# CPJKU/beat_this

Measured on AMD Instinct MI355X. Metric: audio-seconds processed/sec, higher is better.
Workload: dtype f32 activations, f16x3 products (3 x f16 MFMA on hi+lo operand halves, f32 accumulate); main-layer attention P.V: 2 x, probabilities as fp16 hi parts

## Files before the change

beat_this_amd/_lib.py:

```python
from __future__ import annotations

import ctypes as C
import os
import subprocess

import torch

PKG_DIR = os.path.dirname(os.path.abspath(__file__))
LIB_PATH = os.path.join(PKG_DIR, "libbeat_this_amd.so")
if os.environ.get("BT_DEV") == "1" and os.environ.get("BT_LIB_PATH"):
    LIB_PATH = os.environ["BT_LIB_PATH"]
SOURCES = ["gemm.hip", "gemm2.hip", "gemm3.hip", "gemm_mx8.hip", "attn.hip", "attn2.hip", "fused.hip", "fused2.hip", "qkv_front.hip", "frontend.hip", "logmel.hip",
           "tail.hip", "dbn.hip", "metrics.hip", "loss.hip", "data.hip", "train.hip", "optim.hip", "engine.hip"]
HEADERS = ["common.h", "chain.h", "kernels.h", "dropout.h", "train_mixed.inc", "attn_x3_loop.inc", "attn_hq2_loop.inc", os.path.join("..", "..", "include", "beat_this_amd.h")]

BT_OK, BT_ERR_ARG, BT_ERR_HIP, BT_ERR_WORKSPACE = 0, -1, -2, -3
ABI_VERSION = 600
PREC_F32, PREC_HALF, PREC_F32X3 = 0, 1, 3
OPT_X3_ATTN_P16, OPT_X3_GEMM_FP8, OPT_WS_GUARD = 1, 2, 3
MAX_LAYERS = 32
PROFILE_CATEGORIES = ["stem", "qkv_gemm", "attn_flash", "out_gemm", "ff1_gemm", "ff2_gemm", "conv_gemm",
                      "linear_gemm", "head", "ff_fused", "attn_freq_fused", "layer_tail"]

GEMM_EPI_STORE, GEMM_EPI_RESID, GEMM_EPI_QKV = 0, 1, 2
GEMM_F_RMS, GEMM_F_BIAS, GEMM_F_GELU, GEMM_F_OUT_F32, GEMM_F_A_F32, GEMM_F_CONV, GEMM_F_ROWMAP = 1, 2, 4, 8, 16, 32, 64


class PairWeights(C.Structure):
    _fields_ = [("dim", C.c_int32), ("heads", C.c_int32), ("w_qkvg", C.c_void_p * 2), ("b_gates", C.c_void_p),
                ("w_out", C.c_void_p * 2), ("w_ff1", C.c_void_p * 2), ("b_ff1", C.c_void_p),
                ("w_ff2", C.c_void_p * 2), ("b_ff2", C.c_void_p),
                ("w_ff_frag", C.c_void_p * 2), ("w_qkv_frag", C.c_void_p),
                ("w_outff_frag", C.c_void_p * 2), ("w_attnff_frag", C.c_void_p * 2),
                ("w_tail_frag", C.c_void_p),
                ("w_outff_frag_x3", C.c_void_p), ("w_attnff_frag_x3", C.c_void_p),
                ("w_qkvg_x3", C.c_void_p), ("w_out_x3", C.c_void_p), ("w_ff1_x3", C.c_void_p), ("w_ff2_x3", C.c_void_p),
                ("w_qkv_frag_x3", C.c_void_p),
                ("w_qkvg_f8", C.c_void_p), ("w_out_f8", C.c_void_p), ("w_ff1_f8", C.c_void_p), ("w_ff2_f8", C.c_void_p)]


class ModelDesc(C.Structure):
    _fields_ = [("transformer_dim", C.c_int32), ("n_layers", C.c_int32), ("sum_head", C.c_int32),
                ("partial_transformers", C.c_int32),
                ("bn1_scale", C.c_void_p), ("bn1_shift", C.c_void_p), ("stem_w", C.c_void_p), ("stem_b", C.c_void_p),
                ("front", (PairWeights * 2) * 3),
                ("conv_w", (C.c_void_p * 2) * 3), ("conv_b", C.c_void_p * 3),
                ("lin_w", C.c_void_p * 2), ("lin_b", C.c_void_p),
                ("layers", PairWeights * MAX_LAYERS),
                ("head_w", C.c_void_p), ("head_b", C.c_float * 2), ("rope", C.c_void_p), ("ff_mult", C.c_int32),
                ("norm_out_g", C.c_void_p), ("head_w_raw", C.c_void_p),
                ("conv_w_x3", C.c_void_p * 3), ("lin_w_x3", C.c_void_p), ("rope_len", C.c_int32)]


class LogmelTables(C.Structure):
    _fields_ = [("window", C.c_void_p), ("twiddle", C.c_void_p), ("mel_start", C.c_void_p),
                ("mel_len", C.c_void_p), ("mel_w", C.c_void_p)]


class GemmArgs(C.Structure):
    _fields_ = [("A", C.c_void_p), ("lda", C.c_int64), ("W", C.c_void_p), ("M", C.c_int32), ("N", C.c_int32),
                ("K", C.c_int32), ("epi", C.c_int32), ("flags", C.c_int32), ("bias", C.c_void_p),
                ("out", C.c_void_p), ("ldo", C.c_int64), ("x", C.c_void_p), ("ldx", C.c_int64),
                ("conv_C2", C.c_int32), ("conv_T", C.c_int32), ("conv_F", C.c_int32), ("gates", C.c_void_p),
                ("inner", C.c_int32), ("heads", C.c_int32), ("rope", C.c_void_p), ("pdiv", C.c_int32),
                ("pmod", C.c_int32), ("map_T", C.c_int32), ("map_F", C.c_int32)]


class AttnArgs(C.Structure):
    _fields_ = [("qkv", C.c_void_p), ("ld", C.c_int64), ("gates", C.c_void_p), ("out", C.c_void_p),
                ("n_seq", C.c_int32), ("L", C.c_int32), ("heads", C.c_int32), ("inner", C.c_int32),
                ("o_div", C.c_int32), ("o_outer", C.c_int64), ("o_inner", C.c_int64), ("o_tok", C.c_int64)]


class AttnFragArgs(C.Structure):
    _fields_ = [("q", C.c_void_p), ("k", C.c_void_p), ("v", C.c_void_p), ("gates", C.c_void_p), ("out", C.c_void_p),
                ("n_seq", C.c_int32), ("L", C.c_int32), ("heads", C.c_int32), ("inner", C.c_int32),
                ("nbp", C.c_int32), ("o_div", C.c_int32), ("o_outer", C.c_int64), ("o_inner", C.c_int64),
                ("o_tok", C.c_int64), ("x3", C.c_int32), ("out_f32", C.c_int32), ("status", C.c_void_p),
                ("scratch", C.c_void_p)]


class Gemm3Args(C.Structure):
    _fields_ = [("A", C.c_void_p), ("lda", C.c_int64), ("M", C.c_int32), ("K", C.c_int32), ("W", C.c_void_p),
                ("N", C.c_int32), ("epi", C.c_int32), ("bias", C.c_void_p), ("ssq_in", C.c_void_p),
                ("ssq_parts", C.c_int32), ("out", C.c_void_p), ("ldo", C.c_int64), ("x", C.c_void_p),
                ("ldx", C.c_int64), ("xb", C.c_void_p), ("ssq_out", C.c_void_p), ("n_seq", C.c_int32),
                ("L", C.c_int32), ("nbp", C.c_int32), ("heads", C.c_int32), ("rope", C.c_void_p), ("qf", C.c_void_p),
                ("kf", C.c_void_p), ("vf", C.c_void_p), ("gates", C.c_void_p), ("b_gates", C.c_void_p),
                ("no_resid", C.c_int32), ("gelu", C.c_int32), ("conv_C2", C.c_int32),
                ("conv_T", C.c_int32), ("conv_F", C.c_int32), ("x3", C.c_int32), ("status", C.c_void_p)]


class A2BPlan(C.Structure):
    _fields_ = [("n22", C.c_int64), ("n_frames", C.c_int64), ("result_words", C.c_int64), ("B", C.c_int32), ("T", C.c_int32),
                ("ws_bytes", C.c_size_t), ("off_wave22", C.c_size_t), ("off_spect", C.c_size_t), ("off_chunks", C.c_size_t),
                ("off_chunk_logits", C.c_size_t), ("off_logits", C.c_size_t), ("off_result", C.c_size_t),
                ("off_forward", C.c_size_t), ("forward_bytes", C.c_size_t)]


class TrainItem(C.Structure):
    _fields_ = [("row", C.c_int64), ("ann_begin", C.c_int64), ("ann_end", C.c_int64), ("n", C.c_int32),
                ("start_frame", C.c_int32), ("op_begin", C.c_int32), ("op_end", C.c_int32), ("has_downbeats", C.c_int32),
                ("reserved", C.c_int32)]


class TrainOp(C.Structure):
    _fields_ = [("start", C.c_int32), ("length", C.c_int32), ("kind", C.c_int32), ("part_begin", C.c_int32),
                ("part_end", C.c_int32)]


class TrainPart(C.Structure):
    _fields_ = [("new_off", C.c_int32), ("old_off", C.c_int32)]


class TrainArgs(C.Structure):
    _fields_ = [("B", C.c_int32), ("T", C.c_int32), ("dim", C.c_int32), ("hidden", C.c_int32), ("rope_len", C.c_int32),
                ("residual", C.c_int32), ("sum_head", C.c_int32), ("reserved", C.c_int32), ("rope", C.c_void_p),
                ("gamma", C.c_void_p), ("w1", C.c_void_p), ("b1", C.c_void_p), ("w2", C.c_void_p), ("b2", C.c_void_p),
                ("w3", C.c_void_p), ("x", C.c_void_p), ("y", C.c_void_p), ("y2", C.c_void_p), ("save_o", C.c_void_p),
                ("save_lse", C.c_void_p), ("gy", C.c_void_p), ("gy2", C.c_void_p), ("gx", C.c_void_p), ("g_gamma", C.c_void_p),
                ("g_w1", C.c_void_p), ("g_b1", C.c_void_p), ("g_w2", C.c_void_p), ("g_b2", C.c_void_p), ("g_w3", C.c_void_p),
                ("ws", C.c_void_p), ("ws_bytes", C.c_size_t)]


class TrainDropout(C.Structure):
    _fields_ = [("p", C.c_float), ("reserved", C.c_uint32), ("seed", C.c_uint64), ("stream", C.c_uint64)]


class OptimTensor(C.Structure):
    _fields_ = [("param", C.c_void_p), ("offset", C.c_int64), ("numel", C.c_int64), ("group", C.c_int32), ("reserved", C.c_int32)]


class OptimChunk(C.Structure):
    _fields_ = [("tensor", C.c_int32), ("chunk", C.c_int32)]


class OptimGroup(C.Structure):
    _fields_ = [("decay", C.c_float), ("one_minus_beta1", C.c_float), ("beta2", C.c_float), ("one_minus_beta2", C.c_float),
                ("step_size", C.c_float), ("bias2_sqrt", C.c_float), ("eps", C.c_float), ("reserved", C.c_float)]


OPTIM_MAX_GROUPS = 8


class OptimHyper(C.Structure):
    _fields_ = [("n_groups", C.c_int32), ("zero_grads", C.c_int32), ("grad_scale", C.c_float), ("reserved", C.c_int32),
                ("g", OptimGroup * OPTIM_MAX_GROUPS)]


G3_FF1, G3_RESID, G3_QKV = 0, 1, 2
UNIT_STEM, UNIT_PARTIAL, UNIT_CONV, UNIT_LINEAR, UNIT_ATTN, UNIT_FF, UNIT_NORM, UNIT_FRONT_ATTN, UNIT_FRONT_FF = range(9)
TRAIN_UNIT_HEAD = 16
TRAIN_DW_ROWS, TRAIN_CS_ROWS, TRAIN_ATTN_BLOCK = 1024, 64, 64
DROP_ATTN_P, DROP_ATTN_OUT, DROP_FF_HIDDEN, DROP_FF_OUT = range(4)
OPTIM_CHUNK, OPTIM_NORM_SLICE = 4096, 4096

EXPORTS = {
    "bt_last_error": (C.c_char_p, []),
    "bt_version": (C.c_int, []),
    "bt_half_is_bf16": (C.c_int, []),
    "bt_struct_sizes": (None, [C.POINTER(C.c_int32)]),
    "bt_engine_create": (C.c_int, [C.POINTER(ModelDesc), C.POINTER(C.c_void_p)]),
    "bt_engine_destroy": (None, [C.c_void_p]),
    "bt_engine_set_option": (C.c_int, [C.c_void_p, C.c_int, C.c_int]),
    "bt_engine_get_option": (C.c_int, [C.c_void_p, C.c_int, C.POINTER(C.c_int)]),
    "bt_workspace_bytes": (C.c_size_t, [C.c_void_p, C.c_int, C.c_int, C.c_int]),
    "bt_workspace_regions": (C.c_int, [C.c_void_p, C.c_int, C.c_int, C.c_int, C.POINTER(C.c_int64), C.c_int]),
    "bt_forward": (C.c_int, [C.c_void_p, C.c_void_p, C.c_int, C.c_void_p, C.c_int, C.c_int, C.c_void_p, C.c_size_t,
                             C.c_void_p, C.c_void_p]),
    "bt_forward_stages": (C.c_int, [C.c_void_p, C.c_void_p, C.c_int, C.c_int, C.c_int, C.c_void_p, C.c_int, C.c_int, C.c_void_p,
                                    C.c_size_t, C.c_void_p, C.c_void_p, C.c_void_p]),
    "bt_forward_unit": (C.c_int, [C.c_void_p, C.c_void_p, C.c_int, C.c_int, C.c_int, C.c_void_p, C.c_void_p, C.c_int, C.c_int,
                                  C.c_void_p, C.c_size_t]),
    "bt_split_chunks": (C.c_int, [C.c_void_p, C.c_void_p, C.c_int64, C.c_void_p, C.c_int, C.c_int, C.c_void_p]),
    "bt_aggregate": (C.c_int, [C.c_void_p, C.c_void_p, C.c_void_p, C.c_void_p, C.c_int, C.c_int, C.c_int, C.c_int64,
                               C.c_void_p, C.c_void_p]),
    "bt_logmel": (C.c_int, [C.c_void_p, C.POINTER(LogmelTables), C.c_void_p, C.c_int64, C.c_void_p]),
    "bt_resample": (C.c_int, [C.c_void_p, C.c_void_p, C.c_int64, C.c_int, C.c_int, C.c_void_p, C.c_int, C.c_void_p,
                              C.c_int64]),
    "bt_peaks": (C.c_int, [C.c_void_p, C.c_void_p, C.c_int64, C.c_int, C.c_void_p, C.c_void_p]),
    "bt_deduplicate_peaks_host": (C.c_int, [C.c_void_p, C.c_int, C.c_double, C.c_void_p, C.POINTER(C.c_int32)]),
    "bt_postprocess_host": (C.c_int, [C.c_void_p, C.c_int, C.c_void_p, C.c_int, C.c_double, C.c_void_p,
                                      C.POINTER(C.c_int32), C.c_void_p, C.POINTER(C.c_int32)]),
    "bt_audio2beats_plan": (C.c_int, [C.c_void_p, C.c_int64, C.c_int, C.c_int, C.c_int, C.POINTER(A2BPlan)]),
    "bt_audio2beats_enqueue": (C.c_int, [C.c_void_p, C.c_void_p, C.c_int, C.POINTER(LogmelTables), C.c_void_p, C.c_int64, C.c_int, C.c_int,
                                         C.c_void_p, C.c_int, C.c_void_p, C.c_size_t, C.c_void_p, C.c_int]),
    "bt_profile_begin": (None, [C.c_void_p]),
    "bt_profile_end": (C.c_int, [C.c_void_p, C.c_void_p, C.c_void_p, C.c_int]),
    "bt_resample_batch": (C.c_int, [C.c_void_p, C.c_void_p, C.c_int, C.c_int64, C.c_int, C.c_int, C.c_void_p, C.c_int,
                                    C.c_void_p]),
    "bt_logmel_batch": (C.c_int, [C.c_void_p, C.POINTER(LogmelTables), C.c_void_p, C.c_int, C.c_int64, C.c_void_p]),
    "bt_split_chunks_batch": (C.c_int, [C.c_void_p, C.c_void_p, C.c_void_p, C.c_int, C.c_int, C.c_void_p]),
    "bt_aggregate_batch": (C.c_int, [C.c_void_p, C.c_void_p, C.c_void_p, C.c_void_p, C.c_void_p, C.c_int, C.c_int64,
                                     C.c_int, C.c_int, C.c_void_p, C.c_void_p]),
    "bt_peaks_batch": (C.c_int, [C.c_void_p, C.c_void_p, C.c_void_p, C.c_int, C.c_void_p, C.c_void_p]),
    "bt_peaks_host": (C.c_int, [C.c_void_p, C.c_int64, C.c_void_p, C.POINTER(C.c_int32)]),
    "bt_gemm": (C.c_int, [C.c_void_p, C.c_int, C.POINTER(GemmArgs)]),
    "bt_attention": (C.c_int, [C.c_void_p, C.c_int, C.POINTER(AttnArgs)]),
    "bt_gemm3": (C.c_int, [C.c_void_p, C.POINTER(Gemm3Args)]),
    "bt_gemm_mx8": (C.c_int, [C.c_void_p, C.c_void_p, C.c_void_p, C.c_void_p, C.c_void_p, C.c_void_p, C.c_int, C.c_int, C.c_int, C.c_int64]),
    "bt_attn_frag_blocks": (C.c_int, [C.c_int]),
    "bt_attention_frag": (C.c_int, [C.c_void_p, C.POINTER(AttnFragArgs)]),
    "bt_qkv_front": (C.c_int, [C.c_void_p, C.c_int, C.POINTER(PairWeights), C.c_void_p, C.c_void_p, C.c_int, C.c_int, C.c_int,
                               C.c_void_p, C.c_void_p, C.c_void_p, C.c_void_p, C.c_int]),
    "bt_outff_fused": (C.c_int, [C.c_void_p, C.c_int, C.POINTER(PairWeights), C.c_void_p, C.c_void_p, C.c_int64, C.c_void_p]),
    "bt_attnff_fused": (C.c_int, [C.c_void_p, C.c_int, C.POINTER(PairWeights), C.c_void_p, C.c_void_p, C.c_int64]),
    "bt_layer_tail": (C.c_int, [C.c_void_p, C.POINTER(PairWeights), C.c_int, C.c_void_p, C.c_void_p, C.c_int64, C.c_void_p,
                                C.c_void_p]),
    "bt_ff_fused": (C.c_int, [C.c_void_p, C.c_int, C.POINTER(PairWeights), C.c_void_p, C.c_int64]),
    "bt_dbn_tables": (C.c_int, [C.c_double, C.c_double, C.c_double, C.c_int, C.c_double, C.c_double, C.c_double, C.c_void_p,
                                C.c_int, C.c_void_p, C.POINTER(C.c_size_t)]),
    "bt_dbn_workspace_bytes": (C.c_size_t, [C.c_void_p, C.c_int, C.c_int64]),
    "bt_dbn_decode": (C.c_int, [C.c_void_p, C.c_void_p, C.c_void_p, C.c_void_p, C.c_int, C.c_void_p, C.c_int, C.c_int64,
                                C.c_void_p, C.c_void_p, C.c_size_t]),
    "bt_dbn_viterbi": (C.c_int, [C.c_void_p, C.c_void_p, C.c_void_p, C.c_int, C.c_void_p, C.c_int64, C.c_void_p, C.c_void_p,
                                 C.c_void_p, C.c_size_t]),
    "bt_dbn_viterbi_host": (C.c_int, [C.c_void_p, C.c_int, C.c_void_p, C.c_int64, C.c_void_p, C.c_void_p]),
    "bt_dbn_host": (C.c_int, [C.c_void_p, C.c_void_p, C.c_void_p, C.c_int64, C.c_void_p, C.POINTER(C.c_int32)]),
    "bt_dbn_host_act": (C.c_int, [C.c_void_p, C.c_void_p, C.c_int64, C.c_void_p, C.POINTER(C.c_int32)]),
    "bt_beat_metrics_workspace_bytes": (C.c_size_t, [C.c_int, C.c_int64, C.c_int64]),
    "bt_beat_metrics": (C.c_int, [C.c_void_p, C.c_void_p, C.c_void_p, C.c_void_p, C.c_void_p, C.c_int, C.c_double, C.c_double,
                                  C.c_double, C.c_double, C.c_double, C.c_void_p, C.c_size_t, C.c_void_p]),
    "bt_beat_metrics_host": (C.c_int, [C.c_void_p, C.c_void_p, C.c_void_p, C.c_void_p, C.c_int, C.c_double, C.c_double,
                                       C.c_double, C.c_double, C.c_double, C.c_void_p]),
    "bt_bce_loss_workspace_bytes": (C.c_size_t, [C.c_int, C.c_int64]),
    "bt_bce_loss": (C.c_int, [C.c_void_p, C.c_int, C.c_int, C.c_float, C.c_void_p, C.c_void_p, C.c_int, C.c_void_p, C.c_int,
                              C.c_void_p, C.c_int, C.c_void_p, C.c_int, C.c_int64, C.c_int64, C.c_void_p, C.c_size_t,
                              C.c_void_p, C.c_void_p, C.c_void_p, C.c_int, C.c_void_p, C.c_void_p]),
    "bt_bce_loss_backward": (C.c_int, [C.c_void_p, C.c_void_p, C.c_int64, C.c_void_p, C.c_int, C.c_int64, C.c_void_p, C.c_int]),
    "bt_bce_loss_host": (C.c_int, [C.c_int, C.c_int, C.c_float, C.c_void_p, C.c_int, C.c_void_p, C.c_int, C.c_void_p, C.c_int,
                                   C.c_void_p, C.c_int, C.c_void_p, C.c_void_p, C.c_void_p, C.c_void_p, C.c_void_p]),
    "bt_train_batch_struct_sizes": (None, [C.POINTER(C.c_int32)]),
    "bt_train_batch": (C.c_int, [C.c_void_p, C.c_void_p, C.c_int, C.c_int64, C.c_void_p, C.c_int, C.c_int, C.c_void_p, C.c_int,
                                 C.c_void_p, C.c_int, C.c_void_p, C.c_void_p, C.c_int64, C.c_double, C.c_void_p, C.c_int,
                                 C.c_void_p, C.c_void_p, C.c_void_p, C.c_void_p]),
    "bt_train_batch_host": (C.c_int, [C.c_void_p, C.c_int, C.c_int64, C.c_void_p, C.c_int, C.c_int, C.c_void_p, C.c_int,
                                      C.c_void_p, C.c_int, C.c_void_p, C.c_void_p, C.c_int64, C.c_double, C.c_void_p, C.c_int,
                                      C.c_void_p, C.c_void_p, C.c_void_p, C.c_void_p]),
    "bt_train_struct_sizes": (None, [C.POINTER(C.c_int32)]),
    "bt_train_workspace_bytes": (C.c_size_t, [C.c_int, C.c_int, C.c_int, C.c_int, C.c_int, C.c_int]),
    "bt_train_forward": (C.c_int, [C.c_void_p, C.c_int, C.POINTER(TrainArgs)]),
    "bt_train_backward": (C.c_int, [C.c_void_p, C.c_int, C.POINTER(TrainArgs)]),
    "bt_train_dropout_struct_sizes": (None, [C.POINTER(C.c_int32)]),
    "bt_train_workspace_bytes_dropout": (C.c_size_t, [C.c_int, C.c_int, C.c_int, C.c_int, C.c_int, C.c_int]),
    "bt_train_forward_dropout": (C.c_int, [C.c_void_p, C.c_int, C.POINTER(TrainArgs), C.POINTER(TrainDropout)]),
    "bt_train_backward_dropout": (C.c_int, [C.c_void_p, C.c_int, C.POINTER(TrainArgs), C.POINTER(TrainDropout)]),
    "bt_philox4x32_10_host": (None, [C.POINTER(C.c_uint32), C.POINTER(C.c_uint32), C.POINTER(C.c_uint32)]),
    "bt_dropout_mask_host": (C.c_int, [C.POINTER(TrainDropout), C.c_int, C.c_int, C.c_int, C.c_int, C.c_int, C.c_void_p]),
    "bt_train_workspace_bytes_mixed": (C.c_size_t, [C.c_int, C.c_int, C.c_int, C.c_int, C.c_int, C.c_int, C.c_int]),
    "bt_train_forward_mixed": (C.c_int, [C.c_void_p, C.c_int, C.POINTER(TrainArgs), C.POINTER(TrainDropout)]),
    "bt_train_backward_mixed": (C.c_int, [C.c_void_p, C.c_int, C.POINTER(TrainArgs), C.POINTER(TrainDropout)]),
    "bt_train_matmul_mixed": (C.c_int, [C.c_void_p, C.c_int, C.c_void_p, C.c_void_p, C.c_int, C.c_int, C.c_int, C.c_void_p]),
    "bt_optim_struct_sizes": (None, [C.POINTER(C.c_int32)]),
    "bt_optim_plan": (C.c_int, [C.c_int, C.c_void_p, C.c_void_p, C.c_void_p, C.c_int, C.c_void_p, C.POINTER(C.c_int64), C.c_void_p,
                                C.c_int64, C.POINTER(C.c_int64)]),
    "bt_grad_norm_workspace_bytes": (C.c_size_t, [C.c_int64]),
    "bt_grad_norm": (C.c_int, [C.c_void_p, C.c_void_p, C.c_int64, C.c_float, C.c_float, C.c_void_p, C.c_size_t, C.c_void_p]),
    "bt_adamw_step": (C.c_int, [C.c_void_p, C.c_void_p, C.c_int, C.c_void_p, C.c_int64, C.c_void_p, C.c_void_p, C.c_void_p,
                                C.c_int64, C.POINTER(OptimHyper), C.c_void_p]),
    "bt_grad_norm_host": (C.c_int, [C.c_void_p, C.c_int64, C.c_float, C.c_float, C.c_void_p]),
    "bt_adamw_step_host": (C.c_int, [C.c_void_p, C.c_int, C.c_void_p, C.c_int64, C.c_void_p, C.c_void_p, C.c_void_p, C.c_int64,
                                     C.POINTER(OptimHyper), C.c_void_p]),
}


HIPCC_FLAGS = ["-Xclang", "-target-feature", "-Xclang", "-packed-fp32-ops", "-mllvm", "-amdgpu-mfma-vgpr-form"]
FLAGS_BY_SOURCE = {"tail.hip": ["-Xclang", "-target-feature", "-Xclang", "-packed-fp32-ops"],
                   "dbn.hip": HIPCC_FLAGS + ["-ffp-contract=off"],
                   "metrics.hip": HIPCC_FLAGS + ["-ffp-contract=off"],
                   "loss.hip": HIPCC_FLAGS + ["-ffp-contract=off"],
                   "data.hip": HIPCC_FLAGS + ["-ffp-contract=off"],
                   "optim.hip": HIPCC_FLAGS + ["-ffp-contract=off"]}
EXTRA_DEFINES = (["-DBT_DEV"] if os.environ.get("BT_DEV_BUILD") == "1" else []) + os.environ.get("BT_DEFINES", "").split()


def build(force: bool = False, verbose: bool = False, lib_path: str | None = None, obj_dir: str | None = None,
          defines=()) -> str:
    from concurrent.futures import ThreadPoolExecutor

    src_dir = os.path.join(PKG_DIR, "csrc")
    obj_dir = obj_dir or os.path.join(PKG_DIR, "build")
    LIB_PATH = lib_path or os.path.join(PKG_DIR, "libbeat_this_amd.so")
    hdrs = [os.path.join(src_dir, h) for h in HEADERS] + [os.path.abspath(__file__)]
    hdr_time = max(os.path.getmtime(h) for h in hdrs)
    hipcc = os.environ.get("HIPCC", "/opt/rocm/bin/hipcc")
    common = [hipcc, "--offload-arch=gfx950", "-O3", "-std=c++17", "-fPIC"]
    import hashlib

    stamp_path = os.path.join(obj_dir, "flags.stamp")
    stamp = hashlib.sha256(repr((common[1:], HIPCC_FLAGS, sorted(FLAGS_BY_SOURCE.items()), EXTRA_DEFINES, list(defines))).encode()).hexdigest()
    try:
        if open(stamp_path).read().strip() != stamp:
            force = True
    except OSError:
        force = True
    todo, objs = [], []
    for name in SOURCES:
        src = os.path.join(src_dir, name)
        obj = os.path.join(obj_dir, name.replace(".hip", ".o"))
        objs.append(obj)
        if force or not os.path.exists(obj) or os.path.getmtime(obj) < max(os.path.getmtime(src), hdr_time):
            todo.append((src, obj))
    build.last_rebuilt = [os.path.basename(j[0]) for j in todo]
    if not todo and os.path.exists(LIB_PATH) and all(os.path.getmtime(LIB_PATH) >= os.path.getmtime(o) for o in objs):
        return LIB_PATH
    os.makedirs(obj_dir, exist_ok=True)
    if os.path.exists(stamp_path):
        os.unlink(stamp_path)

    def compile_one(job):
        flags = FLAGS_BY_SOURCE.get(os.path.basename(job[0]), HIPCC_FLAGS)
        cmd = [*common, *flags, *EXTRA_DEFINES, *defines, "-c", job[0], "-o", job[1]]
        if verbose:
            print(" ".join(cmd), flush=True)
        r = subprocess.run(cmd, stderr=subprocess.PIPE, text=True)
        err = "\n".join(l for l in r.stderr.splitlines() if "-packed-fp32-ops' is not a recognized feature" not in l)
        if err.strip():
            print(err, flush=True)
        if r.returncode:
            raise subprocess.CalledProcessError(r.returncode, cmd)

    with ThreadPoolExecutor(max_workers=min(len(todo), os.cpu_count() or 4) or 1) as pool:
        list(pool.map(compile_one, todo))
    cmd = [hipcc, "--offload-arch=gfx950", "-shared", "-fPIC", *objs, "-o", LIB_PATH]
    if verbose:
        print(" ".join(cmd), flush=True)
    subprocess.run(cmd, check=True)
    with open(stamp_path, "w") as f:
        f.write(stamp + "\n")
    return LIB_PATH


build.last_rebuilt = []


def device_asm_command(src: str, out: str, defines=()) -> list:
    flags = FLAGS_BY_SOURCE.get(os.path.basename(src), HIPCC_FLAGS)
    return [os.environ.get("HIPCC", "/opt/rocm/bin/hipcc"), "--offload-arch=gfx950", "-O3", "-std=c++17", "-fPIC", *flags,
            *EXTRA_DEFINES, *defines, "-S", "--cuda-device-only", src, "-o", out]


_lib = None


def lib():
    global _lib
    if _lib is None:
        if not os.path.exists(LIB_PATH):
            raise ImportError(
                f"{LIB_PATH} is missing: build it with `python -c 'import __graft_entry__ as g; g.build()'` "
                "(needs hipcc); beat_this_amd has no CPU/PyTorch fallback")
        handle = C.CDLL(LIB_PATH, mode=C.RTLD_GLOBAL)
        handle.bt_version.restype = C.c_int
        if handle.bt_version() != ABI_VERSION:
            raise ImportError(f"{LIB_PATH} has ABI version {handle.bt_version()}, this binding needs {ABI_VERSION}: rebuild it "
                              "(python -c 'import __graft_entry__ as g; g.build()')")
        for name, (res, args) in EXPORTS.items():
            fn = getattr(handle, name)
            fn.restype = res
# ... 42 lines not shown
```

beat_this_amd/csrc/chain.h:

```cpp
#pragma once
#include "common.h"

template <typename T> DEVI Frag<T> ldg_frag(const T* p);
template <> DEVI Frag<float> ldg_frag<float>(const float* p) {
  Frag<float> f;
#pragma unroll
  for (int i = 0; i < 4; ++i) f.v[i] = reinterpret_cast<const f32x4*>(p)[i];
  return f;
}
template <> DEVI Frag<hf> ldg_frag<hf>(const hf* p) {
  Frag<hf> f;
  f.v[0] = reinterpret_cast<const hfx8*>(p)[0];
  f.v[1] = reinterpret_cast<const hfx8*>(p)[1];
  return f;
}

DEVI void split_hl8(Frag<hl>& f, int h, const float (&v)[8]) {
  typedef __attribute__((ext_vector_type(4))) unsigned int u32x4;
  unsigned hi[4], lo[4];
#pragma unroll
  for (int j = 0; j < 4; j += 2)
    split_hl4(v[2 * j] * OpScale<hl>::ACT, v[2 * j + 1] * OpScale<hl>::ACT, v[2 * j + 2] * OpScale<hl>::ACT,
              v[2 * j + 3] * OpScale<hl>::ACT, hi[j], lo[j], hi[j + 1], lo[j + 1]);
  f.v[h] = __builtin_bit_cast(hfx8, u32x4{hi[0], hi[1], hi[2], hi[3]});
  f.v[2 + h] = __builtin_bit_cast(hfx8, u32x4{lo[0], lo[1], lo[2], lo[3]});
}
template <> DEVI Frag<hl> ldg_frag<hl>(const hl* p) {
  Frag<hl> f;
  const f32x4* q = reinterpret_cast<const f32x4*>(p);
#pragma unroll
  for (int h = 0; h < 2; ++h) {
    const f32x4 a = q[2 * h], b = q[2 * h + 1];
    const float v[8] = {a[0], a[1], a[2], a[3], b[0], b[1], b[2], b[3]};
    split_hl8(f, h, v);
  }
  return f;
}

template <typename T> DEVI Frag<T> ldx_frag(const float* p, bool ok, float& ss);
template <> DEVI Frag<float> ldx_frag<float>(const float* p, bool ok, float& ss) {
  Frag<float> f;
#pragma unroll
  for (int i = 0; i < 4; ++i) {
    f.v[i] = ok ? reinterpret_cast<const f32x4*>(p)[i] : f32x4{0.f, 0.f, 0.f, 0.f};
#pragma unroll
    for (int j = 0; j < 4; ++j) ss = fmaf(f.v[i][j], f.v[i][j], ss);
  }
  return f;
}
template <> DEVI Frag<hf> ldx_frag<hf>(const float* p, bool ok, float& ss) {
  Frag<hf> f;
#pragma unroll
  for (int h = 0; h < 2; ++h) {
#pragma unroll
    for (int i = 0; i < 2; ++i) {
      f32x4 v = ok ? reinterpret_cast<const f32x4*>(p)[2 * h + i] : f32x4{0.f, 0.f, 0.f, 0.f};
#pragma unroll
      for (int j = 0; j < 4; ++j) {
        ss = fmaf(v[j], v[j], ss);
        f.v[h][4 * i + j] = (hf)v[j];
      }
    }
  }
  return f;
}

template <> DEVI Frag<hl> ldx_frag<hl>(const float* p, bool ok, float& ss) {
  Frag<hl> f;
#pragma unroll
  for (int h = 0; h < 2; ++h) {
    const f32x4 a = ok ? reinterpret_cast<const f32x4*>(p)[2 * h] : f32x4{0.f, 0.f, 0.f, 0.f};
    const f32x4 b = ok ? reinterpret_cast<const f32x4*>(p)[2 * h + 1] : f32x4{0.f, 0.f, 0.f, 0.f};
    const float v[8] = {a[0], a[1], a[2], a[3], b[0], b[1], b[2], b[3]};
#pragma unroll
    for (int j = 0; j < 8; ++j) ss = fmaf(v[j], v[j], ss);
    split_hl8(f, h, v);
  }
  return f;
}

template <typename T> DEVI Frag<T> pack_frag(const float (&h)[16]);
template <> DEVI Frag<float> pack_frag<float>(const float (&h)[16]) {
  Frag<float> f;
#pragma unroll
  for (int i = 0; i < 4; ++i) f.v[i] = f32x4{h[4 * i], h[4 * i + 1], h[4 * i + 2], h[4 * i + 3]};
  return f;
}
template <> DEVI Frag<hf> pack_frag<hf>(const float (&h)[16]) {
  Frag<hf> f;
#pragma unroll
  for (int s = 0; s < 2; ++s)
#pragma unroll
    for (int j = 0; j < 8; ++j) f.v[s][j] = (hf)h[8 * s + j];
  return f;
}

template <> DEVI Frag<hl> pack_frag<hl>(const float (&h)[16]) {
  Frag<hl> f;
#pragma unroll
  for (int s = 0; s < 2; ++s) {
    const float v[8] = {h[8 * s], h[8 * s + 1], h[8 * s + 2], h[8 * s + 3], h[8 * s + 4], h[8 * s + 5], h[8 * s + 6], h[8 * s + 7]};
    split_hl8(f, s, v);
  }
  return f;
}

DEVI void zero16(f32x16& a) {
#pragma unroll
  for (int r = 0; r < 16; ++r) a[r] = 0.f;
}

template <typename T> DEVI Frag<T> lds_frag(const char* tile, int lane);
template <> DEVI Frag<hf> lds_frag<hf>(const char* tile, int lane) {
  Frag<hf> f;
  f.v[0] = *reinterpret_cast<const hfx8*>(tile + lane * 16);
  f.v[1] = *reinterpret_cast<const hfx8*>(tile + 1024 + lane * 16);
  return f;
}
template <> DEVI Frag<hl> lds_frag<hl>(const char* tile, int lane) {
  Frag<hl> f;
#pragma unroll
  for (int i = 0; i < 4; ++i) f.v[i] = *reinterpret_cast<const hfx8*>(tile + i * 1024 + lane * 16);
  return f;
}
template <> DEVI Frag<float> lds_frag<float>(const char* tile, int lane) {
  Frag<float> f;
#pragma unroll
  for (int i = 0; i < 4; ++i) f.v[i] = *reinterpret_cast<const f32x4*>(tile + i * 1024 + lane * 16);
  return f;
}
```

beat_this_amd/csrc/engine.hip:

```cpp
#include <algorithm>
#include <cmath>
#include <cstddef>
#include <cstdio>
#include <cstring>
#include <mutex>
#include <string>
#include <vector>

#include "../../include/beat_this_amd.h"
#include "common.h"
#include "kernels.h"


static thread_local std::string g_err;
static int bt_set_error(int code, const std::string& msg) {
  g_err = msg;
  return code;
}
int bt_set_error_external(int code, const char* msg) { return bt_set_error(code, msg); }

namespace prof {
struct Rec { int cat; hipEvent_t a, b; };
struct State { bool on = false; std::vector<Rec> recs; };
struct Scope {
  State* st; size_t idx; hipStream_t s;
  Scope(State* state, int cat, hipStream_t stream) : st(state && state->on ? state : nullptr), idx(0), s(stream) {
    if (!st) return;
    Rec r; r.cat = cat;
    (void)hipEventCreate(&r.a); (void)hipEventCreate(&r.b);
    (void)hipEventRecord(r.a, s);
    idx = st->recs.size(); st->recs.push_back(r);
  }
  ~Scope() { if (st) (void)hipEventRecord(st->recs[idx].b, s); }
};
}

struct FwdGraph { int B, T, prec; void* ws; hipGraphExec_t exec; unsigned long stamp; };

struct bt_engine {
  bt_model_desc d;
  prof::State prof;
  std::mutex mu;
  std::vector<FwdGraph> graphs;
  unsigned long graph_clock = 0;
  hipStream_t cap_stream = nullptr;
  std::vector<int> warm;
  int x3_attn_p16 = 1;
  int x3_gemm_fp8 = 0;
  int ws_guard = 0;
};
enum { CAT_STEM = 0, CAT_QKV, CAT_ATTN_FLASH, CAT_OUT, CAT_FF1, CAT_FF2, CAT_CONV, CAT_LINEAR,
       CAT_HEAD, CAT_FF_FUSED, CAT_ATTN_FREQ_FUSED, CAT_LAYER_TAIL, CAT_COUNT };

namespace {

inline size_t align_up(size_t v, size_t a) { return (v + a - 1) / a * a; }

struct Workspace {
  float* xa; float* xb; float* xm; float* gates; void* xmb;
  void* qkv; void* ao; void* hid;
  void* qf; void* kf; void* vf; float* gates_h; int nbp;
  float* ssq[2];
  int* status;
  int* fix_mask;
  size_t total;
};

Workspace carve(char* base, int B, int T, int D, int ff_mult, int prec, size_t guard = 0,
                std::vector<int64_t>* regions = nullptr) {
  const bool x3 = prec == BT_PREC_F32X3;
  if (x3) prec = BT_PREC_F32;
  const size_t es = prec == BT_PREC_F32 ? 4 : 2;
  const size_t bt = (size_t)B * T;
  const size_t dmax = std::max<size_t>(1024, D);
  size_t off = 0;
  auto take = [&](size_t bytes) {
    size_t o = off;
    off += align_up(bytes, 256) + guard;
    if (regions) { regions->push_back((int64_t)o); regions->push_back((int64_t)(o + bytes)); }
    return base ? base + o : (char*)nullptr;
  };
  Workspace w;
  w.status = (int*)take(256);
  w.xa = (float*)take(bt * 1024 * 4);
  w.xb = (float*)take(bt * 1024 * 4);
  w.xm = (float*)take(bt * D * 4);
  w.xmb = take(bt * D * (x3 ? 4 : 2));
  w.gates = (float*)take(bt * std::max(32, D / 32) * 4);
  w.qkv = take(bt * 3 * dmax * es);
  w.ao = take(bt * dmax * es);
  w.hid = take(bt * std::max<size_t>(4 * 1024, (size_t)ff_mult * D) * es);
  w.nbp = attn_frag_blocks(T);
  w.qf = w.kf = w.vf = nullptr; w.gates_h = nullptr;
  if (prec == BT_PREC_HALF || x3) {
    const size_t sh = (size_t)B * std::max(32, D / 32);
    const size_t blk = x3 ? 4096 : 2048;
    w.qf = take(sh * w.nbp * blk); w.kf = take(sh * w.nbp * blk); w.vf = take(sh * w.nbp * blk);
    w.gates_h = (float*)take(sh * w.nbp * 32 * 4);
    w.fix_mask = x3 ? (int*)take(sh * w.nbp * 4) : nullptr;
    w.ssq[0] = (float*)take(bt * (D / 64 + 1) * 4);
    w.ssq[1] = (float*)take(bt * (D / 64 + 1) * 4);
  } else {
    w.ssq[0] = w.ssq[1] = nullptr;
    w.fix_mask = nullptr;
  }
  w.total = off;
  return w;
}

inline float* front_x(const Workspace& ws, int i) { return i & 1 ? ws.xb : ws.xa; }

StemP stem_params(const bt_model_desc& d, const float* spect, float* x, int B, int T) {
  StemP p;
  p.spect = spect; p.x = x; p.bn1_scale = d.bn1_scale; p.bn1_shift = d.bn1_shift;
  p.w = d.stem_w; p.bias = d.stem_b; p.B = B; p.T = T;
  return p;
}

GemmP conv_params(const bt_model_desc& d, int blk, int wp, const float* in, void* out, int B, int T, bool out_f32) {
  const int C = 32 << blk, F = 32 >> blk;
  GemmP g;
  memset(&g, 0, sizeof g);
  g.A = in; g.W = d.conv_w[blk][wp]; g.M = B * T * (F / 2); g.N = 2 * C; g.K = 6 * C;
  g.epi = GEMM_EPI_STORE; g.flags = GEMM_F_CONV | GEMM_F_A_F32 | GEMM_F_BIAS | GEMM_F_GELU | (out_f32 ? GEMM_F_OUT_F32 : 0);
  g.bias = d.conv_b[blk]; g.out = out; g.ldo = 2 * C;
  g.conv_C2 = 2 * C; g.conv_T = T; g.conv_F = F / 2;
  return g;
}

Gemm3P conv3_params(const bt_model_desc& d, const Workspace& ws, int blk, int B, int T, bool x3, bool out_half) {
  const int C = 32 << blk, F = 32 >> blk;
  float* out = front_x(ws, blk + 1);
  Gemm3P g;
  memset(&g, 0, sizeof g);
  g.A = ws.hid; g.lda = 2 * C; g.M = B * T * (F / 2); g.K = 6 * C; g.N = 2 * C;
  g.W = x3 ? d.conv_w_x3[blk] : d.conv_w[blk][BT_PREC_HALF];
  g.epi = G3_RESID; g.no_resid = 1; g.gelu = 1; g.bias = d.conv_b[blk]; g.ldx = 2 * C;
  g.conv_C2 = 2 * C; g.conv_T = T; g.conv_F = F / 2; g.x3 = x3; g.status = ws.status;
  g.x = out_half ? nullptr : out; g.xb = out_half ? (void*)out : nullptr;
  return g;
}

GemmP linear_params(const bt_model_desc& d, int wp, const float* in, float* out, void* xb, float* ssq_out, int B, int T) {
  GemmP g;
  memset(&g, 0, sizeof g);
  g.A = in; g.lda = 1024; g.W = d.lin_w[wp]; g.M = B * T; g.N = d.transformer_dim; g.K = 1024;
  g.epi = GEMM_EPI_STORE; g.flags = GEMM_F_A_F32 | GEMM_F_BIAS | GEMM_F_OUT_F32;
  g.bias = d.lin_b; g.out = out; g.ldo = d.transformer_dim; g.xb = xb; g.ssq_out = ssq_out;
  return g;
}

Gemm3P linear3_params(const bt_model_desc& d, const Workspace& ws, int B, int T, bool x3, bool out_f8) {
  const int D = d.transformer_dim;
  Gemm3P g;
  memset(&g, 0, sizeof g);
  g.A = front_x(ws, 3); g.lda = 1024; g.M = B * T; g.K = 1024; g.W = x3 ? d.lin_w_x3 : d.lin_w[BT_PREC_HALF]; g.N = D;
  g.epi = G3_RESID; g.no_resid = 1; g.bias = d.lin_b; g.x = ws.xm; g.ldx = D; g.xb = ws.xmb; g.ssq_out = ws.ssq[0];
  g.x3 = x3 ? 1 | (out_f8 ? G3_X3_OUT_F8 : 0) : 0; g.status = ws.status;
  return g;
}

HeadP head_params(const bt_model_desc& d, const float* x, const float* w, int prenorm, float* beat, float* downbeat, int M,
                  int* status) {
  HeadP p;
  p.x = x; p.w = w; p.b0 = d.head_b[0]; p.b1 = d.head_b[1];
  p.beat = beat; p.downbeat = downbeat; p.M = M; p.D = d.transformer_dim; p.sum_head = d.sum_head; p.prenorm = prenorm;
  p.status = status;
  return p;
}

template <class P>
void attn_rows(P& a, int B, int T, int F) {
  a.n_seq = B * F; a.L = T; a.o_div = F; a.o_outer = (long)T * F; a.o_inner = F > 1 ? 1 : 0; a.o_tok = F;
}

struct PairRoute {
  bool ff_fused;
  bool outff;
  bool split;
  bool time_frag;
};

struct FragLayer {
  bool qkv8;
  bool out8;
  bool ff8;
  bool next8;
  bool tail;
  bool shadow_dead;
};

enum { LAYERS_GENERIC, LAYERS_FRAG_HALF, LAYERS_FRAG_X3 };

struct Route {
  bool x3;
  int fp;
  int gp, wp;
  int x3_attn, x3_attn_front;
  bool half_shadow;
  int layers;
  struct Block { PairRoute freq, time; bool conv3; bool x_dead; } blk[3];
  bool lin3, lin_f8;
  struct Layer { PairRoute pair; FragLayer frag; } layer[BT_MAX_LAYERS];
};

#ifndef BT_SKIP_DEAD_STORES
#define BT_SKIP_DEAD_STORES 1
#endif
Route plan_route(const bt_engine& e, int B, int T, int prec, int first, int last, const Workspace& ws) {
  const bt_model_desc& d = e.d;
  const int D = d.transformer_dim;
  Route r;
  r.x3 = prec == BT_PREC_F32X3;
  r.fp = r.x3 ? BT_PREC_F32 : prec;
  r.gp = prec;
  r.wp = r.x3 ? BT_PREC_HALF : prec;
  r.x3_attn = r.x3 ? 4 | ((e.x3_attn_p16 == 1 || e.x3_attn_p16 == 2) ? BT_X3_P16 : 0) : 0;
  r.x3_attn_front = r.x3 ? 4 | (e.x3_attn_p16 >= 2 ? BT_X3_P16 : 0) : 0;
  auto pair = [&](const bt_pair_weights& w) {
    PairRoute p;
    p.ff_fused = w.dim <= 128 && w.w_ff_frag[r.fp];
    p.outff = p.ff_fused && w.w_outff_frag[r.fp] && w.w_attnff_frag[r.fp];
    p.split = r.x3 && w.w_outff_frag_x3 && w.w_attnff_frag_x3;
    p.time_frag = r.x3 ? p.outff && p.split && w.w_qkv_frag_x3 : p.ff_fused && r.fp == BT_PREC_HALF && w.w_qkv_frag;
    return p;
  };

  r.half_shadow = prec == BT_PREC_HALF && D >= 128 && D % 64 == 0;
  const long wide = (long)B * T * d.ff_mult * D;
  bool frag_x3 = r.x3 && D >= 128 && D % 128 == 0 && wide * 4 < 0x7fffffffL;
  for (int l = 0; frag_x3 && l < d.n_layers; ++l)
    frag_x3 = d.layers[l].w_qkvg_x3 && d.layers[l].w_out_x3 && d.layers[l].w_ff1_x3 && d.layers[l].w_ff2_x3;
  const bool frag_half = r.half_shadow && D % 128 == 0 && wide * 2 < 0x7fffffffL;
  r.layers = frag_x3 ? LAYERS_FRAG_X3 : frag_half ? LAYERS_FRAG_HALF : LAYERS_GENERIC;

  const bool lin3_fits = (frag_half || (frag_x3 && d.lin_w_x3)) && gemm3_supported(linear3_params(d, ws, B, T, frag_x3, false));
  for (int blk = 0; blk < 3; ++blk) {
    Route::Block& rb = r.blk[blk];
    rb.freq = pair(d.front[blk][0]);
    rb.time = pair(d.front[blk][1]);
    const Gemm3P cg = conv3_params(d, ws, blk, B, T, frag_x3, blk == 2 && lin3_fits);
    rb.conv3 = d.partial_transformers && rb.time.outff && (frag_x3 ? rb.time.split : frag_half) && cg.N >= 128 && cg.W &&
               gemm3_supported(cg);
    rb.x_dead = BT_SKIP_DEAD_STORES && rb.conv3 && frag_x3;
  }
  r.lin3 = lin3_fits && (!frag_x3 || r.blk[2].conv3);
  r.lin_f8 = r.lin3 && frag_x3 && e.x3_gemm_fp8 >= 2 && d.n_layers > 0 && d.layers[0].w_qkvg_f8;

  for (int l = 0; l < d.n_layers; ++l) {
    const bt_pair_weights& w = d.layers[l];
    FragLayer& f = r.layer[l].frag;
    r.layer[l].pair = pair(w);
    f.qkv8 = l == 0 ? first == 0 && r.lin_f8 : r.layer[l - 1].frag.next8;
    f.out8 = frag_x3 && e.x3_gemm_fp8 >= 2 && w.w_out_f8;
    f.ff8 = frag_x3 && e.x3_gemm_fp8 >= 1 && w.w_ff1_f8 && w.w_ff2_f8;
    f.next8 = frag_x3 && e.x3_gemm_fp8 >= 2 && l + 1 < d.n_layers && d.layers[l + 1].w_qkvg_f8 && w.w_ff2_f8;
    f.tail = frag_half && w.w_tail_frag && layer_tail_supported(D, d.ff_mult * D);
    f.shadow_dead = BT_SKIP_DEAD_STORES && frag_x3 && last == 2 && l == d.n_layers - 1;
  }
  return r;
}

#define CHECK_RC(what)                                                         \
  if (_rc != 0) {                                                              \
    char buf[160];                                                             \
    snprintf(buf, sizeof buf, "%s failed (code %d: %s)", what, _rc,            \
             _rc > 0 ? hipGetErrorString((hipError_t)_rc) : "bad arguments");  \
    return bt_set_error(_rc > 0 ? BT_ERR_HIP : BT_ERR_ARG, buf);               \
  }
#define LAUNCH(expr, what) \
  do { int _rc = (expr); CHECK_RC(what) } while (0)
#define LAUNCH_CAT(cat, st, expr, what) \
  do { int _rc; { prof::Scope _ps(pf, cat, st); _rc = (expr); } CHECK_RC(what) } while (0)


int check_rows(long M) {
  return M > 0x7fffffffL ? bt_set_error(BT_ERR_ARG, "batch too large for one forward call") : BT_OK;
}

int out_proj(prof::State* pf, const bt_pair_weights& pw, const Route& r, float* x, void* xs, const Workspace& ws, long M,
             hipStream_t s) {
  const int C = pw.dim;
  GemmP g;
  memset(&g, 0, sizeof g);
  g.A = ws.ao; g.lda = C; g.W = pw.w_out[r.wp]; g.M = (int)M; g.N = C; g.K = C;
  g.epi = GEMM_EPI_RESID; g.flags = 0; g.x = x; g.ldx = C; g.xb = xs;
  LAUNCH_CAT(CAT_OUT, s, launch_gemm(g, r.gp, s), "out-proj gemm");
  return BT_OK;
}

int qkv_attn(prof::State* pf, const bt_pair_weights& pw, const Route& r, const float* rope, float* x, void* xs,
             const Workspace& ws, int B, int T, int F, hipStream_t s) {
  const int C = pw.dim, H = pw.heads;
  GemmP g;
  memset(&g, 0, sizeof g);
  g.A = xs ? xs : (const void*)x; g.lda = C; g.W = pw.w_qkvg[r.wp]; g.M = B * T * F; g.N = 3 * C + H; g.K = C;
  g.epi = GEMM_EPI_QKV; g.flags = GEMM_F_RMS | (xs ? 0 : GEMM_F_A_F32) | (F > 1 ? GEMM_F_ROWMAP : 0);
  g.bias = pw.b_gates; g.out = ws.qkv; g.ldo = 3 * C; g.gates = ws.gates; g.inner = C; g.heads = H;
  g.rope = rope; g.map_T = T; g.map_F = F; g.pdiv = F; g.pmod = T;
  LAUNCH_CAT(CAT_QKV, s, launch_gemm(g, r.gp, s), "qkv gemm");
  AttnP a;
  memset(&a, 0, sizeof a);
  a.qkv = ws.qkv; a.ld = 3 * C; a.gates = ws.gates; a.out = ws.ao; a.heads = H; a.inner = C;
  attn_rows(a, B, T, F);
  LAUNCH_CAT(CAT_ATTN_FLASH, s, launch_attn_flash(a, r.gp, s), F > 1 ? "time attention" : "attention");
  return BT_OK;
}

int ff_half(prof::State* pf, const bt_pair_weights& pw, const PairRoute& pr, const Route& r, float* x, void* xs,
            const Workspace& ws, long M, int ff_mult, hipStream_t s) {
  const int C = pw.dim, HID = ff_mult * C;
  if (pr.ff_fused) {
    FusedFFP ff;
    ff.x = x; ff.M = M; ff.C = C; ff.wfrag = pw.w_ff_frag[r.fp]; ff.b1 = pw.b_ff1; ff.b2 = pw.b_ff2; ff.xb = xs;
    LAUNCH_CAT(CAT_FF_FUSED, s, launch_ff_fused(ff, r.fp, s), "fused feed-forward");
    return BT_OK;
  }
  GemmP g;
  memset(&g, 0, sizeof g);
  g.A = xs ? xs : (const void*)x; g.lda = C; g.W = pw.w_ff1[r.wp]; g.M = (int)M; g.N = HID; g.K = C;
  g.epi = GEMM_EPI_STORE; g.flags = GEMM_F_RMS | (xs ? 0 : GEMM_F_A_F32) | GEMM_F_BIAS | GEMM_F_GELU;
  g.bias = pw.b_ff1; g.out = ws.hid; g.ldo = HID;
  LAUNCH_CAT(CAT_FF1, s, launch_gemm(g, r.gp, s), "ff1 gemm");
  memset(&g, 0, sizeof g);
  g.A = ws.hid; g.lda = HID; g.W = pw.w_ff2[r.wp]; g.M = (int)M; g.N = C; g.K = HID;
  g.epi = GEMM_EPI_RESID; g.flags = GEMM_F_BIAS; g.bias = pw.b_ff2; g.x = x; g.ldx = C; g.xb = xs;
  LAUNCH_CAT(CAT_FF2, s, launch_gemm(g, r.gp, s), "ff2 gemm");
  return BT_OK;
}

int generic_layer(prof::State* pf, const bt_pair_weights& pw, const PairRoute& pr, const Route& r, const float* rope, float* x,
                  void* xs, const Workspace& ws, int B, int T, int ff_mult, bool attn, bool ff, hipStream_t s) {
  const long M = (long)B * T;
  if (int rc = check_rows(M)) return rc;
  if (attn) {
    if (int rc = qkv_attn(pf, pw, r, rope, x, xs, ws, B, T, 1, s)) return rc;
    if (int rc = out_proj(pf, pw, r, x, xs, ws, M, s)) return rc;
  }
  return ff ? ff_half(pf, pw, pr, r, x, xs, ws, M, ff_mult, s) : BT_OK;
}

int freq_half(prof::State* pf, const bt_pair_weights& pw, const PairRoute& pr, const Route& r, const float* rope, float* x,
              int B, int T, int F, hipStream_t s) {
  const long M = (long)B * T * F;
  if (int rc = check_rows(M)) return rc;
  if (!pr.outff) return bt_set_error(BT_ERR_ARG, "frequency-direction half needs bt_pair_weights.w_attnff_frag");
  FusedAttnFFP f;
  f.x = x; f.M = M; f.C = pw.dim; f.b_gates = pw.b_gates; f.rope = rope;
  f.wfrag = pr.split ? pw.w_attnff_frag_x3 : pw.w_attnff_frag[r.fp]; f.b1 = pw.b_ff1; f.b2 = pw.b_ff2;
  LAUNCH_CAT(CAT_ATTN_FREQ_FUSED, s, launch_attnff_fused(f, pr.split ? BT_PREC_F32X3 : r.fp, s),
             "fused frequency attention + feed-forward");
  return BT_OK;
}

int time_half(prof::State* pf, const bt_pair_weights& pw, const PairRoute& pr, const Route& r, const float* rope, float* x,
              const Workspace& ws, int B, int T, int F, void* shadow, bool shadow_only, hipStream_t s) {
  const long M = (long)B * T * F;
  if (int rc = check_rows(M)) return rc;
  if (pr.time_frag) {
    QkvFrontP qp;
    memset(&qp, 0, sizeof qp);
    qp.x = x; qp.B = B; qp.T = T; qp.F = F; qp.C = pw.dim; qp.wfrag = r.x3 ? pw.w_qkv_frag_x3 : pw.w_qkv_frag;
    qp.b_gates = pw.b_gates; qp.rope = rope;
    qp.q = ws.qf; qp.k = ws.kf; qp.v = ws.vf; qp.gates = ws.gates_h; qp.nbp = ws.nbp;
    qp.x3 = r.x3; qp.status = ws.status;
    LAUNCH_CAT(CAT_QKV, s, launch_qkv_front(qp, s), "frontend qkv projection");
    AttnFragP a;
    memset(&a, 0, sizeof a);
    a.q = ws.qf; a.k = ws.kf; a.v = ws.vf; a.gates = ws.gates_h; a.out = ws.ao; a.heads = pw.heads; a.inner = pw.dim;
    a.nbp = ws.nbp; attn_rows(a, B, T, F);
    a.x3 = r.x3_attn_front; a.out_f32 = 1; a.status = ws.status; a.fix_mask = ws.fix_mask;
    LAUNCH_CAT(CAT_ATTN_FLASH, s, launch_attn_frag(a, s), "time attention");
  } else if (int rc = qkv_attn(pf, pw, r, rope, x, nullptr, ws, B, T, F, s)) {
    return rc;
  }
  if (pr.outff) {
    FusedOutFFP f;
    f.x = x; f.M = M; f.C = pw.dim; f.ao = ws.ao; f.wfrag = pr.split ? pw.w_outff_frag_x3 : pw.w_outff_frag[r.fp];
    f.b1 = pw.b_ff1; f.b2 = pw.b_ff2; f.xb = shadow; f.abl = 0; f.shadow_only = shadow && shadow_only && pr.split;
    LAUNCH_CAT(CAT_FF_FUSED, s, launch_outff_fused(f, pr.split ? BT_PREC_F32X3 : r.fp, s), "fused out-projection + feed-forward");
    return BT_OK;
  }
  if (int rc = out_proj(pf, pw, r, x, nullptr, ws, M, s)) return rc;
  return ff_half(pf, pw, pr, r, x, nullptr, ws, M, 4, s);
}

int frag_layer(prof::State* pf, const bt_pair_weights& pw, const FragLayer& f, const Route& r, const float* rope,
               const Workspace& ws, int B, int T, int ff_mult, hipStream_t s) {
  const int D = pw.dim, H = pw.heads, HID = ff_mult * D;
  const int M = B * T;
  const int parts = D / 64;
  int* status = r.x3 ? ws.status : nullptr;
  auto w = [&](const void* const* half, const void* hl32, const void* hl8, bool f8) { return !r.x3 ? half[BT_PREC_HALF] : f8 ? hl8 : hl32; };
  Gemm3P g;
  memset(&g, 0, sizeof g);
  g.A = ws.xmb; g.lda = D; g.M = M; g.K = D; g.W = w(pw.w_qkvg, pw.w_qkvg_x3, pw.w_qkvg_f8, f.qkv8); g.N = 3 * D + H; g.epi = G3_QKV;
  g.ssq_in = ws.ssq[0]; g.ssq_parts = parts; g.x3 = r.x3 | (f.qkv8 ? G3_X3_F8 : 0); g.status = status;
  g.n_seq = B; g.L = T; g.nblk = (T + 31) / 32; g.nbp = ws.nbp; g.heads = H; g.inner = D; g.rope = rope;
  g.qf = ws.qf; g.kf = ws.kf; g.vf = ws.vf; g.gates = ws.gates_h; g.b_gates = pw.b_gates;
  LAUNCH_CAT(CAT_QKV, s, launch_gemm3(g, s), r.x3 ? "qkv gemm (hi + lo)" : "qkv gemm");
  AttnFragP a;
  memset(&a, 0, sizeof a);
  a.q = ws.qf; a.k = ws.kf; a.v = ws.vf; a.gates = ws.gates_h; a.out = ws.ao; a.heads = H; a.inner = D; a.nbp = ws.nbp;
  attn_rows(a, B, T, 1);
  a.x3 = r.x3_attn; a.out_f32 = f.out8 ? 2 : 0; a.status = status; a.fix_mask = ws.fix_mask;
  LAUNCH_CAT(CAT_ATTN_FLASH, s, launch_attn_frag(a, s), r.x3 ? "attention (hi + lo)" : "attention");
  if (f.tail) {
    LayerTailP t;
    t.x = ws.xm; t.M = M; t.C = D; t.hidden = HID; t.ao = ws.ao; t.wfrag = pw.w_tail_frag; t.b1 = pw.b_ff1; t.b2 = pw.b_ff2;
    t.xb = ws.xmb; t.ssq_out = ws.ssq[0];
    LAUNCH_CAT(CAT_LAYER_TAIL, s, launch_layer_tail(t, s), "layer tail (out-projection + feed-forward)");
    return BT_OK;
  }
  memset(&g, 0, sizeof g);
  g.A = ws.ao; g.lda = D; g.M = M; g.K = D; g.W = w(pw.w_out, pw.w_out_x3, pw.w_out_f8, f.out8); g.N = D; g.epi = G3_RESID;
  g.x3 = r.x3 | (f.out8 ? G3_X3_F8 : 0) | (f.ff8 ? G3_X3_OUT_F8 : 0); g.status = status;
  g.x = ws.xm; g.ldx = D; g.xb = ws.xmb; g.ssq_out = ws.ssq[1];
  LAUNCH_CAT(CAT_OUT, s, launch_gemm3(g, s), r.x3 ? "out-proj gemm (hi + lo)" : "out-proj gemm");
  memset(&g, 0, sizeof g);
  g.A = ws.xmb; g.lda = D; g.M = M; g.K = D; g.W = w(pw.w_ff1, pw.w_ff1_x3, pw.w_ff1_f8, f.ff8); g.N = HID; g.epi = G3_FF1;
  g.x3 = r.x3 | (f.ff8 ? G3_X3_F8 | G3_X3_OUT_F8 : 0); g.status = status;
  g.bias = pw.b_ff1; g.ssq_in = ws.ssq[1]; g.ssq_parts = parts; g.out = ws.hid; g.ldo = HID;
  LAUNCH_CAT(CAT_FF1, s, launch_gemm3(g, s), r.x3 ? "ff1 gemm (hi + lo)" : "ff1 gemm");
  memset(&g, 0, sizeof g);
  g.A = ws.hid; g.lda = HID; g.M = M; g.K = HID; g.W = w(pw.w_ff2, pw.w_ff2_x3, pw.w_ff2_f8, f.ff8); g.N = D; g.epi = G3_RESID;
  g.x3 = r.x3 | (f.ff8 ? G3_X3_F8 : 0) | (f.next8 ? G3_X3_OUT_F8 : 0); g.status = status;
  g.bias = pw.b_ff2; g.x = ws.xm; g.ldx = D; g.xb = f.shadow_dead ? nullptr : ws.xmb; g.ssq_out = f.shadow_dead ? nullptr : ws.ssq[0];
  LAUNCH_CAT(CAT_FF2, s, launch_gemm3(g, s), r.x3 ? "ff2 gemm (hi + lo)" : "ff2 gemm");
  return BT_OK;
}

int frontend(prof::State* pf, const bt_model_desc& d, const Route& r, const float* spect, const Workspace& ws, int B, int T,
             hipStream_t s) {
  const StemP sp = stem_params(d, spect, front_x(ws, 0), B, T);
  LAUNCH_CAT(CAT_STEM, s, launch_stem(sp, s), "stem");
  for (int blk = 0; blk < 3; ++blk) {
    const Route::Block& rb = r.blk[blk];
    float* x = front_x(ws, blk);
    if (d.partial_transformers) {
      if (int rc = freq_half(pf, d.front[blk][0], rb.freq, r, d.rope, x, B, T, 32 >> blk, s)) return rc;
      if (int rc = time_half(pf, d.front[blk][1], rb.time, r, d.rope, x, ws, B, T, 32 >> blk, rb.conv3 ? ws.hid : nullptr, rb.x_dead, s))
        return rc;
    }
    if (rb.conv3) {
      const Gemm3P g = conv3_params(d, ws, blk, B, T, r.layers == LAYERS_FRAG_X3, blk == 2 && r.lin3);
      LAUNCH_CAT(CAT_CONV, s, launch_gemm3(g, s), "frontend conv gemm");
    } else {
      const GemmP g = conv_params(d, blk, r.wp, x, front_x(ws, blk + 1), B, T, !(blk == 2 && r.lin3));
      LAUNCH_CAT(CAT_CONV, s, launch_gemm(g, r.gp, s), "frontend conv gemm");
    }
  }
  if (r.lin3) {
    const Gemm3P g = linear3_params(d, ws, B, T, r.layers == LAYERS_FRAG_X3, r.lin_f8);
    LAUNCH_CAT(CAT_LINEAR, s, launch_gemm3(g, s), "frontend linear gemm");
    return BT_OK;
  }
  const GemmP g = linear_params(d, r.wp, front_x(ws, 3), ws.xm, r.half_shadow ? ws.xmb : nullptr,
                                r.layers == LAYERS_FRAG_HALF ? ws.ssq[0] : nullptr, B, T);
  LAUNCH_CAT(CAT_LINEAR, s, launch_gemm(g, r.gp, s), "frontend linear gemm");
  if (r.layers == LAYERS_FRAG_X3)
    LAUNCH_CAT(CAT_LINEAR, s, launch_shadow_ssq(ws.xm, ws.xmb, ws.ssq[0], (long)B * T, d.transformer_dim, s, 1), "hl32 shadow of the residual stream");
  return BT_OK;
}

}

extern "C" {

const char* bt_last_error(void) { return g_err.c_str(); }
int bt_version(void) { return BT_ABI_VERSION; }
int bt_half_is_bf16(void) { return BT_HALF_IS_BF16; }
void bt_struct_sizes(int32_t* out) {
  out[0] = (int32_t)sizeof(bt_pair_weights); out[1] = (int32_t)sizeof(bt_model_desc);
  out[2] = (int32_t)sizeof(bt_logmel_tables); out[3] = (int32_t)sizeof(bt_gemm_args);
  out[4] = (int32_t)sizeof(bt_attn_args); out[5] = (int32_t)offsetof(bt_model_desc, layers);
  out[6] = (int32_t)offsetof(bt_model_desc, rope);
  out[7] = (int32_t)sizeof(bt_attn_frag_args);
  out[8] = (int32_t)sizeof(bt_gemm3_args);
}

int bt_engine_create(const bt_model_desc* desc, bt_engine** out) {
  if (!desc || !out) return bt_set_error(BT_ERR_ARG, "null argument");
  if (desc->transformer_dim % 32 || desc->transformer_dim < 32 || desc->transformer_dim > 1024 ||
      desc->n_layers < 0 || desc->n_layers > BT_MAX_LAYERS || desc->ff_mult < 1 || desc->ff_mult > 16)
    return bt_set_error(BT_ERR_ARG, "unsupported transformer_dim / n_layers / ff_mult");
  bt_engine* e = new bt_engine;
  e->d = *desc;
  *out = e;
  return BT_OK;
}
static void drop_graphs(bt_engine* e) {
  for (auto& g : e->graphs) (void)hipGraphExecDestroy(g.exec);
  e->graphs.clear();
  e->warm.clear();
}
void bt_engine_destroy(bt_engine* e) {
  if (!e) return;
  for (auto& r : e->prof.recs) { (void)hipEventDestroy(r.a); (void)hipEventDestroy(r.b); }
  drop_graphs(e);
  if (e->cap_stream) (void)hipStreamDestroy(e->cap_stream);
  delete e;
}

int bt_engine_set_option(bt_engine* e, int option, int value) {
  if (!e) return bt_set_error(BT_ERR_ARG, "null argument");
  std::lock_guard<std::mutex> lock(e->mu);
  if (option == BT_OPT_X3_ATTN_P16 && value >= 0 && value <= 3) { if (e->x3_attn_p16 != value) drop_graphs(e); e->x3_attn_p16 = value; return BT_OK; }
  if (option == BT_OPT_X3_GEMM_FP8 && value >= 0 && value <= 2) { if (e->x3_gemm_fp8 != value) drop_graphs(e); e->x3_gemm_fp8 = value; return BT_OK; }
  if (option == BT_OPT_WS_GUARD && value >= 0 && value % 256 == 0) { if (e->ws_guard != value) drop_graphs(e); e->ws_guard = value; return BT_OK; }
  return bt_set_error(BT_ERR_ARG, "unknown engine option / value");
}
int bt_engine_get_option(const bt_engine* e, int option, int* value) {
  if (!e || !value) return bt_set_error(BT_ERR_ARG, "null argument");
  if (option == BT_OPT_X3_ATTN_P16) { *value = e->x3_attn_p16; return BT_OK; }
  if (option == BT_OPT_X3_GEMM_FP8) { *value = e->x3_gemm_fp8; return BT_OK; }
  if (option == BT_OPT_WS_GUARD) { *value = e->ws_guard; return BT_OK; }
  return bt_set_error(BT_ERR_ARG, "unknown engine option");
}

size_t bt_workspace_bytes(const bt_engine* e, int B, int T, int prec) {
  if (!e || B <= 0 || T <= 0) return 0;
  return carve(nullptr, B, T, e->d.transformer_dim, e->d.ff_mult, prec, (size_t)e->ws_guard).total;
}

int bt_workspace_regions(const bt_engine* e, int B, int T, int prec, int64_t* begin_end, int max) {
  if (!e || B <= 0 || T <= 0 || max < 0 || (max > 0 && !begin_end)) return bt_set_error(BT_ERR_ARG, "bad argument to bt_workspace_regions");
  if (prec != BT_PREC_F32 && prec != BT_PREC_HALF && prec != BT_PREC_F32X3) return bt_set_error(BT_ERR_ARG, "unknown precision");
  std::vector<int64_t> r;
  carve(nullptr, B, T, e->d.transformer_dim, e->d.ff_mult, prec, (size_t)e->ws_guard, &r);
  const int n = (int)(r.size() / 2);
  for (int i = 0; i < std::min(n, max); ++i) { begin_end[2 * i] = r[2 * i]; begin_end[2 * i + 1] = r[2 * i + 1]; }
  return n;
}

int bt_forward(bt_engine* e, void* stream, int prec, const float* d_spect, int B, int T, void* d_ws, size_t ws_bytes,
               float* d_beat, float* d_downbeat) {
  return bt_forward_stages(e, stream, prec, 0, 2, d_spect, B, T, d_ws, ws_bytes, nullptr, d_beat, d_downbeat);
}

int bt_forward_stages(bt_engine* e, void* stream, int prec, int first, int last, const float* d_spect, int B, int T, void* d_ws,
                      size_t ws_bytes, float* d_out, float* d_beat, float* d_downbeat) {
  if (!e || !d_spect || !d_ws) return bt_set_error(BT_ERR_ARG, "null argument");
  if (first < 0 || last > 2 || first > last) return bt_set_error(BT_ERR_ARG, "stages: need 0 <= first <= last <= 2");
  if (last == 2 ? (!d_beat || !d_downbeat) : !d_out) return bt_set_error(BT_ERR_ARG, "null output");
  const int max_T = e->d.rope_len > 0 ? e->d.rope_len : 1536;
  if (B <= 0 || T <= 0 || T > max_T)
    return bt_set_error(BT_ERR_ARG, "need B >= 1 and 1 <= T <= " + std::to_string(max_T) + " (bt_model_desc.rope_len: rows of the rotary table)");
  if (prec != BT_PREC_F32 && prec != BT_PREC_HALF && prec != BT_PREC_F32X3)
    return bt_set_error(BT_ERR_ARG, "unknown precision");
  const bt_model_desc& d = e->d;
  prof::State* pf = &e->prof;
  const int D = d.transformer_dim;
  const Workspace ws = carve((char*)d_ws, B, T, D, d.ff_mult, prec, (size_t)e->ws_guard);
  if (ws.total > ws_bytes) return bt_set_error(BT_ERR_WORKSPACE, "workspace too small");
  if (prec == BT_PREC_F32X3 && BT_HALF_IS_BF16) return bt_set_error(BT_ERR_ARG, "BT_PREC_F32X3 needs an IEEE fp16 build");
  const Route r = plan_route(*e, B, T, prec, first, last, ws);
  hipStream_t s = (hipStream_t)stream;
  if (r.x3) LAUNCH(launch_clear_words(ws.status, 1, s), "clearing the range flag");
  int* status = r.x3 ? ws.status : nullptr;

  const size_t xm_bytes = (size_t)B * T * D * 4;
  if (first == 2) {
    if (!d.head_w_raw) return bt_set_error(BT_ERR_ARG, "stage entry at task_heads needs head_w_raw");
    const HeadP hp = head_params(d, d_spect, d.head_w_raw, 1, d_beat, d_downbeat, B * T, nullptr);
    LAUNCH_CAT(CAT_HEAD, s, launch_head(hp, s), "head");
    return BT_OK;
  }
  if (first == 1) {
    if (hipMemcpyAsync(ws.xm, d_spect, xm_bytes, hipMemcpyDeviceToDevice, s) != hipSuccess)
      return bt_set_error(BT_ERR_HIP, "copy of the stage input");
    if (r.half_shadow)
      LAUNCH_CAT(CAT_LINEAR, s, launch_shadow_ssq(ws.xm, ws.xmb, r.layers == LAYERS_FRAG_HALF ? ws.ssq[0] : nullptr, (long)B * T, D, s), "stage entry");
    if (r.layers == LAYERS_FRAG_X3) LAUNCH_CAT(CAT_LINEAR, s, launch_shadow_ssq(ws.xm, ws.xmb, ws.ssq[0], (long)B * T, D, s, 1), "stage entry");
  }
  if (first == 0)
    if (int rc = frontend(pf, d, r, d_spect, ws, B, T, s)) return rc;
  if (last == 0) {
    if (hipMemcpyAsync(d_out, ws.xm, xm_bytes, hipMemcpyDeviceToDevice, s) != hipSuccess)
      return bt_set_error(BT_ERR_HIP, "copy of the stage output");
    if (r.x3) LAUNCH_CAT(CAT_HEAD, s, launch_finite_rows(ws.xm, (long)B * T, D, ws.status, s), "range check of the stage output");
    return BT_OK;
  }
  for (int l = 0; l < d.n_layers; ++l) {
    const Route::Layer& rl = r.layer[l];
    const int rc = r.layers == LAYERS_GENERIC
                       ? generic_layer(pf, d.layers[l], rl.pair, r, d.rope, ws.xm, r.half_shadow ? ws.xmb : nullptr, ws, B, T,
                                       d.ff_mult, true, true, s)
                       : frag_layer(pf, d.layers[l], rl.frag, r, d.rope, ws, B, T, d.ff_mult, s);
    if (rc) return rc;
  }
  if (last == 1) {
    if (!d.norm_out_g) return bt_set_error(BT_ERR_ARG, "stage exit after transformer_blocks needs norm_out_g");
    LAUNCH_CAT(CAT_HEAD, s, launch_norm_out(ws.xm, d.norm_out_g, d_out, (long)B * T, D, s, status), "final norm");
    return BT_OK;
  }
  const HeadP hp = head_params(d, ws.xm, d.head_w, 0, d_beat, d_downbeat, B * T, status);
  LAUNCH_CAT(CAT_HEAD, s, launch_head(hp, s), "head");
  return BT_OK;
}

int bt_forward_unit(bt_engine* e, void* stream, int prec, int unit, int index, const float* d_in, float* d_out, int B, int T,
                    void* d_ws, size_t ws_bytes) {
  if (!e || !d_in || !d_out || !d_ws) return bt_set_error(BT_ERR_ARG, "null argument");
  const bt_model_desc& d = e->d;
  const int max_T = d.rope_len > 0 ? d.rope_len : 1536;
  if (B <= 0 || T <= 0 || T > max_T) return bt_set_error(BT_ERR_ARG, "need B >= 1 and 1 <= T <= bt_model_desc.rope_len");
  if (prec == BT_PREC_F32X3) prec = BT_PREC_F32;
  if (prec != BT_PREC_F32 && prec != BT_PREC_HALF) return bt_set_error(BT_ERR_ARG, "unknown precision");
  prof::State* pf = &e->prof;
  const int D = d.transformer_dim;
  const Workspace ws = carve((char*)d_ws, B, T, D, d.ff_mult, prec, (size_t)e->ws_guard);
  if (ws.total > ws_bytes) return bt_set_error(BT_ERR_WORKSPACE, "workspace too small");
  const Route r = plan_route(*e, B, T, prec, 0, 0, ws);
  hipStream_t s = (hipStream_t)stream;
  const bool block_unit = unit == BT_UNIT_PARTIAL || unit == BT_UNIT_CONV;
  const bool layer_unit = unit == BT_UNIT_ATTN || unit == BT_UNIT_FF;
  const bool leaf_unit = unit == BT_UNIT_FRONT_ATTN || unit == BT_UNIT_FRONT_FF;
  if (leaf_unit && (index < 0 || index > 5 || !d.partial_transformers)) return bt_set_error(BT_ERR_ARG, "partial-transformer leaf index out of range");
  if (block_unit && (index < 0 || index > 2)) return bt_set_error(BT_ERR_ARG, "frontend block index out of range");
  if (layer_unit && (index < 0 || index >= d.n_layers)) return bt_set_error(BT_ERR_ARG, "layer index out of range");
  auto copy_in = [&](size_t bytes) -> int {
    if (d_in != d_out && hipMemcpyAsync(d_out, d_in, bytes, hipMemcpyDeviceToDevice, s) != hipSuccess)
      return bt_set_error(BT_ERR_HIP, "copy of the unit's input");
    return BT_OK;
  };
  switch (unit) {
    case BT_UNIT_STEM: {
      const StemP sp = stem_params(d, d_in, d_out, B, T);
      LAUNCH_CAT(CAT_STEM, s, launch_stem(sp, s), "stem");
      return BT_OK;
    }
    case BT_UNIT_PARTIAL: {
      if (!d.partial_transformers) return bt_set_error(BT_ERR_ARG, "this model has no partial transformers");
      const Route::Block& rb = r.blk[index];
      if (int rc = copy_in((size_t)B * T * 1024 * 4)) return rc;
      if (int rc = freq_half(pf, d.front[index][0], rb.freq, r, d.rope, d_out, B, T, 32 >> index, s)) return rc;
      return time_half(pf, d.front[index][1], rb.time, r, d.rope, d_out, ws, B, T, 32 >> index, nullptr, false, s);
    }
    case BT_UNIT_CONV: {
      const GemmP g = conv_params(d, index, r.wp, d_in, d_out, B, T, true);
      LAUNCH_CAT(CAT_CONV, s, launch_gemm(g, r.gp, s), "frontend conv gemm");
      return BT_OK;
    }
    case BT_UNIT_LINEAR: {
      const GemmP g = linear_params(d, r.wp, d_in, d_out, nullptr, nullptr, B, T);
      LAUNCH_CAT(CAT_LINEAR, s, launch_gemm(g, r.gp, s), "frontend linear gemm");
      return BT_OK;
    }
    case BT_UNIT_ATTN:
    case BT_UNIT_FF: {
      if (int rc = copy_in((size_t)B * T * D * 4)) return rc;
      return generic_layer(pf, d.layers[index], r.layer[index].pair, r, d.rope, d_out, nullptr, ws, B, T, d.ff_mult,
                           unit == BT_UNIT_ATTN, unit == BT_UNIT_FF, s);
    }
    case BT_UNIT_FRONT_ATTN:
    case BT_UNIT_FRONT_FF: {
      const bt_pair_weights& pw = d.front[index >> 1][index & 1];
      const Route::Block& rb = r.blk[index >> 1];
      if (int rc = copy_in((size_t)B * T * pw.dim * 4)) return rc;
      return generic_layer(pf, pw, index & 1 ? rb.time : rb.freq, r, d.rope, d_out, nullptr, ws, B, T, 4,
                           unit == BT_UNIT_FRONT_ATTN, unit == BT_UNIT_FRONT_FF, s);
    }
    case BT_UNIT_NORM:
      if (!d.norm_out_g) return bt_set_error(BT_ERR_ARG, "bt_model_desc.norm_out_g is not set");
      LAUNCH_CAT(CAT_HEAD, s, launch_norm_out(d_in, d.norm_out_g, d_out, (long)B * T, D, s), "final norm");
      return BT_OK;
    default:
      return bt_set_error(BT_ERR_ARG, "unknown unit");
  }
// ... 184 lines not shown
  plan->off_wave22 = take(up == down ? 0 : (size_t)n22 * 4);
  plan->off_spect = take((size_t)n * 128 * 4);
  plan->off_logits = take((size_t)2 * n * 4);
  plan->off_result = take((size_t)plan->result_words * 4);
  plan->ws_bytes = off;
  return BT_OK;
}

int bt_audio2beats_enqueue(bt_engine* e, void* stream, int prec, const bt_logmel_tables* t, const float* d_audio, int64_t n_in,
                           int up, int down, const float* d_filter, int half_len, void* d_ws, size_t ws_bytes, int32_t* h_result,
                           int use_graph) {
  if (!e || !t || !d_audio || !d_ws || !h_result) return bt_set_error(BT_ERR_ARG, "null argument");
  if (up != down && (!d_filter || half_len < 0)) return bt_set_error(BT_ERR_ARG, "resampling needs the polyphase filter");
  bt_a2b_plan pl;
  if (int rc = bt_audio2beats_plan(e, n_in, up, down, prec, &pl)) return rc;
  if (pl.ws_bytes > ws_bytes) return bt_set_error(BT_ERR_WORKSPACE, "workspace too small (bt_audio2beats_plan)");
  std::lock_guard<std::mutex> lock(e->mu);
  const int max_T = e->d.rope_len > 0 ? e->d.rope_len : 1536;
  if (pl.T > max_T) return bt_set_error(BT_ERR_ARG, "chunk longer than the rotary table");
  hipStream_t s = (hipStream_t)stream;
  char* ws = (char*)d_ws;
  float* wave22 = (float*)(ws + pl.off_wave22);
  float* spect = (float*)(ws + pl.off_spect);
  float* chunks = (float*)(ws + pl.off_chunks);
  float* cb = (float*)(ws + pl.off_chunk_logits);
  float* cd = cb + (size_t)pl.B * pl.T;
  float* beat = (float*)(ws + pl.off_logits);
  float* downb = beat + pl.n_frames;
  int32_t* res = (int32_t*)(ws + pl.off_result);
  void* fws = ws + pl.off_forward;
  const int border = 6;
  const float* a22 = d_audio;
  if (up != down) {
    const bt_span_t one{d_audio, (long)n_in, 0, (long)pl.n22};
    LAUNCH(launch_resample(one, nullptr, 1, (long)pl.n22, up, down, d_filter, half_len, wave22, s), "resample");
    a22 = wave22;
  }
  LogmelP lp;
  fill_logmel(lp, t, spect);
  lp.one = bt_span_t{a22, (long)pl.n22, 0, (long)pl.n_frames};
  lp.tracks = nullptr; lp.n_tracks = 1; lp.max_frames = (long)pl.n_frames;
  LAUNCH(launch_logmel(lp, s), "logmel");
  LAUNCH(launch_split(spect, (long)pl.n_frames, nullptr, nullptr, pl.B, pl.T, chunks, s, border), "split");
  const int warm_key = prec << 8 | pl.B;
  const bool graphable = use_graph && pl.T == 1500 && pl.B <= 16 && !e->prof.on &&
                         std::find(e->warm.begin(), e->warm.end(), warm_key) != e->warm.end();
  FwdGraph* g = nullptr;
  if (graphable) {
    for (auto& c : e->graphs)
      if (c.B == pl.B && c.T == pl.T && c.prec == prec && c.ws == d_ws) g = &c;
    if (!g) {
      hipGraph_t graph = nullptr;
      if (!e->cap_stream && hipStreamCreateWithFlags(&e->cap_stream, hipStreamNonBlocking) != hipSuccess) e->cap_stream = nullptr;
      if (e->cap_stream && hipStreamBeginCapture(e->cap_stream, hipStreamCaptureModeThreadLocal) == hipSuccess) {
        const int rc = bt_forward_stages(e, e->cap_stream, prec, 0, 2, chunks, pl.B, pl.T, fws, pl.forward_bytes, nullptr, cb, cd);
        const hipError_t he = hipStreamEndCapture(e->cap_stream, &graph);
        hipGraphExec_t exec = nullptr;
        if (rc == BT_OK && he == hipSuccess && graph && hipGraphInstantiate(&exec, graph, nullptr, nullptr, 0) == hipSuccess) {
          if (e->graphs.size() >= 8) {
            size_t old = 0;
            for (size_t i = 1; i < e->graphs.size(); ++i)
              if (e->graphs[i].stamp < e->graphs[old].stamp) old = i;
            (void)hipGraphExecDestroy(e->graphs[old].exec);
            e->graphs.erase(e->graphs.begin() + old);
          }
          e->graphs.push_back(FwdGraph{pl.B, pl.T, prec, d_ws, exec, 0});
          g = &e->graphs.back();
        }
        if (graph) (void)hipGraphDestroy(graph);
        (void)hipGetLastError();
      }
    }
  }
  if (g) {
    g->stamp = ++e->graph_clock;
    if (hipGraphLaunch(g->exec, s) != hipSuccess) return bt_set_error(BT_ERR_HIP, "replay of the captured forward");
  } else {
    if (int rc = bt_forward_stages(e, s, prec, 0, 2, chunks, pl.B, pl.T, fws, pl.forward_bytes, nullptr, cb, cd)) return rc;
    if (pl.T == 1500 && pl.B <= 16 && std::find(e->warm.begin(), e->warm.end(), warm_key) == e->warm.end()) e->warm.push_back(warm_key);
  }
  LAUNCH(launch_aggregate(cb, cd, nullptr, nullptr, nullptr, 1, pl.B, pl.T, border, (long)pl.n_frames, beat, downb, s), "aggregate");
  LAUNCH(launch_peaks(beat, (long)pl.n_frames, nullptr, 2, res, res + 2 * pl.n_frames, s), "peaks");
  if (prec == BT_PREC_F32X3) {
    if (hipMemcpyAsync(res + 2 * pl.n_frames + 2, fws, 4, hipMemcpyDeviceToDevice, s) != hipSuccess)
      return bt_set_error(BT_ERR_HIP, "copy of the range flag");
  } else if (hipMemsetAsync(res + 2 * pl.n_frames + 2, 0, 4, s) != hipSuccess) {
    return bt_set_error(BT_ERR_HIP, "clearing the range flag");
  }
  if (hipMemcpyAsync(h_result, res, (size_t)pl.result_words * 4, hipMemcpyDeviceToHost, s) != hipSuccess)
    return bt_set_error(BT_ERR_HIP, "device-to-host copy of the result");
  return BT_OK;
}

void bt_profile_begin(bt_engine* e) {
  if (!e) return;
  for (auto& r : e->prof.recs) { (void)hipEventDestroy(r.a); (void)hipEventDestroy(r.b); }
  e->prof.recs.clear();
  e->prof.on = true;
}

int bt_profile_end(bt_engine* e, double* ms_by_category, int32_t* launches_by_category, int n_categories) {
  if (!e) return bt_set_error(BT_ERR_ARG, "null engine");
  e->prof.on = false;
  if (!ms_by_category || !launches_by_category || n_categories < CAT_COUNT)
    return bt_set_error(BT_ERR_ARG, "need room for BT_PROFILE_CATEGORIES entries");
  for (int i = 0; i < n_categories; ++i) { ms_by_category[i] = 0.0; launches_by_category[i] = 0; }
  for (auto& r : e->prof.recs) {
    hipError_t e = hipEventSynchronize(r.b);
    float ms = 0.f;
    if (e == hipSuccess) e = hipEventElapsedTime(&ms, r.a, r.b);
    if (e != hipSuccess) return bt_set_error(BT_ERR_HIP, hipGetErrorString(e));
    ms_by_category[r.cat] += ms;
    launches_by_category[r.cat] += 1;
    (void)hipEventDestroy(r.a); (void)hipEventDestroy(r.b);
  }
  e->prof.recs.clear();
  return BT_OK;
}

int bt_ff_fused(void* stream, int prec, const bt_pair_weights* w, float* d_x, int64_t M) {
  if (!w || !d_x || M <= 0 || w->dim > 128 || !w->w_ff_frag[prec]) return bt_set_error(BT_ERR_ARG, "bad argument to bt_ff_fused");
  FusedFFP ff;
  ff.x = d_x; ff.M = M; ff.C = w->dim; ff.wfrag = w->w_ff_frag[prec]; ff.b1 = w->b_ff1; ff.b2 = w->b_ff2;
  ff.xb = nullptr;
  LAUNCH(launch_ff_fused(ff, prec, (hipStream_t)stream), "fused feed-forward");
  return BT_OK;
}

int bt_gemm(void* stream, int prec, const bt_gemm_args* a) {
  if (!a) return bt_set_error(BT_ERR_ARG, "null argument");
  GemmP g;
  memset(&g, 0, sizeof g);
  g.A = a->A; g.lda = a->lda; g.W = a->W; g.M = a->M; g.N = a->N; g.K = a->K; g.epi = a->epi; g.flags = a->flags;
  g.bias = a->bias; g.out = a->out; g.ldo = a->ldo; g.x = a->x; g.ldx = a->ldx;
  g.conv_C2 = a->conv_C2; g.conv_T = a->conv_T; g.conv_F = a->conv_F;
  g.gates = a->gates; g.inner = a->inner; g.heads = a->heads; g.rope = a->rope;
  g.pdiv = a->pdiv; g.pmod = a->pmod; g.map_T = a->map_T; g.map_F = a->map_F;
  LAUNCH(launch_gemm(g, prec, (hipStream_t)stream), "gemm");
  return BT_OK;
}

int bt_attention(void* stream, int prec, const bt_attn_args* a) {
  if (!a) return bt_set_error(BT_ERR_ARG, "null argument");
  AttnP p;
  memset(&p, 0, sizeof p);
  p.qkv = a->qkv; p.ld = a->ld; p.gates = a->gates; p.out = a->out; p.n_seq = a->n_seq; p.L = a->L;
  p.heads = a->heads; p.inner = a->inner; p.o_div = a->o_div; p.o_outer = a->o_outer; p.o_inner = a->o_inner;
  p.o_tok = a->o_tok;
  LAUNCH(launch_attn_flash(p, prec, (hipStream_t)stream), "attention (flash)");
  return BT_OK;
}

int bt_outff_fused(void* stream, int prec, const bt_pair_weights* w, const void* d_ao, float* d_x, int64_t M, void* d_xb) {
  if (prec != BT_PREC_F32 && prec != BT_PREC_HALF && prec != BT_PREC_F32X3) return bt_set_error(BT_ERR_ARG, "unknown precision");
  const void* wf = !w ? nullptr : prec == BT_PREC_F32X3 ? w->w_outff_frag_x3 : w->w_outff_frag[prec];
  if (!w || !d_ao || !d_x || M <= 0 || w->dim > 128 || !wf) return bt_set_error(BT_ERR_ARG, "bad argument to bt_outff_fused");
  FusedOutFFP f;
  f.x = d_x; f.M = M; f.C = w->dim; f.ao = d_ao; f.wfrag = wf; f.b1 = w->b_ff1; f.b2 = w->b_ff2;
  f.xb = prec == BT_PREC_F32 ? nullptr : d_xb; f.abl = 0; f.shadow_only = 0;
  LAUNCH(launch_outff_fused(f, prec, (hipStream_t)stream), "fused out-projection + feed-forward");
  return BT_OK;
}

int bt_attnff_fused(void* stream, int prec, const bt_pair_weights* w, const float* d_rope, float* d_x, int64_t M) {
  if (prec != BT_PREC_F32 && prec != BT_PREC_HALF && prec != BT_PREC_F32X3) return bt_set_error(BT_ERR_ARG, "unknown precision");
  const void* wf = !w ? nullptr : prec == BT_PREC_F32X3 ? w->w_attnff_frag_x3 : w->w_attnff_frag[prec];
  if (!w || !d_x || !d_rope || M <= 0 || w->dim > 128 || !wf) return bt_set_error(BT_ERR_ARG, "bad argument to bt_attnff_fused");
  FusedAttnFFP f;
  f.x = d_x; f.M = M; f.C = w->dim; f.b_gates = w->b_gates; f.rope = d_rope; f.wfrag = wf;
  f.b1 = w->b_ff1; f.b2 = w->b_ff2;
  LAUNCH(launch_attnff_fused(f, prec, (hipStream_t)stream), "fused frequency attention + feed-forward");
  return BT_OK;
}

int bt_layer_tail(void* stream, const bt_pair_weights* w, int hidden, const void* d_ao, float* d_x, int64_t M, void* d_xb,
                  float* d_ssq_out) {
  if (!w || !w->w_tail_frag || !d_ao || !d_x || M <= 0 || !layer_tail_supported(w->dim, hidden))
    return bt_set_error(BT_ERR_ARG, "bad argument to bt_layer_tail");
  LayerTailP t;
  t.x = d_x; t.M = M; t.C = w->dim; t.hidden = hidden; t.ao = d_ao; t.wfrag = w->w_tail_frag; t.b1 = w->b_ff1;
  t.b2 = w->b_ff2; t.xb = d_xb; t.ssq_out = d_ssq_out;
  LAUNCH(launch_layer_tail(t, (hipStream_t)stream), "layer tail");
  return BT_OK;
}

int bt_gemm3(void* stream, const bt_gemm3_args* a) {
  if (!a || !a->A || !a->W) return bt_set_error(BT_ERR_ARG, "null argument");
  Gemm3P g;
  memset(&g, 0, sizeof g);
  g.A = a->A; g.lda = a->lda; g.M = a->M; g.K = a->K; g.W = a->W; g.N = a->N; g.epi = a->epi; g.bias = a->bias;
  g.ssq_in = a->ssq_in; g.ssq_parts = a->ssq_parts; g.out = a->out; g.ldo = a->ldo; g.x = a->x; g.ldx = a->ldx;
  g.xb = a->xb; g.ssq_out = a->ssq_out; g.n_seq = a->n_seq; g.L = a->L; g.nblk = (a->L + 31) / 32; g.nbp = a->nbp;
  g.heads = a->heads; g.inner = a->heads * 32; g.rope = a->rope; g.qf = a->qf; g.kf = a->kf; g.vf = a->vf;
  g.gates = a->gates; g.b_gates = a->b_gates;
  g.x3 = a->x3; g.status = a->status;
  g.no_resid = a->no_resid; g.gelu = a->gelu; g.conv_C2 = a->conv_C2; g.conv_T = a->conv_T; g.conv_F = a->conv_F;
  if (!gemm3_supported(g)) return bt_set_error(BT_ERR_ARG, "shape not supported by bt_gemm3");
  LAUNCH(launch_gemm3(g, (hipStream_t)stream), "gemm3");
  return BT_OK;
}

int bt_gemm_mx8(void* stream, const void* d_A, const void* d_SA, const void* d_W, const void* d_SW, float* d_out, int M, int N, int K,
                int64_t ldo) {
  GemmMx8P g;
  g.A = d_A; g.SA = d_SA; g.W = d_W; g.SW = d_SW; g.out = d_out; g.ldo = (long)ldo; g.M = M; g.N = N; g.K = K;
  if (!d_A || !d_SA || !d_W || !d_SW || !d_out || !gemm_mx8_supported(g)) return bt_set_error(BT_ERR_ARG, "bad argument to bt_gemm_mx8");
  LAUNCH(launch_gemm_mx8(g, (hipStream_t)stream), "MX e4m3 gemm");
  return BT_OK;
}

int bt_attn_frag_blocks(int L) { return L > 0 ? attn_frag_blocks(L) : 0; }

int bt_attention_frag(void* stream, const bt_attn_frag_args* a) {
  if (!a || !a->q || !a->k || !a->v || !a->gates || !a->out) return bt_set_error(BT_ERR_ARG, "null argument");
  AttnFragP p;
  memset(&p, 0, sizeof p);
  p.q = a->q; p.k = a->k; p.v = a->v; p.gates = a->gates; p.out = a->out; p.n_seq = a->n_seq; p.L = a->L;
  p.heads = a->heads; p.inner = a->inner; p.nbp = a->nbp; p.o_div = a->o_div; p.o_outer = a->o_outer;
  p.o_inner = a->o_inner; p.o_tok = a->o_tok;
  p.x3 = a->x3; p.out_f32 = a->out_f32; p.status = a->status; p.fix_mask = a->scratch;
  if (p.x3 > 0 && !p.fix_mask) return bt_set_error(BT_ERR_ARG, "bt_attention_frag: x3 needs the scratch words (overflow map)");
  LAUNCH(launch_attn_frag(p, (hipStream_t)stream), "attention (fragment-major)");
  return BT_OK;
}

int bt_qkv_front(void* stream, int prec, const bt_pair_weights* w, const float* d_rope, const float* d_x, int B, int T, int F,
                 void* d_q, void* d_k, void* d_v, float* d_gates, int nbp) {
  if (prec != BT_PREC_HALF && prec != BT_PREC_F32X3) return bt_set_error(BT_ERR_ARG, "bt_qkv_front: BT_PREC_HALF or BT_PREC_F32X3");
  const bool x3 = prec == BT_PREC_F32X3;
  const void* wf = !w ? nullptr : x3 ? w->w_qkv_frag_x3 : w->w_qkv_frag;
  if (!w || !wf || !d_rope || !d_x || !d_q || !d_k || !d_v || !d_gates || w->dim > 128)
    return bt_set_error(BT_ERR_ARG, "bad argument to bt_qkv_front");
  QkvFrontP p;
  memset(&p, 0, sizeof p);
  p.x = d_x; p.B = B; p.T = T; p.F = F; p.C = w->dim; p.wfrag = wf; p.b_gates = w->b_gates; p.rope = d_rope;
  p.q = d_q; p.k = d_k; p.v = d_v; p.gates = d_gates; p.nbp = nbp; p.x3 = x3;
  LAUNCH(launch_qkv_front(p, (hipStream_t)stream), "frontend qkv projection");
  return BT_OK;
}

}
```

beat_this_amd/csrc/fused2.hip:

```cpp
#include <cstdlib>
#include <type_traits>

#include "chain.h"
#include "kernels.h"

namespace {


typedef __amdgpu_buffer_rsrc_t rsrc_t;
typedef __attribute__((address_space(3))) void* lptr_t;
DEVI unsigned pk2_hf(float a, float b) {
  const hfx2 t = {(hf)a, (hf)b};
  return __builtin_bit_cast(unsigned, t);
}

#ifdef BT_DEV
__device__ long long* g_f2_dbg = nullptr;
#define F2_DBG g_f2_dbg
#define F2_ABL(p) ((p).abl)
#else
#define F2_DBG ((long long*)nullptr)
#define F2_ABL(p) 0
#endif

template <typename T, int C>
struct WRing {
  static constexpr int KT = C / 32;
  static constexpr int TILE_B = 32 * 32 * (int)sizeof(T);
  static constexpr int STEP_B = 2 * KT * TILE_B;
#ifndef BT_F2_NST_HL128
#define BT_F2_NST_HL128 2
#endif
#ifndef BT_F2_NST_HL64
#define BT_F2_NST_HL64 2
#endif
  static constexpr bool HL = sizeof(T) == 4 && !std::is_same<T, float>::value;
  static constexpr int NST = C == 128 ? (HL ? BT_F2_NST_HL128 : 3) : (HL && C == 64 ? BT_F2_NST_HL64 : 4);
  static constexpr int CH = STEP_B / 4096;
  rsrc_t rs;
  char* lds;
  int tid, wave, total;
  long long t_wait = 0, t_bar = 0;
  bool timing = false;
  DEVI void issue(int s) {
    if (s >= total) return;
    char* dst = lds + (s % NST) * STEP_B + wave * 1024;
#pragma unroll
    for (int i = 0; i < CH; ++i)
      __builtin_amdgcn_raw_ptr_buffer_load_lds(rs, (lptr_t)(dst + i * 4096), 16, tid * 16, s * STEP_B + i * 4096, 0, 0);
  }
  DEVI void prologue() {
#pragma unroll
    for (int s = 0; s < NST - 1; ++s) issue(s);
  }
  DEVI const char* acquire(int s) {
    const int ahead = min(NST - 2, total - 1 - s);
    long long q0 = 0, q1 = 0;
    if (timing) q0 = clock64();
    if (ahead >= 2) asm volatile("s_waitcnt vmcnt(%0) lgkmcnt(0)" ::"n"(2 * CH) : "memory");
    else if (ahead == 1) asm volatile("s_waitcnt vmcnt(%0) lgkmcnt(0)" ::"n"(CH) : "memory");
    else asm volatile("s_waitcnt vmcnt(0) lgkmcnt(0)" ::: "memory");
    if (timing) q1 = clock64();
    __builtin_amdgcn_s_barrier();
    if (timing) { const long long q2 = clock64(); t_wait += q1 - q0; t_bar += q2 - q1; }
    issue(s + NST - 1);
    return lds + (s % NST) * STEP_B;
  }
};

template <typename T, int C, bool STORE_X = true>
DEVI void ff_tail(WRing<T, C>& ws, int step0, float (&xn)[C / 32][16], const float* b1s, const float* b2,
                  float* xrow, hf* xbrow, bool ok, int lane, int g) {
  constexpr int KT = C / 32, HB = 4 * C / 32;
  constexpr int TILE_B = WRing<T, C>::TILE_B;
  float ss = 0.f;
#pragma unroll
  for (int kt = 0; kt < KT; ++kt)
#pragma unroll
    for (int r = 0; r < 16; ++r) ss = fmaf(xn[kt][r], xn[kt][r], ss);
  ss += __shfl_xor(ss, 32);
  constexpr float PW = OpScale<T>::PW;
  const float scale = sqrtf((float)C) / fmaxf(sqrtf(ss), 1e-12f) * PW;
  Frag<T> xf[KT];
#pragma unroll
  for (int kt = 0; kt < KT; ++kt) xf[kt] = pack_frag<T>(xn[kt]);
  f32x16 acc2[KT];
#pragma unroll
  for (int mt = 0; mt < KT; ++mt)
#pragma unroll
    for (int r = 0; r < 16; ++r) acc2[mt][r] = xn[mt][r] * (1.f / PW);
#pragma unroll 1
  for (int hb = 0; hb < HB; ++hb) {
    const char* wb = ws.acquire(step0 + hb);
    f32x16 acc1;
    zero16(acc1);
#pragma unroll
    for (int kt = 0; kt < KT; ++kt) mma32(acc1, lds_frag<T>(wb + kt * TILE_B, lane), xf[kt]);
    float h[16];
#pragma unroll
    for (int a = 0; a < 4; ++a) {
      const f32x4 b = *reinterpret_cast<const f32x4*>(b1s + hb * 32 + 8 * a + 4 * g);
#pragma unroll
      for (int j = 0; j < 4; ++j) h[4 * a + j] = gelu_t<T>(fmaf(acc1[4 * a + j], scale, b[j]));
    }
    const Frag<T> hf = pack_frag<T>(h);
#pragma unroll
    for (int mt = 0; mt < KT; ++mt) mma32(acc2[mt], lds_frag<T>(wb + (KT + mt) * TILE_B, lane), hf);
  }
#pragma unroll
  for (int mt = 0; mt < KT; ++mt) {
    f32x4 v[4];
#pragma unroll
    for (int a = 0; a < 4; ++a) {
      const int f0 = mt * 32 + 8 * a + 4 * g;
      const f32x4 b = *reinterpret_cast<const f32x4*>(b2 + f0);
#pragma unroll
      for (int j = 0; j < 4; ++j) v[a][j] = fmaf(acc2[mt][4 * a + j], PW, b[j]);
      if constexpr (STORE_X) {
        if (ok) *reinterpret_cast<f32x4*>(xrow + f0) = v[a];
      }
    }
    if (xbrow) {
      typedef __attribute__((ext_vector_type(4))) unsigned int u32x4;
      if constexpr (std::is_same<T, hl>::value) {
#pragma unroll
        for (int k = 0; k < 2; ++k) {
          unsigned xh[2], xl[2], yh[2], yl[2];
#pragma unroll
          for (int i = 0; i < 2; ++i) {
            split_hl4(v[2 * k][2 * i], v[2 * k][2 * i + 1], v[2 * k + 1][2 * i], v[2 * k + 1][2 * i + 1], xh[i], xl[i], yh[i], yl[i]);
          }
          auto h0 = __builtin_amdgcn_permlane32_swap(xh[0], yh[0], false, false);
          auto h1 = __builtin_amdgcn_permlane32_swap(xh[1], yh[1], false, false);
          auto l0 = __builtin_amdgcn_permlane32_swap(xl[0], yl[0], false, false);
          auto l1 = __builtin_amdgcn_permlane32_swap(xl[1], yl[1], false, false);
          if (ok) {
            *reinterpret_cast<u32x4*>(xbrow + mt * 64 + 16 * k + 8 * g) = u32x4{h0[0], h1[0], h0[1], h1[1]};
            *reinterpret_cast<u32x4*>(xbrow + mt * 64 + 32 + 16 * k + 8 * g) = u32x4{l0[0], l1[0], l0[1], l1[1]};
          }
        }
      } else {
#pragma unroll
      for (int k = 0; k < 2; ++k) {
        const unsigned x0 = pk2_hf(v[2 * k][0], v[2 * k][1]), x1 = pk2_hf(v[2 * k][2], v[2 * k][3]);
        const unsigned y0 = pk2_hf(v[2 * k + 1][0], v[2 * k + 1][1]), y1 = pk2_hf(v[2 * k + 1][2], v[2 * k + 1][3]);
        auto r0 = __builtin_amdgcn_permlane32_swap(x0, y0, false, false);
        auto r1 = __builtin_amdgcn_permlane32_swap(x1, y1, false, false);
        if (ok) *reinterpret_cast<u32x4*>(xbrow + mt * 32 + 16 * k + 8 * g) = u32x4{r0[0], r1[0], r0[1], r1[1]};
      }
      }
    }
  }
}

template <typename T, int C, bool STORE_X = true>
__global__ __launch_bounds__(256) void outff_fused_kernel(const FusedOutFFP p) {
  constexpr int KT = C / 32, HB = 4 * C / 32;
  constexpr int TILE_B = WRing<T, C>::TILE_B, STEP_B = WRing<T, C>::STEP_B, NST = WRing<T, C>::NST;
  __shared__ __attribute__((aligned(16))) char wl[NST * STEP_B + 4 * C * 4];
  float* b1s = reinterpret_cast<float*>(wl + NST * STEP_B);
  const int tid = threadIdx.x, lane = tid & 63, wave = __builtin_amdgcn_readfirstlane(tid >> 6);
  const int g = lane >> 5, lr = lane & 31;
  const long tok = ((long)blockIdx.x * 4 + wave) * 32 + lr;
  const bool ok_st = tok < p.M && !(F2_ABL(p) & 2);
  const bool ok = tok < p.M && !(F2_ABL(p) & 1);
  float* xrow = p.x + (tok < p.M ? tok : 0) * C;
  for (int i = tid; i < 4 * C; i += 256) b1s[i] = p.b1[i];

  const T* arow = reinterpret_cast<const T*>(p.ao) + (ok ? tok : 0) * C;
  Frag<T> af[KT];
#pragma unroll
  for (int kt = 0; kt < KT; ++kt) af[kt] = ldg_frag<T>(arow + kt * 32 + 16 * g);
  float xn[KT][16];
#pragma unroll
  for (int mt = 0; mt < KT; ++mt)
#pragma unroll
    for (int a = 0; a < 4; ++a) {
      const f32x4 v = ok ? *reinterpret_cast<const f32x4*>(xrow + mt * 32 + 8 * a + 4 * g) : f32x4{0.f, 0.f, 0.f, 0.f};
#pragma unroll
      for (int j = 0; j < 4; ++j) xn[mt][4 * a + j] = v[j];
    }
  WRing<T, C> ws;
  ws.rs = __builtin_amdgcn_make_buffer_rsrc(const_cast<void*>(p.wfrag), 0, (unsigned)((KT + HB) * STEP_B), 0x00020000);
  ws.lds = wl; ws.tid = tid; ws.wave = wave; ws.total = KT + HB;
  __syncthreads();
  asm volatile("s_waitcnt vmcnt(0)" ::: "memory");
  ws.prologue();
#pragma unroll
  for (int mt = 0; mt < KT; ++mt) {
    const char* wb = ws.acquire(mt);
    f32x16 acc;
    zero16(acc);
#pragma unroll
    for (int kt = 0; kt < KT; ++kt) mma32(acc, lds_frag<T>(wb + kt * TILE_B, lane), af[kt]);
#pragma unroll
    for (int r = 0; r < 16; ++r) xn[mt][r] = fmaf(acc[r], OpScale<T>::PW, xn[mt][r]);
  }
  hf* xbrow = p.xb ? reinterpret_cast<hf*>(p.xb) + tok * C * (std::is_same<T, hl>::value ? 2 : 1) : nullptr;
  ff_tail<T, C, STORE_X>(ws, KT, xn, b1s, p.b2, xrow, xbrow, ok_st, lane, g);
}

template <typename T, int C>
__global__ __launch_bounds__(256) void attnff_fused_kernel(const FusedAttnFFP p) {
  constexpr int KT = C / 32;
  constexpr int H = C / 32;
  constexpr int F = 1024 / C;
  constexpr int HB = 4 * C / 32;
  constexpr int TILE_B = WRing<T, C>::TILE_B, STEP_B = WRing<T, C>::STEP_B, NST = WRing<T, C>::NST;
  __shared__ __attribute__((aligned(16))) char wl[NST * STEP_B + 4 * C * 4];
  float* b1s = reinterpret_cast<float*>(wl + NST * STEP_B);
  const int tid = threadIdx.x, lane = tid & 63, wave = __builtin_amdgcn_readfirstlane(tid >> 6);
  const int g = lane >> 5, lr = lane & 31;
  const long tok = ((long)blockIdx.x * 4 + wave) * 32 + lr;
  const bool ok = tok < p.M;
  float* xrow = p.x + (ok ? tok : 0) * C;
  long long* dbg = F2_DBG;
  const long long t_in = dbg ? clock64() : 0;
  for (int i = tid; i < 4 * C; i += 256) b1s[i] = p.b1[i];

  float ss = 0.f;
  Frag<T> xf[KT];
#pragma unroll
  for (int kt = 0; kt < KT; ++kt) xf[kt] = ldx_frag<T>(xrow + kt * 32 + 16 * g, ok, ss);
  ss += __shfl_xor(ss, 32);
  constexpr float PW = OpScale<T>::PW, PA = OpScale<T>::PA;
  const float scale = sqrtf((float)C) / fmaxf(sqrtf(ss), 1e-12f) * PW;
  float sk[16];
#pragma unroll
  for (int r = 0; r < 16; ++r) sk[r] = __shfl(scale, crow(r, g));
  const int pos = (int)(tok & (F - 1));
  f32x2 cs[8];
#pragma unroll
  for (int a = 0; a < 4; ++a)
#pragma unroll
    for (int b = 0; b < 2; ++b)
      cs[2 * a + b] = *reinterpret_cast<const f32x2*>(p.rope + ((long)pos * 16 + 4 * a + 2 * g + b) * 2);
  float bg[H];
#pragma unroll
  for (int hd = 0; hd < H; ++hd) bg[hd] = p.b_gates[hd];
  WRing<T, C> ws;
  ws.rs = __builtin_amdgcn_make_buffer_rsrc(const_cast<void*>(p.wfrag), 0, (unsigned)((1 + 2 * H + HB) * STEP_B), 0x00020000);
  ws.lds = wl; ws.tid = tid; ws.wave = wave; ws.total = 1 + 2 * H + HB;
  __syncthreads();
  asm volatile("s_waitcnt vmcnt(0)" ::: "memory");
  ws.timing = dbg != nullptr;
  const long long t_ring = dbg ? clock64() : 0;
  ws.prologue();

  float gate[H];
  {
    const char* wb = ws.acquire(0);
    f32x16 ag;
    zero16(ag);
#pragma unroll
    for (int kt = 0; kt < KT; ++kt) mma32(ag, lds_frag<T>(wb + kt * TILE_B, lane), xf[kt]);
#pragma unroll
    for (int hd = 0; hd < H; ++hd) {
      float v = __shfl(ag[hd], lr);
      gate[hd] = sigmoidf(fmaf(v, scale, bg[hd]));
    }
  }

  f32x16 acco[KT];
#pragma unroll
  for (int mt = 0; mt < KT; ++mt) zero16(acco[mt]);
#pragma unroll 1
  for (int hd = 0; hd < H; ++hd) {
    float pr[16], l = 0.f;
    {
      const char* wb = ws.acquire(1 + 2 * hd);
      f32x16 aq, ak;
      zero16(aq); zero16(ak);
#pragma unroll
      for (int kt = 0; kt < KT; ++kt) {
        mma32(aq, lds_frag<T>(wb + kt * TILE_B, lane), xf[kt]);
        mma32(ak, lds_frag<T>(wb + (KT + kt) * TILE_B, lane), xf[kt]);
      }
      float q[16], k[16];
#pragma unroll
      for (int a = 0; a < 4; ++a)
#pragma unroll
        for (int b = 0; b < 2; ++b) {
          const f32x2 t = cs[2 * a + b];
          const int r = 4 * a + 2 * b;
          const float q0 = aq[r] * scale, q1 = aq[r + 1] * scale, k0 = ak[r] * scale, k1 = ak[r + 1] * scale;
          q[r] = q0 * t.x - q1 * t.y; q[r + 1] = q1 * t.x + q0 * t.y;
          k[r] = k0 * t.x - k1 * t.y; k[r + 1] = k1 * t.x + k0 * t.y;
        }
      f32x16 sc;
      zero16(sc);
      mma32(sc, pack_frag<T>(k), pack_frag<T>(q));
      float mx = -1e30f;
#pragma unroll
      for (int r = 0; r < 16; ++r) {
        sc[r] *= PA;
        if (F < 32 && ((crow(r, g) ^ lr) & ~(F - 1))) sc[r] = -1e30f;
        mx = fmaxf(mx, sc[r]);
      }
      mx = fmaxf(mx, __shfl_xor(mx, 32));
#pragma unroll
      for (int r = 0; r < 16; ++r) {
        pr[r] = __builtin_amdgcn_exp2f(sc[r] - mx);
        l += pr[r];
      }
      l += __shfl_xor(l, 32);
    }
    {
      const char* wb = ws.acquire(2 + 2 * hd);
      f32x16 av;
      zero16(av);
#pragma unroll
      for (int kt = 0; kt < KT; ++kt) mma32(av, xf[kt], lds_frag<T>(wb + kt * TILE_B, lane));
      float v[16];
#pragma unroll
      for (int r = 0; r < 16; ++r) v[r] = av[r] * sk[r];
      f32x16 ao;
      zero16(ao);
      mma32(ao, pack_frag<T>(v), pack_frag<T>(pr));
      float gsel = gate[0];
#pragma unroll
      for (int k = 1; k < H; ++k) gsel = hd == k ? gate[k] : gsel;
      const float fin = gsel / l * PA;
      float o[16];
#pragma unroll
      for (int r = 0; r < 16; ++r) o[r] = ao[r] * fin;
      const Frag<T> of = pack_frag<T>(o);
#pragma unroll
      for (int mt = 0; mt < KT; ++mt) mma32(acco[mt], lds_frag<T>(wb + (KT + mt) * TILE_B, lane), of);
    }
  }
  f32x4 xv[KT][4];
#pragma unroll
  for (int mt = 0; mt < KT; ++mt)
#pragma unroll
    for (int a = 0; a < 4; ++a)
      xv[mt][a] = ok ? *reinterpret_cast<const f32x4*>(xrow + mt * 32 + 8 * a + 4 * g) : f32x4{0.f, 0.f, 0.f, 0.f};
  asm volatile("s_waitcnt vmcnt(0)" ::: "memory");
  __builtin_amdgcn_sched_barrier(0);
  float xn[KT][16];
#pragma unroll
  for (int mt = 0; mt < KT; ++mt)
#pragma unroll
    for (int a = 0; a < 4; ++a)
#pragma unroll
      for (int j = 0; j < 4; ++j) xn[mt][4 * a + j] = fmaf(acco[mt][4 * a + j], PW, xv[mt][a][j]);
  const long long t_ff = dbg ? clock64() : 0;
  ff_tail<T, C>(ws, 1 + 2 * H, xn, b1s, p.b2, xrow, nullptr, ok, lane, g);
  if (dbg && lane == 0) {
    long long* d = dbg + ((long)blockIdx.x * 4 + wave) * 6;
    d[0] = t_ring - t_in; d[1] = t_ff - t_ring; d[2] = clock64() - t_ff; d[3] = ws.t_wait; d[4] = ws.t_bar; d[5] = 0;
  }
}

template <typename T>
int launch_outff_t(const FusedOutFFP& p, hipStream_t s) {
  dim3 grid((unsigned)((p.M + 127) / 128)), block(256);
  if constexpr (std::is_same<T, hl>::value) {
    if (p.shadow_only) {
      if (!p.xb) return -2;
      switch (p.C) {
        case 64: hipLaunchKernelGGL((outff_fused_kernel<T, 64, false>), grid, block, 0, s, p); break;
        case 128: hipLaunchKernelGGL((outff_fused_kernel<T, 128, false>), grid, block, 0, s, p); break;
        default: return -2;
      }
      return (int)hipGetLastError();
    }
  } else if (p.shadow_only) {
    return -2;
  }
  switch (p.C) {
    case 32: hipLaunchKernelGGL((outff_fused_kernel<T, 32>), grid, block, 0, s, p); break;
    case 64: hipLaunchKernelGGL((outff_fused_kernel<T, 64>), grid, block, 0, s, p); break;
    case 128: hipLaunchKernelGGL((outff_fused_kernel<T, 128>), grid, block, 0, s, p); break;
    default: return -2;
  }
  return (int)hipGetLastError();
}
template <typename T>
int launch_attnff_t(const FusedAttnFFP& p, hipStream_t s) {
  dim3 grid((unsigned)((p.M + 127) / 128)), block(256);
  switch (p.C) {
    case 32: hipLaunchKernelGGL((attnff_fused_kernel<T, 32>), grid, block, 0, s, p); break;
    case 64: hipLaunchKernelGGL((attnff_fused_kernel<T, 64>), grid, block, 0, s, p); break;
    case 128: hipLaunchKernelGGL((attnff_fused_kernel<T, 128>), grid, block, 0, s, p); break;
    default: return -2;
  }
  return (int)hipGetLastError();
}

}

#ifdef BT_DEV
extern "C" int bt_debug_fused2_buffer(void* buf) {
  return (int)hipMemcpyToSymbol(HIP_SYMBOL(g_f2_dbg), &buf, sizeof buf);
}
#endif

int launch_outff_fused(const FusedOutFFP& p0, int prec, hipStream_t s) {
  if (p0.M <= 0) return -2;
  FusedOutFFP p = p0;
  p.abl = 0;
#ifdef BT_DEV
  static const int abl = getenv("BT_F2_ABL") ? atoi(getenv("BT_F2_ABL")) : 0;
  p.abl = abl;
#endif
  if (prec == BT_PREC_F32X3) return BT_HALF_IS_BF16 ? -2 : launch_outff_t<hl>(p, s);
  return prec == BT_PREC_F32 ? launch_outff_t<float>(p, s) : launch_outff_t<hf>(p, s);
}
int launch_attnff_fused(const FusedAttnFFP& p, int prec, hipStream_t s) {
  if (p.M <= 0) return -2;
  if (prec == BT_PREC_F32X3) return BT_HALF_IS_BF16 ? -2 : launch_attnff_t<hl>(p, s);
  return prec == BT_PREC_F32 ? launch_attnff_t<float>(p, s) : launch_attnff_t<hf>(p, s);
}
```

beat_this_amd/csrc/kernels.h:

```cpp
#pragma once
#include <hip/hip_runtime.h>
#include <stdint.h>

#ifndef BT_PREC_F32
#define BT_PREC_F32 0
#define BT_PREC_HALF 1
#endif
#ifndef BT_PREC_F32X3
#define BT_PREC_F32X3 3
#endif

enum {
  GEMM_EPI_STORE = 0,
  GEMM_EPI_RESID = 1,
  GEMM_EPI_QKV = 2
};
enum {
  GEMM_F_RMS = 1,
  GEMM_F_BIAS = 2,
  GEMM_F_GELU = 4,
  GEMM_F_OUT_F32 = 8,
  GEMM_F_A_F32 = 16,
  GEMM_F_CONV = 32,
  GEMM_F_ROWMAP = 64
};

struct GemmP {
  const void* A;
  long lda;
  const void* W;
  int M, N, K;
  int epi, flags;
  const float* bias;
  void* out;
  long ldo;
  float* x;
  long ldx;
  void* xb;
  float* ssq_out;
  int conv_C2, conv_T, conv_F;
  float* gates;
  int inner;
  int heads;
  const float* rope;
  int pdiv, pmod;
  int map_T, map_F;
};
int launch_gemm(const GemmP& p, int prec, hipStream_t s);

enum { G3_FF1 = 0, G3_RESID = 1, G3_QKV = 2 };
struct Gemm3P {
  const void* A; long lda; int M, K;
  const void* W; int N;
  int epi;
  const float* bias;
  const float* ssq_in; int ssq_parts;
  void* out; long ldo;
  float* x; long ldx; void* xb;
  float* ssq_out;
  int n_seq, L, nblk, nbp, heads, inner;
  const float* rope; void* qf; void* kf; void* vf; float* gates; const float* b_gates;
  int no_resid;
  int gelu;
  int conv_C2, conv_T, conv_F;
  int x3;
  int* status;
};
enum { G3_X3_F8 = 0x100, G3_X3_OUT_F8 = 0x200 };
bool gemm3_supported(const Gemm3P& p);
int launch_gemm3(const Gemm3P& p, hipStream_t s);

struct GemmMx8P {
  const void* A; const void* SA;
  const void* W; const void* SW;
  float* out; long ldo;
  int M, N, K;
};
bool gemm_mx8_supported(const GemmMx8P& p);
int launch_gemm_mx8(const GemmMx8P& p, hipStream_t s);

struct AttnP {
  const void* qkv;
  long ld;
  const float* gates;
  void* out;
  int n_seq, L, heads, inner;
  int o_div;
  long o_outer, o_inner, o_tok;
};
int launch_attn_flash(const AttnP& p, int prec, hipStream_t s);

struct AttnFragP {
  const void* q; const void* k; const void* v;
  const float* gates;
  void* out;
  int n_seq, L, heads, inner, nbp;
  int o_div;
  long o_outer, o_inner, o_tok;
  int x3, out_f32;
  int* status;
  int* fix_mask;
};
int attn_frag_blocks(int L);
int launch_attn_frag(const AttnFragP& p, hipStream_t s);

struct QkvFrontP {
  const float* x;
  int B, T, F, C;
  const void* wfrag;
  const float* b_gates;
  const float* rope;
  void* q; void* k; void* v;
  float* gates;
  int nbp;
  int x3;
  int* status;
};
int launch_qkv_front(const QkvFrontP& p, hipStream_t s);

struct FusedFFP {
  float* x; long M; int C;
  const void* wfrag;
  const float* b1; const float* b2;
  void* xb;
};
int launch_ff_fused(const FusedFFP& p, int prec, hipStream_t s);

struct FusedOutFFP {
  float* x; long M; int C;
  const void* ao;
  const void* wfrag;
  const float* b1; const float* b2;
  void* xb;
  int abl;
  int shadow_only;
};
int launch_outff_fused(const FusedOutFFP& p, int prec, hipStream_t s);
struct FusedAttnFFP {
  float* x; long M; int C;
  const float* b_gates; const float* rope;
  const void* wfrag;
  const float* b1; const float* b2;
};
int launch_attnff_fused(const FusedAttnFFP& p, int prec, hipStream_t s);

struct LayerTailP {
  float* x; long M; int C; int hidden;
  const void* ao;
  const void* wfrag;
  const float* b1; const float* b2;
  void* xb;
  float* ssq_out;
};
bool layer_tail_supported(int C, int hidden);
int launch_layer_tail(const LayerTailP& p, hipStream_t s);

struct StemP {
  const float* spect;
  float* x;
  const float* bn1_scale; const float* bn1_shift;
  const float* w;
  const float* bias;
  int B, T;
};
int launch_stem(const StemP& p, hipStream_t s);

struct HeadP {
  const float* x;
  const float* w;
  float b0, b1;
  float* beat; float* downbeat;
  int M, D, sum_head;
  int prenorm;
  int* status;
};
int launch_head(const HeadP& p, hipStream_t s);
int launch_clear_words(int* w, int n, hipStream_t s);
int launch_norm_out(const float* x, const float* gamma, float* y, long M, int D, hipStream_t s, int* status = nullptr);
int launch_finite_rows(const float* x, long M, int D, int* status, hipStream_t s);
int launch_shadow_ssq(const float* x, void* xb, float* ssq, long M, int D, hipStream_t s, int hl32 = 0);

struct bt_span_t { const float* data; long n; long out_off; long n_out; };

int launch_split(const float* spect, long n_frames, const int* starts, const int* table, int B, int T, float* chunks,
                 hipStream_t s, int border = 0);
int launch_aggregate(const float* cb, const float* cd, const int* starts, const int* table, const int* pieces, int n_pieces,
                     int B, int T, int border, long n_frames, float* beat, float* downbeat, hipStream_t s);
int launch_resample(const bt_span_t& one, const bt_span_t* tracks, int n_tracks, long max_n_out, int up, int down,
                    const float* h, int half, float* y, hipStream_t s);
int launch_peaks(const float* logits, long n, const int* spans, int n_arrays, int* idx, int* count, hipStream_t s);

struct LogmelP {
  bt_span_t one;
  const bt_span_t* tracks;
  int n_tracks; long max_frames;
  const float* window;
  const float* twiddle;
  const int* mel_start;
  const int* mel_len;
  const float* mel_w;
  float* spect;
};
int launch_logmel(const LogmelP& p, hipStream_t s);
```

beat_this_amd/csrc/qkv_front.hip:

```cpp
#include "chain.h"
#include "kernels.h"

namespace {

typedef const __attribute__((address_space(1))) void* gptr_t;
typedef __attribute__((address_space(3))) void* lptr_t;

DEVI void split2q(float a, float b, unsigned& whi, unsigned& wlo, float& amax) {
  split_hl(a, b, whi, wlo);
  amax = fmaxf(amax, fmaxf(fabsf(a), fabsf(b)));
}

template <typename T, int C>
__global__ __launch_bounds__(256, (sizeof(T) == 2 ? (C == 32 ? 4 : C == 64 ? 3 : 2) : (C == 32 ? 3 : 2)))
void qkv_front_kernel(const QkvFrontP p) {
  constexpr bool X3 = sizeof(T) == 4;
  constexpr int KT = C / 32;
  constexpr int H = C / 32;
  constexpr int TILE_B = 1024 * (int)sizeof(T);
  constexpr int BLK_E = X3 ? 2048 : 1024;
  constexpr int STEP_B = 3 * KT * TILE_B;
  constexpr int NCH = STEP_B / 16;
  constexpr int NBUF = (X3 && C == 128) ? 1 : 2;
  __shared__ __attribute__((aligned(16))) char wl[NBUF * STEP_B];
  const int tid = threadIdx.x, lane = tid & 63, wave = __builtin_amdgcn_readfirstlane(tid >> 6);
  const int g = lane >> 5, lr = lane & 31;
  const int nblk = (p.T + 31) >> 5;
  const long wb_id = (long)blockIdx.x * 4 + wave;
  const long n_wb = (long)p.B * p.F * nblk;
  const bool wave_ok = wb_id < n_wb;
  const long wbc = wave_ok ? wb_id : n_wb - 1;
  const int sq = (int)(wbc / nblk), blk = (int)(wbc - (long)sq * nblk);
  const int b = sq / p.F, f = sq - b * p.F;
  const int t = blk * 32 + lr;
  const bool ok = wave_ok && t < p.T;
  const float* xrow = p.x + (((long)b * p.T + (ok ? t : 0)) * p.F + f) * C;
  const char* Wf = reinterpret_cast<const char*>(p.wfrag);

  auto stage = [&](int step, int buf) {
    const int nch = step < H ? NCH : KT * TILE_B / 16;
#pragma unroll
    for (int i = 0; i < (NCH + 255) / 256; ++i) {
      const int c0 = i * 256 + wave * 64;
      if (c0 < nch)
        __builtin_amdgcn_global_load_lds((gptr_t)(Wf + (long)step * STEP_B + (c0 + lane) * 16),
                                         (lptr_t)(wl + buf * STEP_B + c0 * 16), 16, 0, 0);
    }
  };
  if (NBUF == 2) stage(0, 0);

  float ss = 0.f, amax = 0.f;
  Frag<T> xf[KT];
#pragma unroll
  for (int kt = 0; kt < KT; ++kt) xf[kt] = ldx_frag<T>(xrow + kt * 32 + 16 * g, ok, ss);
  ss += __shfl_xor(ss, 32);
  const float scale = sqrtf((float)C) / fmaxf(sqrtf(ss), 1e-12f) * OpScale<T>::PW;
  float sk[16];
#pragma unroll
  for (int r = 0; r < 16; ++r) sk[r] = __shfl(scale, crow(r, g));
  f32x2 cs[8];
#pragma unroll
  for (int a = 0; a < 4; ++a)
#pragma unroll
    for (int bb = 0; bb < 2; ++bb)
      cs[2 * a + bb] = *reinterpret_cast<const f32x2*>(p.rope + ((long)(ok ? t : 0) * 16 + 4 * a + 2 * g + bb) * 2);

  hf* qf = reinterpret_cast<hf*>(p.q);
  hf* kf = reinterpret_cast<hf*>(p.k);
  hf* vf = reinterpret_cast<hf*>(p.v);
  __syncthreads();
#pragma unroll 1
  for (int step = 0; step <= H; ++step) {
    const char* wb = wl + (NBUF == 2 ? (step & 1) * STEP_B : 0);
    if (NBUF == 2) {
      if (step < H) stage(step + 1, (step + 1) & 1);
    } else {
      stage(step, 0);
      __syncthreads();
    }
    if (step < H) {
      const int hd = step;
      f32x16 aq, ak, av;
      zero16(aq); zero16(ak); zero16(av);
#pragma unroll
      for (int kt = 0; kt < KT; ++kt) {
        mma32(aq, lds_frag<T>(wb + kt * TILE_B, lane), xf[kt]);
        mma32(ak, lds_frag<T>(wb + (KT + kt) * TILE_B, lane), xf[kt]);
        mma32(av, xf[kt], lds_frag<T>(wb + (2 * KT + kt) * TILE_B, lane));
      }
      if (wave_ok) {
        const long base = (((long)sq * H + hd) * p.nbp + blk) * BLK_E;
#pragma unroll
        for (int a = 0; a < 4; ++a) {
          float q[4], k[4];
#pragma unroll
          for (int bb = 0; bb < 2; ++bb) {
            const f32x2 cth = cs[2 * a + bb];
            const int r = 4 * a + 2 * bb;
            const float q0 = aq[r] * scale, q1 = aq[r + 1] * scale, k0 = ak[r] * scale, k1 = ak[r + 1] * scale;
            q[2 * bb] = q0 * cth.x - q1 * cth.y; q[2 * bb + 1] = q1 * cth.x + q0 * cth.y;
            k[2 * bb] = k0 * cth.x - k1 * cth.y; k[2 * bb + 1] = k1 * cth.x + k0 * cth.y;
          }
          const long off = base + (a * 32 + lr) * 8 + 4 * g;
          if constexpr (X3) {
            typedef __attribute__((ext_vector_type(2))) unsigned int u32x2;
            unsigned qh[2], ql[2], kh[2], kl[2];
            split2q(q[0], q[1], qh[0], ql[0], amax); split2q(q[2], q[3], qh[1], ql[1], amax);
            split2q(k[0], k[1], kh[0], kl[0], amax); split2q(k[2], k[3], kh[1], kl[1], amax);
            *reinterpret_cast<u32x2*>(qf + off) = u32x2{qh[0], qh[1]}; *reinterpret_cast<u32x2*>(qf + off + 1024) = u32x2{ql[0], ql[1]};
            *reinterpret_cast<u32x2*>(kf + off) = u32x2{kh[0], kh[1]}; *reinterpret_cast<u32x2*>(kf + off + 1024) = u32x2{kl[0], kl[1]};
          } else {
            *reinterpret_cast<hfx4*>(qf + off) = hfx4{(hf)q[0], (hf)q[1], (hf)q[2], (hf)q[3]};
            *reinterpret_cast<hfx4*>(kf + off) = hfx4{(hf)k[0], (hf)k[1], (hf)k[2], (hf)k[3]};
          }
        }
#pragma unroll
        for (int s = 0; s < 2; ++s) {
          if constexpr (X3) {
            typedef __attribute__((ext_vector_type(4))) unsigned int u32x4;
            unsigned oh[4], ol[4];
#pragma unroll
            for (int j = 0; j < 4; ++j)
              split2q(av[8 * s + 2 * j] * sk[8 * s + 2 * j], av[8 * s + 2 * j + 1] * sk[8 * s + 2 * j + 1], oh[j], ol[j], amax);
            *reinterpret_cast<u32x4*>(vf + base + (s * 64 + lane) * 8) = u32x4{oh[0], oh[1], oh[2], oh[3]};
            *reinterpret_cast<u32x4*>(vf + base + 1024 + (s * 64 + lane) * 8) = u32x4{ol[0], ol[1], ol[2], ol[3]};
          } else {
            hfx8 o;
#pragma unroll
            for (int j = 0; j < 8; ++j) o[j] = (hf)(av[8 * s + j] * sk[8 * s + j]);
            *reinterpret_cast<hfx8*>(vf + base + (s * 64 + lane) * 8) = o;
          }
        }
      }
    } else {
      f32x16 ag;
      zero16(ag);
#pragma unroll
      for (int kt = 0; kt < KT; ++kt) mma32(ag, lds_frag<T>(wb + kt * TILE_B, lane), xf[kt]);
      if (wave_ok && g == 0) {
#pragma unroll
        for (int hd = 0; hd < H; ++hd)
          p.gates[((long)sq * H + hd) * p.nbp * 32 + t] = sigmoidf(fmaf(ag[hd], scale, p.b_gates[hd]));
      }
    }
    __syncthreads();
  }
  if (X3 && p.status && __any(!(amax <= 65504.f)) && lane == 0) atomicOr(p.status, 1);
}

}

int launch_qkv_front(const QkvFrontP& p, hipStream_t s) {
  if (p.B <= 0 || p.T <= 0 || p.F <= 0 || p.nbp < attn_frag_blocks(p.T)) return -2;
  const long n_wb = (long)p.B * p.F * ((p.T + 31) / 32);
  dim3 grid((unsigned)((n_wb + 3) / 4)), block(256);
  if (p.x3) {
    if (BT_HALF_IS_BF16) return -2;
    switch (p.C) {
      case 32: hipLaunchKernelGGL((qkv_front_kernel<hl, 32>), grid, block, 0, s, p); break;
      case 64: hipLaunchKernelGGL((qkv_front_kernel<hl, 64>), grid, block, 0, s, p); break;
      case 128: hipLaunchKernelGGL((qkv_front_kernel<hl, 128>), grid, block, 0, s, p); break;
      default: return -2;
    }
    return (int)hipGetLastError();
  }
  switch (p.C) {
    case 32: hipLaunchKernelGGL((qkv_front_kernel<hf, 32>), grid, block, 0, s, p); break;
    case 64: hipLaunchKernelGGL((qkv_front_kernel<hf, 64>), grid, block, 0, s, p); break;
    case 128: hipLaunchKernelGGL((qkv_front_kernel<hf, 128>), grid, block, 0, s, p); break;
    default: return -2;
  }
  return (int)hipGetLastError();
}
```

beat_this_amd/pack.py:

```python
from __future__ import annotations

import collections
import ctypes as C
import math
import threading

import torch

from . import _lib, tables

LOG2E = 1.4426950408889634
BN_EPS = 1e-5


def perm32(w: torch.Tensor) -> torch.Tensor:
    idx = torch.tensor([(r & 3) + 8 * (r >> 2) + 4 * g for g in range(2) for r in range(16)])
    n, k = w.shape
    return w.reshape(n, k // 32, 32)[:, :, idx].reshape(n, k).contiguous()


def fragment_tiles(w: torch.Tensor) -> torch.Tensor:
    r, k = w.shape
    t = w.reshape(r // 32, 32, k // 32, 2, 16)
    return t.permute(0, 2, 3, 1, 4).reshape(r // 32, k // 32, 64, 16)
# ... 153 lines not shown
        return t.data_ptr()

    def _hl8(self, w: torch.Tensor) -> int:
        if _lib.lib().bt_half_is_bf16() or not hasattr(torch, "float8_e4m3fn"):
            return 0
        w = _pad_rows(w.to(torch.float32), 256)
        n, k = w.shape
        hi = w.to(torch.float16)
        lo = (w - hi.to(torch.float32)) * 2048.0
        t = torch.empty((n, k // 32, 128), dtype=torch.uint8)
        t[:, :, :64] = hi.contiguous().view(n, k // 32, 32).view(torch.uint8)
        t[:, :, 64:96] = w.clamp(-448, 448).to(torch.float8_e4m3fn).view(torch.uint8).view(n, k // 32, 32)
        t[:, :, 96:] = lo.clamp(-448, 448).to(torch.float8_e4m3fn).view(torch.uint8).view(n, k // 32, 32)
        t = t.contiguous().to(self.device)
        self._keep.append(t)
        return t.data_ptr()

    def ensure_hl8(self):
        todo, self._hl8_todo = self._hl8_todo, []
        if not todo:
            return None
        old, n_keep = [(pw, field, getattr(pw, field)) for pw, field, _, _ in todo], len(self._keep)
        for pw, field, src, rows in todo:
            w = self._by_ptr[getattr(pw, src)[0]][:rows].cpu()
            setattr(pw, field, self._hl8(w))

        def undo():
            for pw, field, value in old:
                setattr(pw, field, value)
            del self._keep[n_keep:]
            self._hl8_todo = todo
        return undo

    def _pair(self, pw, sd, pa: str, pf: str, dim: int, x3: bool = False) -> None:
        heads = dim // 32
        pw.dim, pw.heads = dim, heads
        ga = sd[pa + "norm.gamma"]
        wqkv = sd[pa + "to_qkv.weight"].clone()
        wqkv[:dim] *= LOG2E / math.sqrt(32.0)
        wg = sd[pa + "to_gates.weight"]
        w = torch.cat([wqkv, wg], 0) * ga[None, :]
        pw.w_qkvg[0], pw.w_qkvg[1] = self._mat(w)
        if dim <= 128:
            qflat = qkv_fragment_major(_pad_rows(w.to(torch.float32)), dim)
            qf = qflat.to(_lib.half_torch_dtype()).to(self.device)
            self._keep.append(qf)
            pw.w_qkv_frag = qf.data_ptr()
            if not _lib.lib().bt_half_is_bf16():
                pw.w_qkv_frag_x3 = self._x3_stream(qflat)
        pw.b_gates = self._f32(sd[pa + "to_gates.bias"])
        pw.w_out[0], pw.w_out[1] = self._mat(sd[pa + "to_out.0.weight"])
        if x3 and dim % 128 == 0:
            pw.w_qkvg_x3 = self._hl32(w)
            pw.w_out_x3 = self._hl32(sd[pa + "to_out.0.weight"])
            pw.w_ff1_x3 = self._hl32(sd[pf + "net.1.weight"] * sd[pf + "net.0.gamma"][None, :])
            pw.w_ff2_x3 = self._hl32(sd[pf + "net.4.weight"])
            if hasattr(self, "_hl8_todo"):
                self._hl8_todo += [(pw, "w_qkvg_f8", "w_qkvg", w.shape[0]), (pw, "w_out_f8", "w_out", dim),
                                   (pw, "w_ff1_f8", "w_ff1", sd[pf + "net.1.weight"].shape[0]), (pw, "w_ff2_f8", "w_ff2", dim)]
        if dim <= 128 and sd[pf + "net.1.weight"].shape[0] == 4 * dim:
            w1 = (sd[pf + "net.1.weight"] * sd[pf + "net.0.gamma"][None, :]).to(torch.float32)
            w2p = perm32(sd[pf + "net.4.weight"].to(torch.float32))
            f32 = ff_fragment_major(w1, w2p, 4).to(self.device)
            b16 = ff_fragment_major(w1, w2p, 8).to(_lib.half_torch_dtype()).to(self.device)
            self._keep += [f32, b16]
            pw.w_ff_frag[0], pw.w_ff_frag[1] = f32.data_ptr(), b16.data_ptr()
            wo = sd[pa + "to_out.0.weight"].to(torch.float32)
            w1p = perm32(w1)
            for i, (epp, dt) in enumerate(((4, torch.float32), (8, _lib.half_torch_dtype()))):
                ot = fragment_tiles(wo)
                ot = ot.reshape(ot.shape[0], ot.shape[1], 64, 16 // epp, epp).permute(0, 1, 3, 2, 4)
                ot = torch.cat([ot, torch.zeros_like(ot)], 1).reshape(-1)
                flat = torch.cat([ot, ff_fragment_major(w1p, w2p, epp)])
                t = flat.to(dt).to(self.device)
                self._keep.append(t)
                pw.w_outff_frag[i] = t.data_ptr()
                if i == 1 and dt == torch.float16:
                    pw.w_outff_frag_x3 = self._x3_stream(flat)
                kt = dim // 32

                def pieces(tiles):
                    sh = tiles.shape[:-2]
                    return tiles.reshape(*sh, 64, 16 // epp, epp).transpose(-3, -2).reshape(-1)
                qt = fragment_tiles(_pad_rows(w.to(torch.float32))[:3 * dim + 32])
                opt = fragment_tiles(perm32(wo))
                steps = [pieces(qt[3 * heads]), torch.zeros(kt * 32 * 32)]
                for hd in range(heads):
                    steps += [pieces(qt[hd]), pieces(qt[heads + hd]), pieces(qt[2 * heads + hd]), pieces(opt[:, hd])]
                steps.append(ff_fragment_major(w1p, w2p, epp))
                flat = torch.cat(steps)
                t = flat.to(dt).to(self.device)
                self._keep.append(t)
                pw.w_attnff_frag[i] = t.data_ptr()
                if i == 1 and dt == torch.float16:
                    pw.w_attnff_frag_x3 = self._x3_stream(flat)
        gf = sd[pf + "net.0.gamma"]
        pw.w_ff1[0], pw.w_ff1[1] = self._mat(sd[pf + "net.1.weight"] * gf[None, :])
        pw.b_ff1 = self._f32(sd[pf + "net.1.bias"])
        pw.w_ff2[0], pw.w_ff2[1] = self._mat(sd[pf + "net.4.weight"])
        pw.b_ff2 = self._f32(sd[pf + "net.4.bias"])
        hidden = sd[pf + "net.1.weight"].shape[0]
        if dim in (256, 512) and hidden % 64 == 0 and 128 <= hidden <= 4096:
            w1 = (sd[pf + "net.1.weight"] * gf[None, :]).to(torch.float32)
            t = tail_fragment_major(sd[pa + "to_out.0.weight"].to(torch.float32), perm32(w1),
                                    perm32(sd[pf + "net.4.weight"].to(torch.float32)))
            t = t.to(_lib.half_torch_dtype()).to(self.device)
            self._keep.append(t)
            pw.w_tail_frag = t.data_ptr()


class PackedPair:

    def __init__(self, sd: dict, attn_prefix: str, ff_prefix: str, dim: int, device):
        self.device = torch.device(device)
        self._keep: list[torch.Tensor] = []
        self.weights = _lib.PairWeights()
        sd = {k: v.detach().to("cpu", torch.float32) for k, v in sd.items()}
        PackedModel._pair(self, self.weights, sd, attn_prefix, ff_prefix, dim, x3=True)

    _f32 = PackedModel._f32
    _mat = PackedModel._mat
    _hl32 = PackedModel._hl32
    _hl8 = PackedModel._hl8
    _x3_stream = PackedModel._x3_stream


class Engine:

    def __init__(self, packed: PackedModel):
        self.packed = packed
        self.device = packed.device
        h = C.c_void_p()
        _lib.check(_lib.lib().bt_engine_create(C.byref(packed.desc), C.byref(h)))
        self._h = h
        self._ws = collections.OrderedDict()
        self._graphs = collections.OrderedDict()
        self._graph_ws = {}
        self._a2b_ws = {}
        self._graphs_ok = True
        self.profiling = False
        self._lock = threading.Lock()
        self.last_fallbacks = 0

    def __del__(self):
        try:
            if getattr(self, "_h", None):
                _lib.lib().bt_engine_destroy(self._h)
                self._h = None
        except Exception:
            pass

    MAX_WORKSPACES = 4
    SHRINK_AFTER = 8
    OPTIONS = {"x3_attn_p16": 1, "x3_gemm_fp8": 2, "ws_guard": 3}

    def set_options(self, opts: dict) -> None:
        for name in opts:
            if name not in self.OPTIONS:
                raise ValueError(f"unknown engine option {name!r} (known: {sorted(self.OPTIONS)})")
        if int(opts.get("x3_gemm_fp8", 0)) > 0:
            undo = self.packed.ensure_hl8()
            if undo is not None:
                self._rebuild_handle(undo)
        for name, value in opts.items():
            _lib.check(_lib.lib().bt_engine_set_option(self._h, self.OPTIONS[name], int(value)))
        self._drop_graphs()

    def _drop_graphs(self) -> None:
        self._graphs = collections.OrderedDict()
        self._graph_ws = {}

    def _rebuild_handle(self, undo) -> None:
        torch.cuda.synchronize(self.device)
        lib, h = _lib.lib(), C.c_void_p()
        try:
            _lib.check(lib.bt_engine_create(C.byref(self.packed.desc), C.byref(h)))
            for name, opt in self.OPTIONS.items():
                _lib.check(lib.bt_engine_set_option(h, opt, self.get_option(name)))
        except Exception:
            if h.value:
                lib.bt_engine_destroy(h)
            undo()
            raise
        old, self._h = self._h, h
        lib.bt_engine_destroy(old)
        self._drop_graphs()

    def get_option(self, name: str) -> int:
        v = C.c_int(0)
        _lib.check(_lib.lib().bt_engine_get_option(self._h, self.OPTIONS[name], C.byref(v)))
        return int(v.value)

    def ensure_positions(self, T: int) -> None:
        if T <= self.packed.desc.rope_len:
            return
        p = self.packed
        old = p.desc.rope, p.desc.rope_len, p._rope_t
        p.set_positions(-(-T // 512) * 512)

        def undo():
            p.desc.rope, p.desc.rope_len, p._rope_t = old
        self._rebuild_handle(undo)

    def _workspace(self, need: int) -> torch.Tensor:
        key = torch.cuda.current_stream(self.device)
        ws, small = self._ws.pop(key, (None, 0))
        if ws is not None and ws.numel() < need:
            ws = None
        elif ws is not None and ws.numel() > 4 * need:
            small += 1
            if small >= self.SHRINK_AFTER:
                ws = None
        else:
            small = 0
        if ws is None:
            ws, small = torch.empty(need, dtype=torch.uint8, device=self.device), 0
        self._ws[key] = (ws, small)
        while len(self._ws) > self.MAX_WORKSPACES:
            self._ws.popitem(last=False)
        return ws

    def forward(self, spect: torch.Tensor, prec: int):
        return self.forward_stages(spect, prec, 0, 2)

    def forward_stages(self, spect: torch.Tensor, prec: int, first: int, last: int, logits_out=None, checks=None):
        _lib.require_gpu(spect, "stage input")
        B, T, M = spect.shape
        D = self.packed.desc.transformer_dim
        if M != (128 if first == 0 else D):
            raise ValueError(f"expected {128 if first == 0 else D} input features, got {M}")
        x = spect.to(torch.float32).contiguous()
        self.ensure_positions(T)
        need = _lib.lib().bt_workspace_bytes(self._h, B, T, prec)
        if need == 0:
            raise ValueError("empty batch")
        ws = self._workspace(need)
        beat = down = out = None
        if last == 2 and logits_out is not None:
            beat, down = logits_out
            for t in (beat, down):
                if t.dtype != torch.float32 or tuple(t.shape) != (B, T) or not t.is_contiguous() or t.device != x.device:
                    raise ValueError("logits_out: two contiguous fp32 (batch, time) tensors on the input's device")
        elif last == 2:
            beat = torch.empty((B, T), dtype=torch.float32, device=self.device)
            down = torch.empty((B, T), dtype=torch.float32, device=self.device)
        else:
            out = torch.empty((B, T, D), dtype=torch.float32, device=self.device)
        with torch.cuda.device(self.device):
            _lib.check(_lib.lib().bt_forward_stages(self._h, _lib.stream_ptr(self.device), prec, first, last, x.data_ptr(), B, T,
                                                    ws.data_ptr(), ws.numel(), _lib.ptr(out), _lib.ptr(beat), _lib.ptr(down)))
            if prec == _lib.PREC_F32X3:
                flag = ws[:4].view(torch.int32)
                if checks is not None:
                    host = torch.empty(1, dtype=torch.int32, pin_memory=True)
                    host.copy_(flag, non_blocking=True)
                    ev = torch.cuda.Event()
                    ev.record(torch.cuda.current_stream(self.device))
                    checks.append((host, ev))
                elif int(flag.item()) != 0:
                    self._count_fallback()
                    return self.forward_stages(spect, _lib.PREC_F32, first, last, logits_out=logits_out)
        return (beat, down) if last == 2 else out

    def forward_unit(self, x: torch.Tensor, prec: int, unit: int, index: int, out_shape) -> torch.Tensor:
        _lib.require_gpu(x, "sub-module input")
        B, T = int(x.shape[0]), int(x.shape[1])
        if B == 0 or T == 0:
            raise ValueError("empty batch")
        if prec == _lib.PREC_F32X3:
            prec = _lib.PREC_F32
        x = x.to(torch.float32).contiguous()
        self.ensure_positions(T)
        ws = self._workspace(_lib.lib().bt_workspace_bytes(self._h, B, T, prec))
        out = torch.empty(tuple(out_shape), dtype=torch.float32, device=self.device)
        with torch.cuda.device(self.device):
            _lib.check(_lib.lib().bt_forward_unit(self._h, _lib.stream_ptr(self.device), prec, unit, index, x.data_ptr(),
                                                  out.data_ptr(), B, T, ws.data_ptr(), ws.numel()))
        return out

    GRAPH_MAX_CHUNKS = 11
    GRAPH_T = 1500
    GRAPH_MAX_ENTRIES = 12

    def graph_forward(self, B: int, T: int, prec: int):
        if not self._graphs_ok or T != self.GRAPH_T or B > self.GRAPH_MAX_CHUNKS or self.profiling:
            return None
        stream = torch.cuda.current_stream(self.device)
        key = (stream, B, T, prec)
        e = self._graphs.pop(key, None)
        if e is None:
            try:
                e = _GraphEntry(self, B, T, prec, stream)
            except Exception as err:
                self._graphs_ok = False
                self._graph_error = repr(err)
                return None
        cache = self._graphs
        cache[key] = e
        while len(cache) > self.GRAPH_MAX_ENTRIES:
            cache.popitem(last=False)
        return e

    def _graph_workspace(self, stream, need: int) -> torch.Tensor:
        pool = self._graph_ws
        ws = pool.get(stream)
        if ws is None or ws.numel() < need:
            ws = pool[stream] = torch.empty(need, dtype=torch.uint8, device=self.device)
# ... 69 lines not shown
```

include/beat_this_amd.h:

```cpp
#ifndef BEAT_THIS_AMD_H
#define BEAT_THIS_AMD_H
#include <stddef.h>
#include <stdint.h>

#ifdef __cplusplus
extern "C" {
#endif

#define BT_OK 0
#define BT_ERR_ARG (-1)
#define BT_ERR_HIP (-2)
#define BT_ERR_WORKSPACE (-3)

#define BT_PREC_F32 0
#define BT_PREC_HALF 1

#define BT_PREC_F32X3 3

#define BT_MAX_LAYERS 32

typedef struct bt_engine bt_engine;

typedef struct {
  int32_t dim, heads;
  const void* w_qkvg[2];
  const float* b_gates;
  const void* w_out[2];
  const void* w_ff1[2];
  const float* b_ff1;
  const void* w_ff2[2];
  const float* b_ff2;
  const void* w_ff_frag[2];
  const void* w_qkv_frag;
  const void* w_outff_frag[2];
  const void* w_attnff_frag[2];
  const void* w_tail_frag;
  const void* w_outff_frag_x3;
  const void* w_attnff_frag_x3;
  const void* w_qkvg_x3;
  const void* w_out_x3;
  const void* w_ff1_x3;
  const void* w_ff2_x3;
  const void* w_qkv_frag_x3;
  const void* w_qkvg_f8;
  const void* w_out_f8;
  const void* w_ff1_f8;
  const void* w_ff2_f8;
} bt_pair_weights;

typedef struct {
  int32_t transformer_dim, n_layers, sum_head, partial_transformers;
  const float* bn1_scale;
  const float* bn1_shift;
  const float* stem_w;
  const float* stem_b;
  bt_pair_weights front[3][2];
  const void* conv_w[3][2];
  const float* conv_b[3];
  const void* lin_w[2];
  const float* lin_b;
  bt_pair_weights layers[BT_MAX_LAYERS];
  const float* head_w;
  float head_b[2];
  const float* rope;
  int32_t ff_mult;
  const float* norm_out_g;
  const float* head_w_raw;
  const void* conv_w_x3[3];
  const void* lin_w_x3;
  int32_t rope_len;
} bt_model_desc;

typedef struct {
  const float* window;
  const float* twiddle;
  const int32_t* mel_start;
  const int32_t* mel_len;
  const float* mel_w;
} bt_logmel_tables;

const char* bt_last_error(void);
#define BT_ABI_VERSION 600
int bt_version(void);
int bt_half_is_bf16(void);
void bt_struct_sizes(int32_t* out);

int bt_engine_create(const bt_model_desc* desc, bt_engine** out);
void bt_engine_destroy(bt_engine* e);
#define BT_OPT_X3_ATTN_P16 1
#define BT_OPT_X3_GEMM_FP8 2
#define BT_OPT_WS_GUARD 3
int bt_engine_set_option(bt_engine* e, int option, int value);
int bt_engine_get_option(const bt_engine* e, int option, int* value);
size_t bt_workspace_bytes(const bt_engine* e, int B, int T, int prec);
int bt_workspace_regions(const bt_engine* e, int B, int T, int prec, int64_t* begin_end, int max);

int bt_forward(bt_engine* e, void* stream, int prec, const float* d_spect, int B, int T, void* d_ws,
               size_t ws_bytes, float* d_beat, float* d_downbeat);

int bt_forward_stages(bt_engine* e, void* stream, int prec, int first, int last, const float* d_in, int B, int T, void* d_ws,
                      size_t ws_bytes, float* d_out, float* d_beat, float* d_downbeat);

enum { BT_UNIT_STEM = 0, BT_UNIT_PARTIAL = 1, BT_UNIT_CONV = 2, BT_UNIT_LINEAR = 3, BT_UNIT_ATTN = 4, BT_UNIT_FF = 5, BT_UNIT_NORM = 6,
       BT_UNIT_FRONT_ATTN = 7, BT_UNIT_FRONT_FF = 8 };
int bt_forward_unit(bt_engine* e, void* stream, int prec, int unit, int index, const float* d_in, float* d_out, int B, int T,
                    void* d_ws, size_t ws_bytes);

int bt_split_chunks(void* stream, const float* d_spect, int64_t n_frames, const int32_t* d_starts, int B, int T,
                    float* d_chunks);
int bt_aggregate(void* stream, const float* d_chunk_beat, const float* d_chunk_downbeat, const int32_t* d_starts,
                 int B, int T, int border, int64_t n_frames, float* d_beat, float* d_downbeat);

int bt_logmel(void* stream, const bt_logmel_tables* tables, const float* d_audio, int64_t n_samples,
              float* d_spect);

typedef struct { const float* d_in; int64_t n_in; int64_t out_off; int64_t n_out; } bt_span;
int bt_resample_batch(void* stream, const bt_span* d_tracks, int n_tracks, int64_t max_n_out, int up, int down,
                      const float* d_filter, int half_len, float* d_out);
int bt_logmel_batch(void* stream, const bt_logmel_tables* tables, const bt_span* d_tracks, int n_tracks,
                    int64_t max_frames, float* d_spect);
int bt_split_chunks_batch(void* stream, const float* d_spect, const int32_t* d_chunk_table, int B, int T, float* d_chunks);
int bt_aggregate_batch(void* stream, const float* d_chunk_beat, const float* d_chunk_downbeat, const int32_t* d_chunk_table,
                       const int32_t* d_pieces, int n_pieces, int64_t max_frames, int T, int border, float* d_beat,
                       float* d_downbeat);

int bt_resample(void* stream, const float* d_in, int64_t n_in, int up, int down, const float* d_filter, int half_len,
                float* d_out, int64_t n_out);

int bt_peaks(void* stream, const float* d_logits, int64_t n, int n_arrays, int32_t* d_idx, int32_t* d_count);
int bt_peaks_batch(void* stream, const float* d_logits, const int32_t* d_spans, int n_arrays, int32_t* d_idx,
                   int32_t* d_count);
int bt_peaks_host(const float* logits, int64_t n, int32_t* idx, int32_t* count);

int bt_dbn_tables(double fps, double min_bpm, double max_bpm, int num_tempi, double transition_lambda,
                  double observation_lambda, double threshold, const int32_t* beats_per_bar, int n_hmm, void* tables,
                  size_t* bytes);
size_t bt_dbn_workspace_bytes(const void* tables, int n_tracks, int64_t total_frames);
int bt_dbn_decode(void* stream, const void* tables, const void* d_tables, const void* d_logits, int f64,
                  const int32_t* d_spans, int n_tracks, int64_t total_frames, int32_t* d_out, void* d_ws, size_t ws_bytes);
int bt_dbn_viterbi(void* stream, const void* tables, const void* d_tables, int hmm, const double* d_dens, int64_t n,
                   int32_t* d_path, double* d_log_prob, void* d_ws, size_t ws_bytes);
int bt_dbn_viterbi_host(const void* tables, int hmm, const double* dens, int64_t n, int32_t* path, double* log_prob);
int bt_dbn_host(const void* tables, const double* beat, const double* downbeat, int64_t n, int32_t* rows, int32_t* n_rows);
int bt_dbn_host_act(const void* tables, const double* act, int64_t n, int32_t* rows, int32_t* n_rows);

#define BT_METRICS_COLS 12
#define BT_METRICS_NONFINITE 1
#define BT_METRICS_UNSORTED 2
#define BT_METRICS_LATE 4
#define BT_METRICS_NEAREST 64
#define BT_METRICS_OFFSETS 128
size_t bt_beat_metrics_workspace_bytes(int n_tracks, int64_t total_ref, int64_t total_est);
int bt_beat_metrics(void* stream, const double* d_ref, const int64_t* d_ref_off, const double* d_est, const int64_t* d_est_off,
                    int n_tracks, double min_beat_time, double f_window, double cemgil_sigma, double phase_thr,
                    double period_thr, void* d_ws, size_t ws_bytes, double* d_out);
int bt_beat_metrics_host(const double* ref, const int64_t* ref_off, const double* est, const int64_t* est_off, int n_tracks,
                         double min_beat_time, double f_window, double cemgil_sigma, double phase_thr, double period_thr,
                         double* out);

#define BT_LOSS_MASKED 0
#define BT_LOSS_SHIFT_TOLERANT 1
#define BT_LOSS_SPLITTED 2
#define BT_LOSS_F32 0
#define BT_LOSS_F16 1
#define BT_LOSS_BF16 2
#define BT_LOSS_U8 3
#define BT_LOSS_MAX_TOLERANCE 32
#define BT_LOSS_SEGMENT 256
size_t bt_bce_loss_workspace_bytes(int n_rows, int64_t max_len);
int bt_bce_loss(void* stream, int kind, int tolerance, float pos_weight, const float* d_pos_weight, const void* d_logits,
                int logit_dtype, const void* d_targets, int target_dtype, const void* d_mask, int mask_dtype,
                const int64_t* d_offsets, int n_rows, int64_t min_len, int64_t max_len, void* d_ws, size_t ws_bytes,
                double* d_row_sum, int64_t* d_row_count, void* d_loss, int loss_dtype, float* d_grad, float* d_terms);
int bt_bce_loss_backward(void* stream, const float* d_grad, int64_t n, const void* d_grad_output, int grad_output_dtype,
                         int64_t count, void* d_grad_in, int grad_in_dtype);
int bt_bce_loss_host(int kind, int tolerance, float pos_weight, const void* logits, int logit_dtype, const void* targets,
                     int target_dtype, const void* mask, int mask_dtype, const int64_t* offsets, int n_rows, double* row_sum,
                     int64_t* row_count, double* total, float* grad, float* terms);

#define BT_MASK_ZERO 0
#define BT_MASK_PERMUTE 1
#define BT_TRAIN_FRAME_BLOCK 64
typedef struct {
  int64_t row;
  int64_t ann_begin, ann_end;
  int32_t n;
  int32_t start_frame;
  int32_t op_begin, op_end;
  int32_t has_downbeats;
  int32_t reserved;
} bt_train_item;
typedef struct {
  int32_t start, length, kind;
  int32_t part_begin, part_end;
} bt_train_op;
typedef struct {
  int32_t new_off, old_off;
} bt_train_part;
void bt_train_batch_struct_sizes(int32_t* out);
int bt_train_batch(void* stream, const void* d_store, int store_dtype, int64_t store_rows, const bt_train_item* d_items, int B,
                   int L, const bt_train_op* d_ops, int n_ops, const bt_train_part* d_parts, int n_parts,
                   const double* d_ann_time, const int32_t* d_ann_value, int64_t n_ann, double fps, void* d_spect,
                   int spect_dtype, uint8_t* d_truth_beat, uint8_t* d_truth_downbeat, uint8_t* d_padding_mask,
                   uint8_t* d_downbeat_mask);
int bt_train_batch_host(const void* store, int store_dtype, int64_t store_rows, const bt_train_item* items, int B, int L,
                        const bt_train_op* ops, int n_ops, const bt_train_part* parts, int n_parts, const double* ann_time,
                        const int32_t* ann_value, int64_t n_ann, double fps, void* spect, int spect_dtype, uint8_t* truth_beat,
                        uint8_t* truth_downbeat, uint8_t* padding_mask, uint8_t* downbeat_mask);

int bt_deduplicate_peaks_host(const int32_t* idx, int n, double width, double* out, int32_t* n_out);
int bt_postprocess_host(const int32_t* beat_idx, int n_beat_idx, const int32_t* down_idx, int n_down_idx,
                        double fps, double* beats, int32_t* n_beats, double* downbeats, int32_t* n_downbeats);

typedef struct {
  int64_t n22, n_frames, result_words;
  int32_t B, T;
  size_t ws_bytes, off_wave22, off_spect, off_chunks, off_chunk_logits, off_logits, off_result, off_forward, forward_bytes;
} bt_a2b_plan;
int bt_audio2beats_plan(const bt_engine* e, int64_t n_in, int up, int down, int prec, bt_a2b_plan* plan);
int bt_audio2beats_enqueue(bt_engine* e, void* stream, int prec, const bt_logmel_tables* tables, const float* d_audio, int64_t n_in,
                           int up, int down, const float* d_filter, int half_len, void* d_ws, size_t ws_bytes, int32_t* h_result,
                           int use_graph);

#define BT_CAT_STEM 0
#define BT_CAT_QKV_GEMM 1
#define BT_CAT_ATTN_FLASH 2
#define BT_CAT_OUT_GEMM 3
#define BT_CAT_FF1_GEMM 4
#define BT_CAT_FF2_GEMM 5
#define BT_CAT_CONV_GEMM 6
#define BT_CAT_LINEAR_GEMM 7
#define BT_CAT_HEAD 8
#define BT_CAT_FF_FUSED 9
#define BT_CAT_ATTN_FREQ_FUSED 10
#define BT_CAT_LAYER_TAIL 11
#define BT_PROFILE_CATEGORIES 12
void bt_profile_begin(bt_engine* e);
int bt_profile_end(bt_engine* e, double* ms_by_category, int32_t* launches_by_category, int n_categories);

typedef struct {
  const void* A; int64_t lda; const void* W; int32_t M, N, K; int32_t epi, flags;
  const float* bias; void* out; int64_t ldo; float* x; int64_t ldx;
  int32_t conv_C2, conv_T, conv_F;
  float* gates; int32_t inner, heads; const float* rope; int32_t pdiv, pmod, map_T, map_F;
} bt_gemm_args;
int bt_gemm(void* stream, int prec, const bt_gemm_args* a);

typedef struct {
  const void* qkv; int64_t ld; const float* gates; void* out;
  int32_t n_seq, L, heads, inner, o_div; int64_t o_outer, o_inner, o_tok;
} bt_attn_args;
int bt_attention(void* stream, int prec, const bt_attn_args* a);

#define BT_X3_P16 8
typedef struct {
  const void* q; const void* k; const void* v; const float* gates; void* out;
  int32_t n_seq, L, heads, inner, nbp, o_div; int64_t o_outer, o_inner, o_tok;
  int32_t x3, out_f32; int32_t* status;
  int32_t* scratch;
} bt_attn_frag_args;
int bt_gemm_mx8(void* stream, const void* d_A, const void* d_SA, const void* d_W, const void* d_SW, float* d_out, int M, int N,
                int K, int64_t ldo);

typedef struct {
  const void* A; int64_t lda; int32_t M, K; const void* W; int32_t N, epi; const float* bias;
  const float* ssq_in; int32_t ssq_parts; void* out; int64_t ldo; float* x; int64_t ldx; void* xb; float* ssq_out;
  int32_t n_seq, L, nbp, heads; const float* rope; void* qf; void* kf; void* vf; float* gates; const float* b_gates;
  int32_t no_resid;
  int32_t gelu, conv_C2, conv_T, conv_F;
  int32_t x3; int32_t* status;
} bt_gemm3_args;
int bt_gemm3(void* stream, const bt_gemm3_args* a);
int bt_attn_frag_blocks(int L);
int bt_attention_frag(void* stream, const bt_attn_frag_args* a);
int bt_qkv_front(void* stream, int prec, const bt_pair_weights* w, const float* d_rope, const float* d_x, int B, int T, int F,
                 void* d_q, void* d_k, void* d_v, float* d_gates, int nbp);
int bt_ff_fused(void* stream, int prec, const bt_pair_weights* w, float* d_x, int64_t M);
int bt_outff_fused(void* stream, int prec, const bt_pair_weights* w, const void* d_ao, float* d_x, int64_t M, void* d_xb);
int bt_attnff_fused(void* stream, int prec, const bt_pair_weights* w, const float* d_rope, float* d_x, int64_t M);
int bt_layer_tail(void* stream, const bt_pair_weights* w, int hidden, const void* d_ao, float* d_x, int64_t M, void* d_xb,
                  float* d_ssq_out);

#define BT_TRAIN_UNIT_HEAD 16
#define BT_TRAIN_DW_ROWS 1024
#define BT_TRAIN_CS_ROWS 64
#define BT_TRAIN_ATTN_BLOCK 64
typedef struct {
  int32_t B, T, dim, hidden, rope_len, residual, sum_head, reserved;
  const float* rope;
  const float* gamma; const float* w1; const float* b1; const float* w2; const float* b2; const float* w3;
  const float* x; float* y; float* y2; float* save_o; float* save_lse;
  const float* gy; const float* gy2;
  float* gx; float* g_gamma; float* g_w1; float* g_b1; float* g_w2; float* g_b2; float* g_w3;
  void* ws; size_t ws_bytes;
} bt_train_args;
void bt_train_struct_sizes(int32_t* out);
size_t bt_train_workspace_bytes(int unit, int backward, int B, int T, int dim, int hidden);
int bt_train_forward(void* stream, int unit, const bt_train_args* a);
int bt_train_backward(void* stream, int unit, const bt_train_args* a);

#define BT_DROP_ATTN_P 0
#define BT_DROP_ATTN_OUT 1
#define BT_DROP_FF_HIDDEN 2
#define BT_DROP_FF_OUT 3
typedef struct {
  float p; uint32_t reserved; uint64_t seed; uint64_t stream;
} bt_train_dropout;
void bt_train_dropout_struct_sizes(int32_t* out);
size_t bt_train_workspace_bytes_dropout(int unit, int backward, int B, int T, int dim, int hidden);
int bt_train_forward_dropout(void* stream, int unit, const bt_train_args* a, const bt_train_dropout* dropout);
int bt_train_backward_dropout(void* stream, int unit, const bt_train_args* a, const bt_train_dropout* dropout);
void bt_philox4x32_10_host(const uint32_t* ctr, const uint32_t* key, uint32_t* out);
int bt_dropout_mask_host(const bt_train_dropout* dropout, int site, int B, int T, int dim, int hidden, uint8_t* out);

size_t bt_train_workspace_bytes_mixed(int unit, int backward, int B, int T, int dim, int hidden, int with_dropout);
int bt_train_forward_mixed(void* stream, int unit, const bt_train_args* a, const bt_train_dropout* dropout_or_null);
int bt_train_backward_mixed(void* stream, int unit, const bt_train_args* a, const bt_train_dropout* dropout_or_null);
int bt_train_matmul_mixed(void* stream, int form, const float* A, const float* B, int M, int N, int K, float* C);

#define BT_OPTIM_CHUNK 4096
#define BT_OPTIM_NORM_SLICE 4096
#define BT_OPTIM_MAX_GROUPS 8
typedef struct {
  float* param; int64_t offset, numel; int32_t group, reserved;
} bt_optim_tensor;
typedef struct {
  int32_t tensor, chunk;
} bt_optim_chunk;
typedef struct {
  float decay, one_minus_beta1, beta2, one_minus_beta2, step_size, bias2_sqrt, eps, reserved;
} bt_optim_group;
typedef struct {
  int32_t n_groups, zero_grads; float grad_scale; int32_t reserved;
  bt_optim_group g[BT_OPTIM_MAX_GROUPS];
} bt_optim_hyper;
void bt_optim_struct_sizes(int32_t* out);
int bt_optim_plan(int n_tensors, const void* const* params, const int64_t* numel, const int32_t* groups, int n_groups,
                  bt_optim_tensor* tensors, int64_t* total, bt_optim_chunk* chunks, int64_t chunk_capacity, int64_t* n_chunks);
size_t bt_grad_norm_workspace_bytes(int64_t total);
int bt_grad_norm(void* stream, const float* d_grad, int64_t total, float grad_scale, float max_norm, void* d_ws, size_t ws_bytes,
                 float* d_record);
int bt_adamw_step(void* stream, const bt_optim_tensor* d_tensors, int n_tensors, const bt_optim_chunk* d_chunks, int64_t n_chunks,
                  float* d_grad, float* d_m, float* d_v, int64_t total, const bt_optim_hyper* hyper, const float* d_coef);
int bt_grad_norm_host(const float* grad, int64_t total, float grad_scale, float max_norm, float* record);
int bt_adamw_step_host(const bt_optim_tensor* tensors, int n_tensors, const bt_optim_chunk* chunks, int64_t n_chunks, float* grad,
                       float* m, float* v, int64_t total, const bt_optim_hyper* hyper, const float* coef);

#ifdef __cplusplus
}
#endif
#endif
```

Before: 62700.

## Add persistent LDS-resident-weight kernels for frontend qkv, attnff and outff

Adds persistent-grid variants of the frontend QKV projection, frequency attention+FF, and out-projection+FF kernels for the x3 path. Each workgroup loads the full weight image into LDS once via buffer-to-LDS loads, then loops over work blocks while prefetching the next block's activation rows into registers. This removes the repeated per-block weight streaming of the tiled kernels. The persistent form is enabled by default through a new engine option. It raises LDS use and lowers occupancy, and adds new API entry points that take a form and workgroup count.

```diff
diff --git a/beat_this_amd/_lib.py b/beat_this_amd/_lib.py
--- a/beat_this_amd/_lib.py
+++ b/beat_this_amd/_lib.py
@@ -17,7 +17,8 @@
 BT_OK, BT_ERR_ARG, BT_ERR_HIP, BT_ERR_WORKSPACE = 0, -1, -2, -3
 ABI_VERSION = 600
 PREC_F32, PREC_HALF, PREC_F32X3 = 0, 1, 3
-OPT_X3_ATTN_P16, OPT_X3_GEMM_FP8, OPT_WS_GUARD = 1, 2, 3
+OPT_X3_ATTN_P16, OPT_X3_GEMM_FP8, OPT_WS_GUARD, OPT_FRONT_PERSISTENT = 1, 2, 3, 4
+FRONT_FORM_DEFAULT, FRONT_FORM_TILED, FRONT_FORM_PERSISTENT = 0, 1, 2
 MAX_LAYERS = 32
 PROFILE_CATEGORIES = ["stem", "qkv_gemm", "attn_flash", "out_gemm", "ff1_gemm", "ff2_gemm", "conv_gemm",
                       "linear_gemm", "head", "ff_fused", "attn_freq_fused", "layer_tail"]
@@ -205,6 +206,11 @@
                                C.c_void_p, C.c_void_p, C.c_void_p, C.c_void_p, C.c_int]),
     "bt_outff_fused": (C.c_int, [C.c_void_p, C.c_int, C.POINTER(PairWeights), C.c_void_p, C.c_void_p, C.c_int64, C.c_void_p]),
     "bt_attnff_fused": (C.c_int, [C.c_void_p, C.c_int, C.POINTER(PairWeights), C.c_void_p, C.c_void_p, C.c_int64]),
+    "bt_qkv_front_ex": (C.c_int, [C.c_void_p, C.c_int, C.POINTER(PairWeights), C.c_void_p, C.c_void_p, C.c_int, C.c_int, C.c_int,
+                                  C.c_void_p, C.c_void_p, C.c_void_p, C.c_void_p, C.c_int, C.c_int, C.c_int]),
+    "bt_outff_fused_ex": (C.c_int, [C.c_void_p, C.c_int, C.POINTER(PairWeights), C.c_void_p, C.c_void_p, C.c_int64, C.c_void_p,
+                                    C.c_int, C.c_int]),
+    "bt_attnff_fused_ex": (C.c_int, [C.c_void_p, C.c_int, C.POINTER(PairWeights), C.c_void_p, C.c_void_p, C.c_int64, C.c_int, C.c_int]),
     "bt_layer_tail": (C.c_int, [C.c_void_p, C.POINTER(PairWeights), C.c_int, C.c_void_p, C.c_void_p, C.c_int64, C.c_void_p,
                                 C.c_void_p]),
     "bt_ff_fused": (C.c_int, [C.c_void_p, C.c_int, C.POINTER(PairWeights), C.c_void_p, C.c_int64]),
diff --git a/beat_this_amd/csrc/chain.h b/beat_this_amd/csrc/chain.h
--- a/beat_this_amd/csrc/chain.h
+++ b/beat_this_amd/csrc/chain.h
@@ -79,6 +79,41 @@
   return f;
 }
 
+struct RawFrag { f32x4 v[4]; };
+DEVI RawFrag ldg_raw(const float* p) {
+  RawFrag r;
+#pragma unroll
+  for (int i = 0; i < 4; ++i) r.v[i] = reinterpret_cast<const f32x4*>(p)[i];
+  return r;
+}
+DEVI RawFrag ldx_raw(const float* p, bool ok) {
+  RawFrag r;
+#pragma unroll
+  for (int i = 0; i < 4; ++i) r.v[i] = ok ? reinterpret_cast<const f32x4*>(p)[i] : f32x4{0.f, 0.f, 0.f, 0.f};
+  return r;
+}
+DEVI Frag<hl> split_raw(const RawFrag& r) {
+  Frag<hl> f;
+#pragma unroll
+  for (int h = 0; h < 2; ++h) {
+    const f32x4 a = r.v[2 * h], b = r.v[2 * h + 1];
+    const float v[8] = {a[0], a[1], a[2], a[3], b[0], b[1], b[2], b[3]};
+    split_hl8(f, h, v);
+  }
+  return f;
+}
+DEVI Frag<hl> split_raw(const RawFrag& r, float& ss) {
+  Frag<hl> f;
+#pragma unroll
+  for (int h = 0; h < 2; ++h) {
+    const f32x4 a = r.v[2 * h], b = r.v[2 * h + 1];
+    const float v[8] = {a[0], a[1], a[2], a[3], b[0], b[1], b[2], b[3]};
+#pragma unroll
+    for (int j = 0; j < 8; ++j) ss = fmaf(v[j], v[j], ss);
+    split_hl8(f, h, v);
+  }
+  return f;
+}
 template <typename T> DEVI Frag<T> pack_frag(const float (&h)[16]);
 template <> DEVI Frag<float> pack_frag<float>(const float (&h)[16]) {
   Frag<float> f;
@@ -129,3 +164,13 @@
   for (int i = 0; i < 4; ++i) f.v[i] = *reinterpret_cast<const f32x4*>(tile + i * 1024 + lane * 16);
   return f;
 }
+
+template <int NW, int PIECE>
+DEVI void lds_image_load(char* dst, __amdgpu_buffer_rsrc_t rs, int bytes, int lane, int wave) {
+  typedef __attribute__((address_space(3))) void* lds_t;
+  static_assert(PIECE == 16 || PIECE == 4, "piece size");
+  constexpr int OP_B = 64 * PIECE;
+  for (int off = wave * OP_B; off < bytes; off += NW * OP_B)
+    if constexpr (PIECE == 16) __builtin_amdgcn_raw_ptr_buffer_load_lds(rs, (lds_t)(dst + off), 16, lane * 16, off, 0, 0);
+    else __builtin_amdgcn_raw_ptr_buffer_load_lds(rs, (lds_t)(dst + off), 4, lane * 4, off, 0, 0);
+}
diff --git a/beat_this_amd/csrc/engine.hip b/beat_this_amd/csrc/engine.hip
--- a/beat_this_amd/csrc/engine.hip
+++ b/beat_this_amd/csrc/engine.hip
@@ -47,6 +47,7 @@
   std::vector<int> warm;
   int x3_attn_p16 = 1;
   int x3_gemm_fp8 = 0;
+  int front_persistent = 1;
   int ws_guard = 0;
 };
 enum { CAT_STEM = 0, CAT_QKV, CAT_ATTN_FLASH, CAT_OUT, CAT_FF1, CAT_FF2, CAT_CONV, CAT_LINEAR,
@@ -179,6 +180,7 @@
   bool outff;
   bool split;
   bool time_frag;
+  int persistent;
 };
 
 struct FragLayer {
@@ -223,6 +225,12 @@
     p.outff = p.ff_fused && w.w_outff_frag[r.fp] && w.w_attnff_frag[r.fp];
     p.split = r.x3 && w.w_outff_frag_x3 && w.w_attnff_frag_x3;
     p.time_frag = r.x3 ? p.outff && p.split && w.w_qkv_frag_x3 : p.ff_fused && r.fp == BT_PREC_HALF && w.w_qkv_frag;
+    p.persistent = 0;
+    if (r.x3 && e.front_persistent) {
+      if (p.split && front_persistent_routed(FRONT_K_ATTNFF, w.dim)) p.persistent |= FRONT_K_ATTNFF;
+      if (p.split && front_persistent_routed(FRONT_K_OUTFF, w.dim)) p.persistent |= FRONT_K_OUTFF;
+      if (p.time_frag && front_persistent_routed(FRONT_K_QKV, w.dim)) p.persistent |= FRONT_K_QKV;
+    }
     return p;
   };
 
@@ -348,7 +356,8 @@
   FusedAttnFFP f;
   f.x = x; f.M = M; f.C = pw.dim; f.b_gates = pw.b_gates; f.rope = rope;
   f.wfrag = pr.split ? pw.w_attnff_frag_x3 : pw.w_attnff_frag[r.fp]; f.b1 = pw.b_ff1; f.b2 = pw.b_ff2;
-  LAUNCH_CAT(CAT_ATTN_FREQ_FUSED, s, launch_attnff_fused(f, pr.split ? BT_PREC_F32X3 : r.fp, s),
+  LAUNCH_CAT(CAT_ATTN_FREQ_FUSED, s,
+             launch_attnff_fused(f, pr.split ? BT_PREC_F32X3 : r.fp, s, pr.persistent & FRONT_K_ATTNFF ? FRONT_FORM_PERSISTENT : FRONT_FORM_TILED),
              "fused frequency attention + feed-forward");
   return BT_OK;
 }
@@ -364,7 +373,8 @@
     qp.b_gates = pw.b_gates; qp.rope = rope;
     qp.q = ws.qf; qp.k = ws.kf; qp.v = ws.vf; qp.gates = ws.gates_h; qp.nbp = ws.nbp;
     qp.x3 = r.x3; qp.status = ws.status;
-    LAUNCH_CAT(CAT_QKV, s, launch_qkv_front(qp, s), "frontend qkv projection");
+    LAUNCH_CAT(CAT_QKV, s, launch_qkv_front(qp, s, pr.persistent & FRONT_K_QKV ? FRONT_FORM_PERSISTENT : FRONT_FORM_TILED),
+               "frontend qkv projection");
     AttnFragP a;
     memset(&a, 0, sizeof a);
     a.q = ws.qf; a.k = ws.kf; a.v = ws.vf; a.gates = ws.gates_h; a.out = ws.ao; a.heads = pw.heads; a.inner = pw.dim;
@@ -378,7 +388,9 @@
     FusedOutFFP f;
     f.x = x; f.M = M; f.C = pw.dim; f.ao = ws.ao; f.wfrag = pr.split ? pw.w_outff_frag_x3 : pw.w_outff_frag[r.fp];
     f.b1 = pw.b_ff1; f.b2 = pw.b_ff2; f.xb = shadow; f.abl = 0; f.shadow_only = shadow && shadow_only && pr.split;
-    LAUNCH_CAT(CAT_FF_FUSED, s, launch_outff_fused(f, pr.split ? BT_PREC_F32X3 : r.fp, s), "fused out-projection + feed-forward");
+    LAUNCH_CAT(CAT_FF_FUSED, s,
+               launch_outff_fused(f, pr.split ? BT_PREC_F32X3 : r.fp, s, pr.persistent & FRONT_K_OUTFF ? FRONT_FORM_PERSISTENT : FRONT_FORM_TILED),
+               "fused out-projection + feed-forward");
     return BT_OK;
   }
   if (int rc = out_proj(pf, pw, r, x, nullptr, ws, M, s)) return rc;
@@ -507,6 +519,7 @@
   std::lock_guard<std::mutex> lock(e->mu);
   if (option == BT_OPT_X3_ATTN_P16 && value >= 0 && value <= 3) { if (e->x3_attn_p16 != value) drop_graphs(e); e->x3_attn_p16 = value; return BT_OK; }
   if (option == BT_OPT_X3_GEMM_FP8 && value >= 0 && value <= 2) { if (e->x3_gemm_fp8 != value) drop_graphs(e); e->x3_gemm_fp8 = value; return BT_OK; }
+  if (option == BT_OPT_FRONT_PERSISTENT && (value == 0 || value == 1)) { if (e->front_persistent != value) drop_graphs(e); e->front_persistent = value; return BT_OK; }
   if (option == BT_OPT_WS_GUARD && value >= 0 && value % 256 == 0) { if (e->ws_guard != value) drop_graphs(e); e->ws_guard = value; return BT_OK; }
   return bt_set_error(BT_ERR_ARG, "unknown engine option / value");
 }
@@ -515,6 +528,7 @@
   if (option == BT_OPT_X3_ATTN_P16) { *value = e->x3_attn_p16; return BT_OK; }
   if (option == BT_OPT_X3_GEMM_FP8) { *value = e->x3_gemm_fp8; return BT_OK; }
   if (option == BT_OPT_WS_GUARD) { *value = e->ws_guard; return BT_OK; }
+  if (option == BT_OPT_FRONT_PERSISTENT) { *value = e->front_persistent; return BT_OK; }
   return bt_set_error(BT_ERR_ARG, "unknown engine option");
 }
 
@@ -1005,24 +1019,41 @@
 }
 
 int bt_outff_fused(void* stream, int prec, const bt_pair_weights* w, const void* d_ao, float* d_x, int64_t M, void* d_xb) {
+  return bt_outff_fused_ex(stream, prec, w, d_ao, d_x, M, d_xb, 0, 0);
+}
+
+static bool bad_form(int prec, int form, int workgroups, int kernel, int dim) {
+  if (form < FRONT_FORM_DEFAULT || form > FRONT_FORM_PERSISTENT || workgroups < 0) return true;
+  return form == FRONT_FORM_PERSISTENT && !(prec == BT_PREC_F32X3 && front_persistent_exists(kernel, dim));
+}
+
+int bt_outff_fused_ex(void* stream, int prec, const bt_pair_weights* w, const void* d_ao, float* d_x, int64_t M, void* d_xb, int form,
+                      int workgroups) {
   if (prec != BT_PREC_F32 && prec != BT_PREC_HALF && prec != BT_PREC_F32X3) return bt_set_error(BT_ERR_ARG, "unknown precision");
   const void* wf = !w ? nullptr : prec == BT_PREC_F32X3 ? w->w_outff_frag_x3 : w->w_outff_frag[prec];
   if (!w || !d_ao || !d_x || M <= 0 || w->dim > 128 || !wf) return bt_set_error(BT_ERR_ARG, "bad argument to bt_outff_fused");
+  if (bad_form(prec, form, workgroups, FRONT_K_OUTFF, w->dim)) return bt_set_error(BT_ERR_ARG, "bt_outff_fused_ex: no such form for this precision / width");
   FusedOutFFP f;
   f.x = d_x; f.M = M; f.C = w->dim; f.ao = d_ao; f.wfrag = wf; f.b1 = w->b_ff1; f.b2 = w->b_ff2;
   f.xb = prec == BT_PREC_F32 ? nullptr : d_xb; f.abl = 0; f.shadow_only = 0;
-  LAUNCH(launch_outff_fused(f, prec, (hipStream_t)stream), "fused out-projection + feed-forward");
+  LAUNCH(launch_outff_fused(f, prec, (hipStream_t)stream, prec == BT_PREC_F32X3 ? form : FRONT_FORM_TILED, workgroups), "fused out-projection + feed-forward");
   return BT_OK;
 }
 
 int bt_attnff_fused(void* stream, int prec, const bt_pair_weights* w, const float* d_rope, float* d_x, int64_t M) {
+  return bt_attnff_fused_ex(stream, prec, w, d_rope, d_x, M, 0, 0);
+}
+
+int bt_attnff_fused_ex(void* stream, int prec, const bt_pair_weights* w, const float* d_rope, float* d_x, int64_t M, int form,
+                       int workgroups) {
   if (prec != BT_PREC_F32 && prec != BT_PREC_HALF && prec != BT_PREC_F32X3) return bt_set_error(BT_ERR_ARG, "unknown precision");
   const void* wf = !w ? nullptr : prec == BT_PREC_F32X3 ? w->w_attnff_frag_x3 : w->w_attnff_frag[prec];
   if (!w || !d_x || !d_rope || M <= 0 || w->dim > 128 || !wf) return bt_set_error(BT_ERR_ARG, "bad argument to bt_attnff_fused");
+  if (bad_form(prec, form, workgroups, FRONT_K_ATTNFF, w->dim)) return bt_set_error(BT_ERR_ARG, "bt_attnff_fused_ex: no such form for this precision / width");
   FusedAttnFFP f;
   f.x = d_x; f.M = M; f.C = w->dim; f.b_gates = w->b_gates; f.rope = d_rope; f.wfrag = wf;
   f.b1 = w->b_ff1; f.b2 = w->b_ff2;
-  LAUNCH(launch_attnff_fused(f, prec, (hipStream_t)stream), "fused frequency attention + feed-forward");
+  LAUNCH(launch_attnff_fused(f, prec, (hipStream_t)stream, prec == BT_PREC_F32X3 ? form : FRONT_FORM_TILED, workgroups), "fused frequency attention + feed-forward");
   return BT_OK;
 }
 
@@ -1079,17 +1110,23 @@
 
 int bt_qkv_front(void* stream, int prec, const bt_pair_weights* w, const float* d_rope, const float* d_x, int B, int T, int F,
                  void* d_q, void* d_k, void* d_v, float* d_gates, int nbp) {
+  return bt_qkv_front_ex(stream, prec, w, d_rope, d_x, B, T, F, d_q, d_k, d_v, d_gates, nbp, 0, 0);
+}
+
+int bt_qkv_front_ex(void* stream, int prec, const bt_pair_weights* w, const float* d_rope, const float* d_x, int B, int T, int F,
+                    void* d_q, void* d_k, void* d_v, float* d_gates, int nbp, int form, int workgroups) {
   if (prec != BT_PREC_HALF && prec != BT_PREC_F32X3) return bt_set_error(BT_ERR_ARG, "bt_qkv_front: BT_PREC_HALF or BT_PREC_F32X3");
   const bool x3 = prec == BT_PREC_F32X3;
   const void* wf = !w ? nullptr : x3 ? w->w_qkv_frag_x3 : w->w_qkv_frag;
   if (!w || !wf || !d_rope || !d_x || !d_q || !d_k || !d_v || !d_gates || w->dim > 128)
     return bt_set_error(BT_ERR_ARG, "bad argument to bt_qkv_front");
+  if (bad_form(prec, form, workgroups, FRONT_K_QKV, w->dim)) return bt_set_error(BT_ERR_ARG, "bt_qkv_front_ex: no such form for this precision / width");
   QkvFrontP p;
   memset(&p, 0, sizeof p);
   p.x = d_x; p.B = B; p.T = T; p.F = F; p.C = w->dim; p.wfrag = wf; p.b_gates = w->b_gates; p.rope = d_rope;
   p.q = d_q; p.k = d_k; p.v = d_v; p.gates = d_gates; p.nbp = nbp; p.x3 = x3;
-  LAUNCH(launch_qkv_front(p, (hipStream_t)stream), "frontend qkv projection");
-  return BT_OK;
-}
-
-}
+  LAUNCH(launch_qkv_front(p, (hipStream_t)stream, x3 ? form : FRONT_FORM_TILED, workgroups), "frontend qkv projection");
+  return BT_OK;
+}
+
+}
diff --git a/beat_this_amd/csrc/fused2.hip b/beat_this_amd/csrc/fused2.hip
--- a/beat_this_amd/csrc/fused2.hip
+++ b/beat_this_amd/csrc/fused2.hip
@@ -1,5 +1,7 @@
 #include <cstdlib>
+#include <mutex>
 #include <type_traits>
+#include <vector>
 
 #include "chain.h"
 #include "kernels.h"
@@ -68,8 +70,14 @@
   }
 };
 
-template <typename T, int C, bool STORE_X = true>
-DEVI void ff_tail(WRing<T, C>& ws, int step0, float (&xn)[C / 32][16], const float* b1s, const float* b2,
+template <typename T, int C>
+struct WResident {
+  const char* lds;
+  DEVI const char* acquire(int s) const { return lds + s * WRing<T, C>::STEP_B; }
+};
+
+template <typename T, int C, bool STORE_X = true, typename WS>
+DEVI void ff_tail(WS& ws, int step0, float (&xn)[C / 32][16], const float* b1s, const float* b2,
                   float* xrow, hf* xbrow, bool ok, int lane, int g) {
   constexpr int KT = C / 32, HB = 4 * C / 32;
   constexpr int TILE_B = WRing<T, C>::TILE_B;
@@ -352,10 +360,269 @@
   }
 }
 
+#ifndef BT_FP_NW_ATTNFF
+#define BT_FP_NW_ATTNFF 8
+#endif
+#ifndef BT_FP_WPS_ATTNFF
+#define BT_FP_WPS_ATTNFF 4
+#endif
+#ifndef BT_FP_ATTNFF_SWAP
+#define BT_FP_ATTNFF_SWAP 0
+#endif
+#ifndef BT_FP_NW_OUTFF
+#define BT_FP_NW_OUTFF 8
+#endif
+#ifndef BT_FP_WPS_OUTFF
+#define BT_FP_WPS_OUTFF 4
+#endif
+
+template <typename T, int C, typename WS>
+DEVI void out_proj_steps(WS& ws, const Frag<T> (&af)[C / 32], float (&xn)[C / 32][16], int lane) {
+  constexpr int KT = C / 32, TILE_B = WRing<T, C>::TILE_B;
+#pragma unroll
+  for (int mt = 0; mt < KT; ++mt) {
+    const char* wb = ws.acquire(mt);
+    f32x16 acc;
+    zero16(acc);
+#pragma unroll
+    for (int kt = 0; kt < KT; ++kt) mma32(acc, lds_frag<T>(wb + kt * TILE_B, lane), af[kt]);
+#pragma unroll
+    for (int r = 0; r < 16; ++r) xn[mt][r] = fmaf(acc[r], OpScale<T>::PW, xn[mt][r]);
+  }
+}
+
+template <typename T, int C, typename WS>
+DEVI void attn_freq_steps(WS& ws, const Frag<T> (&xf)[C / 32], float scale, const float (&sk)[16], const f32x2 (&cs)[8],
+                          const float (&bg)[C / 32], int lane, f32x16 (&acco)[C / 32]) {
+  constexpr int KT = C / 32, H = C / 32, F = 1024 / C, TILE_B = WRing<T, C>::TILE_B;
+  constexpr float PA = OpScale<T>::PA;
+  const int g = lane >> 5, lr = lane & 31;
+  float gate[H];
+  {
+    const char* wb = ws.acquire(0);
+    f32x16 ag;
+    zero16(ag);
+#pragma unroll
+    for (int kt = 0; kt < KT; ++kt) mma32(ag, lds_frag<T>(wb + kt * TILE_B, lane), xf[kt]);
+#pragma unroll
+    for (int hd = 0; hd < H; ++hd) {
+      float v = __shfl(ag[hd], lr);
+      gate[hd] = sigmoidf(fmaf(v, scale, bg[hd]));
+    }
+  }
+
+#pragma unroll
+  for (int mt = 0; mt < KT; ++mt) zero16(acco[mt]);
+#pragma unroll 1
+  for (int hd = 0; hd < H; ++hd) {
+    float pr[16], l = 0.f;
+    {
+      const char* wb = ws.acquire(1 + 2 * hd);
+      f32x16 aq, ak;
+      zero16(aq); zero16(ak);
+#pragma unroll
+      for (int kt = 0; kt < KT; ++kt) {
+        mma32(aq, lds_frag<T>(wb + kt * TILE_B, lane), xf[kt]);
+        mma32(ak, lds_frag<T>(wb + (KT + kt) * TILE_B, lane), xf[kt]);
+      }
+      float q[16], k[16];
+#pragma unroll
+      for (int a = 0; a < 4; ++a)
+#pragma unroll
+        for (int b = 0; b < 2; ++b) {
+          const f32x2 t = cs[2 * a + b];
+          const int r = 4 * a + 2 * b;
+          const float q0 = aq[r] * scale, q1 = aq[r + 1] * scale, k0 = ak[r] * scale, k1 = ak[r + 1] * scale;
+          q[r] = q0 * t.x - q1 * t.y; q[r + 1] = q1 * t.x + q0 * t.y;
+          k[r] = k0 * t.x - k1 * t.y; k[r + 1] = k1 * t.x + k0 * t.y;
+        }
+      f32x16 sc;
+      zero16(sc);
+      mma32(sc, pack_frag<T>(k), pack_frag<T>(q));
+      float mx = -1e30f;
+#pragma unroll
+      for (int r = 0; r < 16; ++r) {
+        sc[r] *= PA;
+        if (F < 32 && ((crow(r, g) ^ lr) & ~(F - 1))) sc[r] = -1e30f;
+        mx = fmaxf(mx, sc[r]);
+      }
+      mx = fmaxf(mx, __shfl_xor(mx, 32));
+#pragma unroll
+      for (int r = 0; r < 16; ++r) {
+        pr[r] = __builtin_amdgcn_exp2f(sc[r] - mx);
+        l += pr[r];
+      }
+      l += __shfl_xor(l, 32);
+    }
+    {
+      const char* wb = ws.acquire(2 + 2 * hd);
+      f32x16 av;
+      zero16(av);
+#pragma unroll
+      for (int kt = 0; kt < KT; ++kt) mma32(av, xf[kt], lds_frag<T>(wb + kt * TILE_B, lane));
+      float v[16];
+#pragma unroll
+      for (int r = 0; r < 16; ++r) v[r] = av[r] * sk[r];
+      f32x16 ao;
+      zero16(ao);
+      mma32(ao, pack_frag<T>(v), pack_frag<T>(pr));
+      float gsel = gate[0];
+#pragma unroll
+      for (int k = 1; k < H; ++k) gsel = hd == k ? gate[k] : gsel;
+      const float fin = gsel / l * PA;
+      float o[16];
+#pragma unroll
+      for (int r = 0; r < 16; ++r) o[r] = ao[r] * fin;
+      const Frag<T> of = pack_frag<T>(o);
+#pragma unroll
+      for (int mt = 0; mt < KT; ++mt) mma32(acco[mt], lds_frag<T>(wb + (KT + mt) * TILE_B, lane), of);
+    }
+  }
+}
+
+template <int NW>
+DEVI void resident_image(char* wl, const void* wfrag, int img_b, const float* b1, int b1_b, int lane, int wave) {
+  lds_image_load<NW, 16>(wl, __builtin_amdgcn_make_buffer_rsrc(const_cast<void*>(wfrag), 0, (unsigned)img_b, 0x00020000), img_b, lane, wave);
+  lds_image_load<NW, 4>(wl + img_b, __builtin_amdgcn_make_buffer_rsrc(const_cast<float*>(b1), 0, (unsigned)b1_b, 0x00020000), b1_b, lane, wave);
+  asm volatile("s_waitcnt vmcnt(0)" ::: "memory");
+  __syncthreads();
+}
+
+template <int NW>
+__global__ __launch_bounds__(NW * 64, BT_FP_WPS_ATTNFF) void attnff_resident_kernel(const FusedAttnFFP p) {
+  typedef hl T;
+  constexpr int C = 32, KT = 1, H = 1, HB = 4;
+  constexpr int IMG_B = (1 + 2 * H + HB) * WRing<T, C>::STEP_B;
+  __shared__ __attribute__((aligned(16))) char wl[IMG_B + 4 * C * 4];
+  const float* b1s = reinterpret_cast<const float*>(wl + IMG_B);
+  const int tid = threadIdx.x, lane = tid & 63, wave = __builtin_amdgcn_readfirstlane(tid >> 6);
+  const int g = lane >> 5, lr = lane & 31;
+  resident_image<NW>(wl, p.wfrag, IMG_B, p.b1, 4 * C * 4, lane, wave);
+  WResident<T, C> ws{wl};
+  const long nblk = (p.M + 31) >> 5, stride = (long)gridDim.x * NW;
+  f32x2 cs[8];
+#pragma unroll
+  for (int a = 0; a < 4; ++a)
+#pragma unroll
+    for (int b = 0; b < 2; ++b) cs[2 * a + b] = *reinterpret_cast<const f32x2*>(p.rope + ((long)lr * 16 + 4 * a + 2 * g + b) * 2);
+  const float bg[H] = {p.b_gates[0]};
+  RawFrag xr;
+  auto load_rows = [&](long blk) {
+    const long tok = blk * 32 + lr;
+    const bool ok = tok < p.M;
+    xr = ldx_raw(p.x + (ok ? tok : 0) * C + 16 * g, ok);
+  };
+  long blk = (long)blockIdx.x * NW + wave;
+  load_rows(blk);
+#pragma unroll 1
+  for (; blk < nblk; blk += stride) {
+    const long tok = blk * 32 + lr;
+    const bool ok = tok < p.M;
+    float* xrow = p.x + (ok ? tok : 0) * C;
+    float ss = 0.f;
+    Frag<T> xf[KT];
+    xf[0] = split_raw(xr, ss);
+#if BT_FP_ATTNFF_SWAP
+    const RawFrag xr0 = xr;
+#endif
+    ss += __shfl_xor(ss, 32);
+    constexpr float PW = OpScale<T>::PW;
+    const float scale = sqrtf((float)C) / fmaxf(sqrtf(ss), 1e-12f) * PW;
+    float sk[16];
+#pragma unroll
+    for (int r = 0; r < 16; ++r) sk[r] = __shfl(scale, crow(r, g));
+    f32x16 acco[KT];
+    attn_freq_steps<T, C>(ws, xf, scale, sk, cs, bg, lane, acco);
+    f32x4 xv[4];
+#if BT_FP_ATTNFF_SWAP
+    load_rows(blk + stride);
+#pragma unroll
+    for (int a = 0; a < 2; ++a)
+#pragma unroll
+      for (int j = 0; j < 4; ++j) {
+        const float lo = xr0.v[2 * a][j], hi = xr0.v[2 * a + 1][j];
+        const auto sw = __builtin_amdgcn_permlane32_swap(__builtin_bit_cast(unsigned, lo), __builtin_bit_cast(unsigned, hi), false, false);
+        xv[a][j] = __builtin_bit_cast(float, sw[0]);
+        xv[a + 2][j] = __builtin_bit_cast(float, sw[1]);
+      }
+#else
+#pragma unroll
+    for (int a = 0; a < 4; ++a) xv[a] = ok ? *reinterpret_cast<const f32x4*>(xrow + 8 * a + 4 * g) : f32x4{0.f, 0.f, 0.f, 0.f};
+    load_rows(blk + stride);
+#endif
+    float xn[KT][16];
+#pragma unroll
+    for (int a = 0; a < 4; ++a)
+#pragma unroll
+      for (int j = 0; j < 4; ++j) xn[0][4 * a + j] = fmaf(acco[0][4 * a + j], PW, xv[a][j]);
+    ff_tail<T, C>(ws, 1 + 2 * H, xn, b1s, p.b2, xrow, nullptr, ok, lane, g);
+  }
+}
+
+template <int NW>
+__global__ __launch_bounds__(NW * 64, BT_FP_WPS_OUTFF) void outff_resident_kernel(const FusedOutFFP p) {
+  typedef hl T;
+  constexpr int C = 32, KT = 1, HB = 4;
+  constexpr int IMG_B = (KT + HB) * WRing<T, C>::STEP_B;
+  __shared__ __attribute__((aligned(16))) char wl[IMG_B + 4 * C * 4];
+  const float* b1s = reinterpret_cast<const float*>(wl + IMG_B);
+  const int tid = threadIdx.x, lane = tid & 63, wave = __builtin_amdgcn_readfirstlane(tid >> 6);
+  const int g = lane >> 5, lr = lane & 31;
+  resident_image<NW>(wl, p.wfrag, IMG_B, p.b1, 4 * C * 4, lane, wave);
+  WResident<T, C> ws{wl};
+  const long nblk = (p.M + 31) >> 5, stride = (long)gridDim.x * NW;
+  RawFrag ar;
+  f32x4 xv[4];
+  auto load_rows = [&](long blk) {
+    const long tok = blk * 32 + lr;
+    const bool ok = tok < p.M;
+    ar = ldg_raw(reinterpret_cast<const float*>(p.ao) + (ok ? tok : 0) * C + 16 * g);
+    const float* xrow = p.x + (ok ? tok : 0) * C;
+#pragma unroll
+    for (int a = 0; a < 4; ++a) xv[a] = ok ? *reinterpret_cast<const f32x4*>(xrow + 8 * a + 4 * g) : f32x4{0.f, 0.f, 0.f, 0.f};
+  };
+  long blk = (long)blockIdx.x * NW + wave;
+  if (blk < nblk) load_rows(blk);
+#pragma unroll 1
+  for (; blk < nblk; blk += stride) {
+    const long tok = blk * 32 + lr;
+    const bool ok = tok < p.M;
+    float* xrow = p.x + (ok ? tok : 0) * C;
+    Frag<T> af[KT];
+    af[0] = split_raw(ar);
+    float xn[KT][16];
+#pragma unroll
+    for (int a = 0; a < 4; ++a)
+#pragma unroll
+      for (int j = 0; j < 4; ++j) xn[0][4 * a + j] = xv[a][j];
+    if (blk + stride < nblk) load_rows(blk + stride);
+    out_proj_steps<T, C>(ws, af, xn, lane);
+    hf* xbrow = p.xb ? reinterpret_cast<hf*>(p.xb) + tok * C * 2 : nullptr;
+    ff_tail<T, C>(ws, KT, xn, b1s, p.b2, xrow, xbrow, ok, lane, g);
+  }
+}
+
+inline bool want_persistent(int form, int kernel, int C) {
+  return form == FRONT_FORM_PERSISTENT || (form == FRONT_FORM_DEFAULT && front_persistent_routed(kernel, C));
+}
+template <typename K, typename P>
+int launch_resident(K kernel, int nw, const P& p, int workgroups, hipStream_t s) {
+  const long need = ((p.M + 31) / 32 + nw - 1) / nw;
+  long wgs = workgroups > 0 ? workgroups : persistent_workgroups(reinterpret_cast<const void*>(kernel), nw * 64);
+  if (wgs <= 0) return -2;
+  if (workgroups <= 0 && wgs > need) wgs = need;
+  hipLaunchKernelGGL(kernel, dim3((unsigned)wgs), dim3(nw * 64), 0, s, p);
+  return (int)hipGetLastError();
+}
+
 template <typename T>
-int launch_outff_t(const FusedOutFFP& p, hipStream_t s) {
+int launch_outff_t(const FusedOutFFP& p, hipStream_t s, int form, int workgroups) {
   dim3 grid((unsigned)((p.M + 127) / 128)), block(256);
   if constexpr (std::is_same<T, hl>::value) {
+    if (want_persistent(form, FRONT_K_OUTFF, p.C)) {
+      if (p.C != 32 || p.shadow_only) return -2;
+      return launch_resident(outff_resident_kernel<BT_FP_NW_OUTFF>, BT_FP_NW_OUTFF, p, workgroups, s);
+    }
     if (p.shadow_only) {
       if (!p.xb) return -2;
       switch (p.C) {
@@ -365,7 +632,7 @@
       }
       return (int)hipGetLastError();
     }
-  } else if (p.shadow_only) {
+  } else if (p.shadow_only || form == FRONT_FORM_PERSISTENT) {
     return -2;
   }
   switch (p.C) {
@@ -377,7 +644,15 @@
   return (int)hipGetLastError();
 }
 template <typename T>
-int launch_attnff_t(const FusedAttnFFP& p, hipStream_t s) {
+int launch_attnff_t(const FusedAttnFFP& p, hipStream_t s, int form, int workgroups) {
+  if constexpr (std::is_same<T, hl>::value) {
+    if (want_persistent(form, FRONT_K_ATTNFF, p.C)) {
+      if (p.C != 32) return -2;
+      return launch_resident(attnff_resident_kernel<BT_FP_NW_ATTNFF>, BT_FP_NW_ATTNFF, p, workgroups, s);
+    }
+  } else if (form == FRONT_FORM_PERSISTENT) {
+    return -2;
+  }
   dim3 grid((unsigned)((p.M + 127) / 128)), block(256);
   switch (p.C) {
     case 32: hipLaunchKernelGGL((attnff_fused_kernel<T, 32>), grid, block, 0, s, p); break;
@@ -396,7 +671,24 @@
 }
 #endif
 
-int launch_outff_fused(const FusedOutFFP& p0, int prec, hipStream_t s) {
+int persistent_workgroups(const void* fn, int block) {
+  struct Entry { int dev; const void* fn; int block, wgs; };
+  static std::mutex mu;
+  static std::vector<Entry> cache;
+  int dev = 0;
+  if (hipGetDevice(&dev) != hipSuccess) return -1;
+  std::lock_guard<std::mutex> lock(mu);
+  for (const Entry& e : cache)
+    if (e.dev == dev && e.fn == fn && e.block == block) return e.wgs;
+  int cus = 0, per_cu = 0;
+  if (hipDeviceGetAttribute(&cus, hipDeviceAttributeMultiprocessorCount, dev) != hipSuccess) return -1;
+  if (hipOccupancyMaxActiveBlocksPerMultiprocessor(&per_cu, fn, block, 0) != hipSuccess) return -1;
+  if (cus <= 0 || per_cu <= 0) return -1;
+  cache.push_back({dev, fn, block, cus * per_cu});
+  return cus * per_cu;
+}
+
+int launch_outff_fused(const FusedOutFFP& p0, int prec, hipStream_t s, int form, int workgroups) {
   if (p0.M <= 0) return -2;
   FusedOutFFP p = p0;
   p.abl = 0;
@@ -404,11 +696,11 @@
   static const int abl = getenv("BT_F2_ABL") ? atoi(getenv("BT_F2_ABL")) : 0;
   p.abl = abl;
 #endif
-  if (prec == BT_PREC_F32X3) return BT_HALF_IS_BF16 ? -2 : launch_outff_t<hl>(p, s);
-  return prec == BT_PREC_F32 ? launch_outff_t<float>(p, s) : launch_outff_t<hf>(p, s);
-}
-int launch_attnff_fused(const FusedAttnFFP& p, int prec, hipStream_t s) {
+  if (prec == BT_PREC_F32X3) return BT_HALF_IS_BF16 ? -2 : launch_outff_t<hl>(p, s, form, workgroups);
+  return prec == BT_PREC_F32 ? launch_outff_t<float>(p, s, form, workgroups) : launch_outff_t<hf>(p, s, form, workgroups);
+}
+int launch_attnff_fused(const FusedAttnFFP& p, int prec, hipStream_t s, int form, int workgroups) {
   if (p.M <= 0) return -2;
-  if (prec == BT_PREC_F32X3) return BT_HALF_IS_BF16 ? -2 : launch_attnff_t<hl>(p, s);
-  return prec == BT_PREC_F32 ? launch_attnff_t<float>(p, s) : launch_attnff_t<hf>(p, s);
-}
+  if (prec == BT_PREC_F32X3) return BT_HALF_IS_BF16 ? -2 : launch_attnff_t<hl>(p, s, form, workgroups);
+  return prec == BT_PREC_F32 ? launch_attnff_t<float>(p, s, form, workgroups) : launch_attnff_t<hf>(p, s, form, workgroups);
+}
diff --git a/beat_this_amd/csrc/kernels.h b/beat_this_amd/csrc/kernels.h
--- a/beat_this_amd/csrc/kernels.h
+++ b/beat_this_amd/csrc/kernels.h
@@ -104,6 +104,18 @@
 int attn_frag_blocks(int L);
 int launch_attn_frag(const AttnFragP& p, hipStream_t s);
 
+#ifndef BT_FRONT_PERSISTENT
+#define BT_FRONT_PERSISTENT 1
+#endif
+enum { FRONT_FORM_DEFAULT = 0, FRONT_FORM_TILED = 1, FRONT_FORM_PERSISTENT = 2 };
+enum { FRONT_K_ATTNFF = 1, FRONT_K_OUTFF = 2, FRONT_K_QKV = 4 };
+inline bool front_persistent_exists(int kernel, int C) { return C == 32 || (kernel == FRONT_K_QKV && C == 64); }
+inline bool front_persistent_routed(int kernel, int C) {
+  if (BT_FRONT_PERSISTENT >= 2) return front_persistent_exists(kernel, C);
+  return BT_FRONT_PERSISTENT && kernel == FRONT_K_QKV && C == 64;
+}
+int persistent_workgroups(const void* fn, int block);
+
 struct QkvFrontP {
   const float* x;
   int B, T, F, C;
@@ -116,7 +128,7 @@
   int x3;
   int* status;
 };
-int launch_qkv_front(const QkvFrontP& p, hipStream_t s);
+int launch_qkv_front(const QkvFrontP& p, hipStream_t s, int form = FRONT_FORM_TILED, int workgroups = 0);
 
 struct FusedFFP {
   float* x; long M; int C;
@@ -135,14 +147,14 @@
   int abl;
   int shadow_only;
 };
-int launch_outff_fused(const FusedOutFFP& p, int prec, hipStream_t s);
+int launch_outff_fused(const FusedOutFFP& p, int prec, hipStream_t s, int form = FRONT_FORM_TILED, int workgroups = 0);
 struct FusedAttnFFP {
   float* x; long M; int C;
   const float* b_gates; const float* rope;
   const void* wfrag;
   const float* b1; const float* b2;
 };
-int launch_attnff_fused(const FusedAttnFFP& p, int prec, hipStream_t s);
+int launch_attnff_fused(const FusedAttnFFP& p, int prec, hipStream_t s, int form = FRONT_FORM_TILED, int workgroups = 0);
 
 struct LayerTailP {
   float* x; long M; int C; int hidden;
diff --git a/beat_this_amd/csrc/qkv_front.hip b/beat_this_amd/csrc/qkv_front.hip
--- a/beat_this_amd/csrc/qkv_front.hip
+++ b/beat_this_amd/csrc/qkv_front.hip
@@ -148,14 +148,172 @@
   if (X3 && p.status && __any(!(amax <= 65504.f)) && lane == 0) atomicOr(p.status, 1);
 }
 
-}
-
-int launch_qkv_front(const QkvFrontP& p, hipStream_t s) {
+template <typename T, int C>
+DEVI void qkv_head_step(const QkvFrontP& p, const char* wb, int hd, const Frag<T> (&xf)[C / 32], float scale, const float (&sk)[16],
+                        const f32x2 (&cs)[8], bool wave_ok, int sq, int blk, int lane, float& amax) {
+  constexpr bool X3 = sizeof(T) == 4;
+  constexpr int KT = C / 32, H = C / 32, TILE_B = 1024 * (int)sizeof(T), BLK_E = X3 ? 2048 : 1024;
+  const int g = lane >> 5, lr = lane & 31;
+  hf* qf = reinterpret_cast<hf*>(p.q);
+  hf* kf = reinterpret_cast<hf*>(p.k);
+  hf* vf = reinterpret_cast<hf*>(p.v);
+  f32x16 aq, ak, av;
+  zero16(aq); zero16(ak); zero16(av);
+#pragma unroll
+  for (int kt = 0; kt < KT; ++kt) {
+    mma32(aq, lds_frag<T>(wb + kt * TILE_B, lane), xf[kt]);
+    mma32(ak, lds_frag<T>(wb + (KT + kt) * TILE_B, lane), xf[kt]);
+    mma32(av, xf[kt], lds_frag<T>(wb + (2 * KT + kt) * TILE_B, lane));
+  }
+  if (wave_ok) {
+    const long base = (((long)sq * H + hd) * p.nbp + blk) * BLK_E;
+#pragma unroll
+    for (int a = 0; a < 4; ++a) {
+      float q[4], k[4];
+#pragma unroll
+      for (int bb = 0; bb < 2; ++bb) {
+        const f32x2 cth = cs[2 * a + bb];
+        const int r = 4 * a + 2 * bb;
+        const float q0 = aq[r] * scale, q1 = aq[r + 1] * scale, k0 = ak[r] * scale, k1 = ak[r + 1] * scale;
+        q[2 * bb] = q0 * cth.x - q1 * cth.y; q[2 * bb + 1] = q1 * cth.x + q0 * cth.y;
+        k[2 * bb] = k0 * cth.x - k1 * cth.y; k[2 * bb + 1] = k1 * cth.x + k0 * cth.y;
+      }
+      const long off = base + (a * 32 + lr) * 8 + 4 * g;
+      if constexpr (X3) {
+        typedef __attribute__((ext_vector_type(2))) unsigned int u32x2;
+        unsigned qh[2], ql[2], kh[2], kl[2];
+        split2q(q[0], q[1], qh[0], ql[0], amax); split2q(q[2], q[3], qh[1], ql[1], amax);
+        split2q(k[0], k[1], kh[0], kl[0], amax); split2q(k[2], k[3], kh[1], kl[1], amax);
+        *reinterpret_cast<u32x2*>(qf + off) = u32x2{qh[0], qh[1]}; *reinterpret_cast<u32x2*>(qf + off + 1024) = u32x2{ql[0], ql[1]};
+        *reinterpret_cast<u32x2*>(kf + off) = u32x2{kh[0], kh[1]}; *reinterpret_cast<u32x2*>(kf + off + 1024) = u32x2{kl[0], kl[1]};
+      } else {
+        *reinterpret_cast<hfx4*>(qf + off) = hfx4{(hf)q[0], (hf)q[1], (hf)q[2], (hf)q[3]};
+        *reinterpret_cast<hfx4*>(kf + off) = hfx4{(hf)k[0], (hf)k[1], (hf)k[2], (hf)k[3]};
+      }
+    }
+#pragma unroll
+    for (int s = 0; s < 2; ++s) {
+      if constexpr (X3) {
+        typedef __attribute__((ext_vector_type(4))) unsigned int u32x4;
+        unsigned oh[4], ol[4];
+#pragma unroll
+        for (int j = 0; j < 4; ++j)
+          split2q(av[8 * s + 2 * j] * sk[8 * s + 2 * j], av[8 * s + 2 * j + 1] * sk[8 * s + 2 * j + 1], oh[j], ol[j], amax);
+        *reinterpret_cast<u32x4*>(vf + base + (s * 64 + lane) * 8) = u32x4{oh[0], oh[1], oh[2], oh[3]};
+        *reinterpret_cast<u32x4*>(vf + base + 1024 + (s * 64 + lane) * 8) = u32x4{ol[0], ol[1], ol[2], ol[3]};
+      } else {
+        hfx8 o;
+#pragma unroll
+        for (int j = 0; j < 8; ++j) o[j] = (hf)(av[8 * s + j] * sk[8 * s + j]);
+        *reinterpret_cast<hfx8*>(vf + base + (s * 64 + lane) * 8) = o;
+      }
+    }
+  }
+}
+
+template <typename T, int C>
+DEVI void qkv_gate_step(const QkvFrontP& p, const char* wb, const Frag<T> (&xf)[C / 32], float scale, bool wave_ok, int sq, int t,
+                        int lane) {
+  constexpr int KT = C / 32, H = C / 32, TILE_B = 1024 * (int)sizeof(T);
+  const int g = lane >> 5;
+  f32x16 ag;
+  zero16(ag);
+#pragma unroll
+  for (int kt = 0; kt < KT; ++kt) mma32(ag, lds_frag<T>(wb + kt * TILE_B, lane), xf[kt]);
+  if (wave_ok && g == 0) {
+#pragma unroll
+    for (int hd = 0; hd < H; ++hd)
+      p.gates[((long)sq * H + hd) * p.nbp * 32 + t] = sigmoidf(fmaf(ag[hd], scale, p.b_gates[hd]));
+  }
+}
+
+#ifndef BT_FP_NW_QKV
+#define BT_FP_NW_QKV 4
+#endif
+#ifndef BT_FP_WPS_QKV
+#define BT_FP_WPS_QKV 3
+#endif
+#ifndef BT_FP_NW_QKV64
+#define BT_FP_NW_QKV64 4
+#endif
+template <int C, int NW>
+__global__ __launch_bounds__(NW * 64, C == 32 ? BT_FP_WPS_QKV : 2) void qkv_front_resident_kernel(const QkvFrontP p) {
+  typedef hl T;
+  constexpr int KT = C / 32, H = C / 32, TILE_B = 1024 * (int)sizeof(T), STEP_B = 3 * KT * TILE_B;
+  constexpr int IMG_B = H * STEP_B + KT * TILE_B;
+  __shared__ __attribute__((aligned(16))) char wl[IMG_B];
+  const int tid = threadIdx.x, lane = tid & 63, wave = __builtin_amdgcn_readfirstlane(tid >> 6);
+  const int g = lane >> 5, lr = lane & 31;
+  lds_image_load<NW, 16>(wl, __builtin_amdgcn_make_buffer_rsrc(const_cast<void*>(p.wfrag), 0, (unsigned)IMG_B, 0x00020000), IMG_B, lane, wave);
+  asm volatile("s_waitcnt vmcnt(0)" ::: "memory");
+  __syncthreads();
+  const int nblk = (p.T + 31) >> 5;
+  const long n_wb = (long)p.B * p.F * nblk, stride = (long)gridDim.x * NW;
+  int sq = 0, blk = 0;
+  RawFrag xr[KT];
+  f32x2 cs[8];
+  auto load_rows = [&](long wb_id) {
+    sq = (int)(wb_id / nblk); blk = (int)(wb_id - (long)sq * nblk);
+    const int b = sq / p.F, f = sq - b * p.F;
+    const int t = blk * 32 + lr;
+    const bool ok = t < p.T;
+    const float* xrow = p.x + (((long)b * p.T + (ok ? t : 0)) * p.F + f) * C;
+#pragma unroll
+    for (int kt = 0; kt < KT; ++kt) xr[kt] = ldx_raw(xrow + kt * 32 + 16 * g, ok);
+#pragma unroll
+    for (int a = 0; a < 4; ++a)
+#pragma unroll
+      for (int bb = 0; bb < 2; ++bb)
+        cs[2 * a + bb] = *reinterpret_cast<const f32x2*>(p.rope + ((long)(ok ? t : 0) * 16 + 4 * a + 2 * g + bb) * 2);
+  };
+  long wb_id = (long)blockIdx.x * NW + wave;
+  if (wb_id < n_wb) load_rows(wb_id);
+  float amax = 0.f;
+#pragma unroll 1
+  for (; wb_id < n_wb; wb_id += stride) {
+    const int sq0 = sq, blk0 = blk, t = blk0 * 32 + lr;
+    float ss = 0.f;
+    Frag<T> xf[KT];
+#pragma unroll
+    for (int kt = 0; kt < KT; ++kt) xf[kt] = split_raw(xr[kt], ss);
+    f32x2 cs0[8];
+#pragma unroll
+    for (int i = 0; i < 8; ++i) cs0[i] = cs[i];
+    if (wb_id + stride < n_wb) load_rows(wb_id + stride);
+    ss += __shfl_xor(ss, 32);
+    const float scale = sqrtf((float)C) / fmaxf(sqrtf(ss), 1e-12f) * OpScale<T>::PW;
+    float sk[16];
+#pragma unroll
+    for (int r = 0; r < 16; ++r) sk[r] = __shfl(scale, crow(r, g));
+#pragma unroll
+    for (int hd = 0; hd < H; ++hd) qkv_head_step<T, C>(p, wl + hd * STEP_B, hd, xf, scale, sk, cs0, true, sq0, blk0, lane, amax);
+    qkv_gate_step<T, C>(p, wl + H * STEP_B, xf, scale, true, sq0, t, lane);
+  }
+  if (p.status && __any(!(amax <= 65504.f)) && lane == 0) atomicOr(p.status, 1);
+}
+
+template <int C>
+int launch_qkv_resident(const QkvFrontP& p, long n_wb, int workgroups, hipStream_t s) {
+  constexpr int NW = C == 32 ? BT_FP_NW_QKV : BT_FP_NW_QKV64;
+  const long need = (n_wb + NW - 1) / NW;
+  long wgs = workgroups > 0 ? workgroups : persistent_workgroups(reinterpret_cast<const void*>(qkv_front_resident_kernel<C, NW>), NW * 64);
+  if (wgs <= 0) return -2;
+  if (workgroups <= 0 && wgs > need) wgs = need;
+  hipLaunchKernelGGL((qkv_front_resident_kernel<C, NW>), dim3((unsigned)wgs), dim3(NW * 64), 0, s, p);
+  return (int)hipGetLastError();
+}
+
+}
+
+int launch_qkv_front(const QkvFrontP& p, hipStream_t s, int form, int workgroups) {
   if (p.B <= 0 || p.T <= 0 || p.F <= 0 || p.nbp < attn_frag_blocks(p.T)) return -2;
   const long n_wb = (long)p.B * p.F * ((p.T + 31) / 32);
   dim3 grid((unsigned)((n_wb + 3) / 4)), block(256);
+  if (form == FRONT_FORM_PERSISTENT && !(p.x3 && front_persistent_exists(FRONT_K_QKV, p.C))) return -2;
   if (p.x3) {
     if (BT_HALF_IS_BF16) return -2;
+    if (form == FRONT_FORM_PERSISTENT || (form == FRONT_FORM_DEFAULT && front_persistent_routed(FRONT_K_QKV, p.C)))
+      return p.C == 32 ? launch_qkv_resident<32>(p, n_wb, workgroups, s) : launch_qkv_resident<64>(p, n_wb, workgroups, s);
     switch (p.C) {
       case 32: hipLaunchKernelGGL((qkv_front_kernel<hl, 32>), grid, block, 0, s, p); break;
       case 64: hipLaunchKernelGGL((qkv_front_kernel<hl, 64>), grid, block, 0, s, p); break;
diff --git a/beat_this_amd/pack.py b/beat_this_amd/pack.py
--- a/beat_this_amd/pack.py
+++ b/beat_this_amd/pack.py
@@ -329,7 +329,7 @@
 
     MAX_WORKSPACES = 4
     SHRINK_AFTER = 8
-    OPTIONS = {"x3_attn_p16": 1, "x3_gemm_fp8": 2, "ws_guard": 3}
+    OPTIONS = {"x3_attn_p16": 1, "x3_gemm_fp8": 2, "ws_guard": 3, "front_persistent": 4}
 
     def set_options(self, opts: dict) -> None:
         for name in opts:
diff --git a/include/beat_this_amd.h b/include/beat_this_amd.h
--- a/include/beat_this_amd.h
+++ b/include/beat_this_amd.h
@@ -90,6 +90,7 @@
 #define BT_OPT_X3_ATTN_P16 1
 #define BT_OPT_X3_GEMM_FP8 2
 #define BT_OPT_WS_GUARD 3
+#define BT_OPT_FRONT_PERSISTENT 4
 int bt_engine_set_option(bt_engine* e, int option, int value);
 int bt_engine_get_option(const bt_engine* e, int option, int* value);
 size_t bt_workspace_bytes(const bt_engine* e, int B, int T, int prec);
@@ -278,6 +279,12 @@
 int bt_ff_fused(void* stream, int prec, const bt_pair_weights* w, float* d_x, int64_t M);
 int bt_outff_fused(void* stream, int prec, const bt_pair_weights* w, const void* d_ao, float* d_x, int64_t M, void* d_xb);
 int bt_attnff_fused(void* stream, int prec, const bt_pair_weights* w, const float* d_rope, float* d_x, int64_t M);
+int bt_qkv_front_ex(void* stream, int prec, const bt_pair_weights* w, const float* d_rope, const float* d_x, int B, int T, int F,
+                    void* d_q, void* d_k, void* d_v, float* d_gates, int nbp, int form, int workgroups);
+int bt_outff_fused_ex(void* stream, int prec, const bt_pair_weights* w, const void* d_ao, float* d_x, int64_t M, void* d_xb, int form,
+                      int workgroups);
+int bt_attnff_fused_ex(void* stream, int prec, const bt_pair_weights* w, const float* d_rope, float* d_x, int64_t M, int form,
+                       int workgroups);
 int bt_layer_tail(void* stream, const bt_pair_weights* w, int hidden, const void* d_ao, float* d_x, int64_t M, void* d_xb,
                   float* d_ssq_out);
 
```

Result: no change. 62630, median of 2 (-0.1%).
